# bghira/universal-metal-flash-attention

Measured on AMD Instinct MI355X. Metric: SDPA fwd TFLOPS (bf16) + int8 speedup, B=1 H=24 S=4096 D=128, 1/2/4/8 GPU, higher is better.
Workload: dtype bf16

## Files before the change

universal-metal-flash-attention_amd/csrc/fa_fwd16_w64.hip:

```cpp
#include <algorithm>
#include <cmath>
#include <cstdlib>
#include <type_traits>

#include "fa_fwd16_w64_params.h"

namespace umfa {

#define W64_I8 0
#define W64_BODY_INC "fa_fwd16_w64_body.inc"
#define W64_T __bf16
#define W64_MFMA "v_mfma_f32_32x32x16_bf16"
#define W64_MFMA_QK "v_mfma_f32_32x32x16_bf16"
#define W64_MSUM "v_mfma_f32_4x4x4_16b_bf16"
#define W64_ONES_BITS 0x3f803f80u
#define W64_LAZY_PARTS 1
#define W64_CVT "v_cvt_pk_bf16_f32"
#define W64_KERNEL fa_fwd16_w64_bf16
#include "fa_fwd16_w64_kernel.inc"
#undef W64_T
#undef W64_MFMA
#undef W64_MFMA_QK
#undef W64_MSUM
#undef W64_ONES_BITS
// ... 152 lines not shown
}

static int w64_cu_count() { return device_cu_count(); }

static bool w64_is_window(const FwdParams& p) { return p.mask_kind == MK_WINDOW; }
static uint32_t w64_win_left(const FwdParams& p) { return p.win_left < p.Sq ? p.win_left : p.Sq; }
static uint32_t w64_win_right(const FwdParams& p) { return p.causal ? 0u : (p.win_right < p.Skv ? p.win_right : p.Skv); }
static uint32_t w64_tiles_per_item(const FwdParams& p) {
    const uint32_t T = (p.Skv + 63) / 64;
    if (!w64_is_window(p)) return T;
    const uint64_t tw = ((uint64_t)w64_win_left(p) + 63) / 64 + (255ull + w64_win_right(p)) / 64 + 1;
    return tw < T ? (uint32_t)tw : T;
}

static uint32_t w64_grid(const FwdParams& p);

struct W64Cost { float t0, c_seg, t_step, c_fold, cast_a, cast_tbps; };
struct R128Cost { float t0, c_item, tau1, f2, f3, cast_a, cast_tbps, c_tail, g16; };
static const W64Cost kW64Cost[2][2] = {
    {{1.9654f, 5.6596f, 1.0164f, 1.8670f, 4.8672f, 4.1271f}, {9.3795f, 0.0000f, 1.1237f, 48.8617f, 2.7924f, 2.2478f}},
    {{0.4243f, 10.5808f, 1.5482f, 3.2266f, 3.4018f, 3.8643f}, {0.0000f, 6.7763f, 1.4334f, 52.2072f, 2.5095f, 2.6358f}}};
static const R128Cost kR128Cost[2][2] = {
    {{1.9627f, 3.9851f, 0.6098f, 2.0000f, 1.0000f, 0.0000f, 20.0000f, 1.3083f, 0.9054f}, {0.2449f, 5.9446f, 0.7894f, 1.4608f, 1.0000f, 0.0000f, 20.0000f, 0.6456f, 0.8727f}},
    {{0.0000f, 8.3967f, 1.0624f, 2.0000f, 2.8549f, 5.1811f, 20.0000f, 3.2320f, 1.0191f}, {0.0000f, 8.4229f, 1.2922f, 1.7176f, 1.0000f, 0.0000f, 12.7398f, 0.4806f, 0.8916f}}};
struct CbalCost { float a1, b1, a2, b2; };
static const CbalCost kCbalCost[2] = {{8.5243f, 1.1660f, 11.3665f, 1.3999f}, {11.7677f, 1.5652f, 21.1185f, 1.7844f}};

static double route_v_megabytes(const FwdParams& p) {
    return (double)(p.vs[0] == 0 ? 1u : p.B) * (p.vs[1] == 0 ? 1u : p.H) * p.Skv * p.D * 2.0 * 1e-6;
}

double fwd_w64_predict_us(const FwdParams& p) {
    const W64Cost& c = kW64Cost[p.D == 64 ? 0 : 1][p.causal ? 1 : 0];
    const uint64_t nqb = (p.Sq + 255) / 256, items = (uint64_t)p.B * p.H * nqb, T = (p.Skv + 63) / 64;
    const uint64_t G = w64_grid(p);
    double segs, steps, fold = 0.0;
    if (p.causal) {
        const uint64_t jobs = (uint64_t)p.B * p.H * ((nqb + 1) / 2), rounds = (jobs + G - 1) / G;
        uint64_t longest = 0;
        for (uint64_t j = 0; j < (nqb + 1) / 2; ++j) {
            const uint64_t a = std::min<uint64_t>(T, 4 * j + 4), m = nqb - 1 - j, b2 = m != j ? std::min<uint64_t>(T, 4 * m + 4) : 0;
            longest = std::max(longest, a + b2);
        }
        segs = 2.0 * rounds;
        steps = (double)(rounds * longest);
    } else {
        const uint64_t full = items / G, rem = items % G;
        segs = (double)(full + (rem ? 1 : 0));
        steps = (double)(full * T + (rem ? (rem * T + G - 1) / G : 0));
        if (rem) fold = std::max((double)G / (double)rem - 1.0, 0.0);
    }
    const double cast = (p.in_prec == P_BF16 && p.pv16) ? c.cast_a + 2.0 * route_v_megabytes(p) / c.cast_tbps : 0.0;
    return c.t0 + cast + segs * c.c_seg + steps * c.t_step + fold * c.c_fold;
}

double fwd_16_predict_us(const FwdParams& p) {
    const R128Cost& c = kR128Cost[p.D == 64 ? 0 : 1][p.causal ? 1 : 0];
    const uint64_t cus = (uint64_t)w64_cu_count();
    const uint64_t nqb = (p.Sq + 127) / 128, items = (uint64_t)p.B * p.H * nqb, T = (p.Skv + 63) / 64;
    const uint32_t R = (p.D == 128 && !p.causal) ? 3u : 2u;
    const double fr[4] = {0.0, 1.0, c.f2, c.f3};
    const double tau1 = (p.in_prec == P_BF16 && p.pv16) ? c.tau1 : c.tau1 * c.g16;
    const FwdSplitPlan plan = fwd_16_split_plan(p);
    const uint64_t k = plan.nsplit > 1 ? plan.nsplit : 1;
    const double n = (double)(items * k) / (double)cus;
    double body;
    if (plan.cbal) {
        const uint64_t lastq = nqb - 1;
        const double h = 0.5 * (double)(std::min<uint64_t>(T, 2) + std::min<uint64_t>(T, (lastq * 128 + 128 + 63) / 64));
        const CbalCost& cb = kCbalCost[p.D == 64 ? 0 : 1];
        const double one = cb.a1 + cb.b1 * h, two = cb.a2 + cb.b2 * h;
        const uint64_t full = (uint64_t)(n / 2.0);
        const double rest = n - 2.0 * (double)full;
        body = ((double)full * two + (rest > 1e-9 ? (rest <= 1.0 ? one : two) : 0.0)) * (p.in_prec == P_BF16 && p.pv16 ? 1.0 : (double)c.g16) - c.t0;
    } else if (p.causal) {
        uint64_t tot = 0, longest = 0;
        for (uint64_t qb = 0; qb < nqb; ++qb) {
            const uint64_t len = std::min<uint64_t>(T, (qb * 128 + 128 + 63) / 64);
            tot += len;
            longest = std::max(longest, len);
        }
        tot *= (uint64_t)p.B * p.H;
        if (n <= (double)R) {
            const int r = std::max(1, (int)std::ceil(n));
            body = c.c_item + (double)longest * tau1 * fr[r];
        } else {
            const double thr = (double)tot / (double)cus * tau1 * fr[R] / R + n * c.c_item / R;
            body = std::max(thr + c.c_tail * (double)longest * tau1, c.c_item + (double)longest * tau1 * fr[R]);
        }
    } else {
        const double L = (double)T / (double)k;
        const uint64_t full = (uint64_t)(n / R);
        const int rest = (int)std::ceil(n - (double)(full * R) - 1e-9);
        body = (double)full * (c.c_item + L * tau1 * fr[R]) + (rest > 0 ? c.c_item + L * tau1 * fr[rest] : 0.0) + (k > 1 ? c.c_tail * (double)k : 0.0);
    }
    const bool cast_on = p.in_prec == P_BF16 && p.pv16 && route_v_megabytes(p) * 1e6 >= (double)((size_t)16 << 20) && p.Sq >= 1024;
    const double cast = cast_on ? c.cast_a + 2.0 * route_v_megabytes(p) / c.cast_tbps : 0.0;
    return c.t0 + cast + body;
}

bool fwd_w64_supported(const FwdParams& p) {
    if (tuning().no_w64.load(std::memory_order_relaxed) || !fwd_16_supported(p)) return false;
    if ((p.D != 128 && p.D != 64) || (p.mask_kind != MK_NONE && p.mask_kind != MK_WINDOW && p.mask_kind != MK_BOOL && p.mask_kind != MK_F16 && p.mask_kind != MK_BF16 && p.mask_kind != MK_F32)) return false;
    if (p.mask_kind == MK_F16 || p.mask_kind == MK_BF16 || p.mask_kind == MK_F32) {
        if (tuning().no_w64_mask.load(std::memory_order_relaxed) || tuning().no_w64_bias.load(std::memory_order_relaxed) || !p.mask || (p.D != 128 && p.D != 64) || p.rope_cos || p.causal) return false;
        if (p.in_prec == P_BF16 && !p.pv16) return false;
        const bool ragged = !p.mask_padded && (p.Sq % 64 != 0 || p.Skv % 64 != 0);
        if (p.Sq < 256 || p.Skv < 64 || (p.Sq % 64 != 0 && p.Sq < 1024) || ((p.Skv + 63) / 64) > 1024u) return false;
        if (ragged && tuning().no_w64_ragged_mask.load(std::memory_order_relaxed)) return false;
        if (p.out_prec != P_FP32 && p.out_prec != p.in_prec) return false;
        if (p.ms[3] != 1) return false;
        if (!mask_needs_copy(p)) {
            if (((uintptr_t)p.mask & 15) != 0 || (p.ms[0] & 7) != 0 || (p.ms[1] & 7) != 0 || (p.ms[2] & 7) != 0) return false;
        } else if (tuning().no_w64_ragged_mask.load(std::memory_order_relaxed) && p.mask_kind == MK_F16) {
            return false;
        }
        if (p.mask_kind != MK_F32 && p.ms[2] != 0 && (uint64_t)p.ms[2] * 2 * 64 > 0x7fffffffull) return false;
        if (mask_copy_bytes(p) > ((size_t)1 << 30)) return false;
        if (p.mask_kind == MK_F32) {
            if (tuning().no_w64_f32_mask.load(std::memory_order_relaxed)) return false;
            const int ratio = tuning().f32_mask_ratio.load(std::memory_order_relaxed);
            if (ratio > 0) {
                const uint64_t Bm = p.ms[0] != 0 ? p.B : 1, Hm = p.ms[1] != 0 ? p.H : 1, eb = 2;
                const uint64_t mask_bytes = Bm * Hm * p.Sq * p.Skv * 4, qkvo = (uint64_t)p.B * p.H * p.D * ((uint64_t)p.Sq * (eb + 4) + 2ull * p.Skv * eb);
                if (mask_bytes > (uint64_t)ratio * qkvo) return false;
            } else if (!mask_flags_worthwhile(p)) {
                return false;
            }
        }
        if (w64_grid(p) > 512u) return false;
        if (tuning().force_w64.load(std::memory_order_relaxed)) return true;
        const uint64_t blocks = (uint64_t)p.B * p.H * ((p.Sq + 255) / 256), cus = (uint64_t)w64_cu_count();
        return blocks >= cus;
    }
    if (p.mask_kind == MK_BOOL) {
        if (tuning().no_w64_mask.load(std::memory_order_relaxed) || !p.mask || (p.D != 128 && p.D != 64) || p.rope_cos) return false;
        if (p.in_prec == P_BF16 && !p.pv16) return false;
        if (p.Skv < 64 || p.Sq < 256 || (p.Sq % 256 != 0 && p.Sq < 1024) || ((p.Skv + 63) / 64) > 1024u) return false;
        if (p.out_prec != P_FP32 && p.out_prec != p.in_prec) return false;
        const uint64_t blocks = (uint64_t)p.B * p.H * ((p.Sq + 255) / 256), cus = (uint64_t)w64_cu_count();
        if (w64_grid(p) > 512u) return false;
        if (tuning().force_w64.load(std::memory_order_relaxed)) return true;
        if (p.causal) return false;
        if (p.in_prec == P_BF16 && p.Sq < 1024) return false;
        if (p.in_prec == P_BF16 && p.Sq < 2048 && ((p.ms[0] == 0 && p.ms[1] == 0) || p.ms[2] == 0)) return false;
        return blocks >= cus || (p.ms[2] == 0 && blocks * ((p.Skv + 63) / 64) >= cus * 10) || ((p.ms[0] != 0 || p.ms[1] != 0) && blocks * 8 >= cus * 3);
    }
    if (w64_is_window(p) && p.rope_cos) return false;
    if (p.D == 64 && p.rope_cos) return false;
    if (p.Skv < 64 || p.Sq < 256 || (p.Sq % 256 != 0 && p.Sq < 1024)) return false;
    if (p.out_prec != P_FP32 && p.out_prec != p.in_prec) return false;
    if (!tuning().force_w64.load(std::memory_order_relaxed)) {
        if (w64_is_window(p)) {
            const uint64_t cus = (uint64_t)w64_cu_count(), nqb = (p.Sq + 255) / 256;
            const uint64_t items = (uint64_t)p.B * p.H * nqb, steps = items * w64_tiles_per_item(p);
            if (items % cus != 0 && steps < cus * 10) return false;
        } else if (!(fwd_w64_predict_us(p) < fwd_16_predict_us(p))) {
            return false;
        }
    }
    return true;
}

static uint32_t w64_grid(const FwdParams& p) {
    if (p.mask_kind == MK_BOOL || p.mask_kind == MK_F16 || p.mask_kind == MK_BF16) {
        const uint64_t items = (uint64_t)p.B * p.H * ((p.Sq + 255) / 256);
        const uint64_t cus = (uint64_t)w64_cu_count();
        if (const int gi = tuning().w64_grid.load(std::memory_order_relaxed)) {
            if (gi > 0 && (uint64_t)gi <= cus && (uint64_t)gi <= items && gi <= 512) return (uint32_t)gi;
        }
        const uint64_t gmax = cus < 512 ? cus : 512;
        if (items < cus) return (uint32_t)((p.ms[2] == 0 && items * ((p.Skv + 63) / 64) >= cus * 10) ? gmax : items);
        return (uint32_t)gmax;
    }
    const bool pairs = p.causal && !w64_is_window(p);
    uint64_t total = (uint64_t)p.B * p.H * ((p.Sq + 255) / 256) * w64_tiles_per_item(p);
    if (pairs) total = (uint64_t)p.B * p.H * (((p.Sq + 255) / 256 + 1) / 2);
    const uint32_t cus = (uint32_t)w64_cu_count();
    if (const int gi = tuning().w64_grid.load(std::memory_order_relaxed)) {
        const uint32_t g = (uint32_t)gi;
        if (gi > 0 && g <= cus && g <= total) return g;
    }
    if (!pairs) {
        const uint64_t items = (uint64_t)p.B * p.H * ((p.Sq + 255) / 256);
        if (items < cus && cus / items >= 2 && items * (cus / items) <= total) return (uint32_t)(items * (cus / items));
        if (items < cus && 2 * (uint64_t)w64_tiles_per_item(p) * (cus - items) < 35 * cus) return (uint32_t)items;
    }
    return total < cus ? (uint32_t)total : cus;
}

uint32_t fwd_w64_grid(const FwdParams& p) { return w64_grid(p); }

FwdW64Plan fwd_w64_plan(const FwdParams& p) {
    FwdW64Plan plan;
    const uint32_t items = p.B * p.H * ((p.Sq + 255) / 256);
    (void)items;
    plan.cnt_bytes = ((size_t)w64_grid(p) * sizeof(uint32_t) + 255) & ~(size_t)255;
    plan.buf_bytes = (size_t)2 * w64_grid(p) * (4 * 2 * 17 * 1024);
    return plan;
}

template <typename KFN>
static hipError_t launch_w64_kernel(KFN kfn, const FwdParams& p, const W64Params& wp, hipStream_t stream) {
    const uint32_t grid = w64_grid(p);
    const size_t lds = 65536 + 4 * 32 * (512 + 16) + 64 + 4096 + 8192 + 2048 + 64;
    if (hipError_t e = ensure_dynamic_lds((const void*)kfn, lds); e != hipSuccess) return e;
    hipLaunchKernelGGL(kfn, dim3(grid), dim3(256), lds, stream, wp);
    return hipGetLastError();
}

hipError_t launch_fwd_w64(const FwdParams& p, float* part_buf, uint32_t* part_cnt, hipStream_t stream, const char** name) {
    if (!fwd_w64_supported(p) || !part_buf || !part_cnt) return hipErrorNotSupported;
    W64Params wp;
    wp.q = p.q; wp.k = p.k; wp.v = p.v; wp.o = p.o; wp.lse = p.lse;
    for (int i = 0; i < 3; ++i) { wp.qs[i] = p.qs[i]; wp.ks[i] = p.ks[i]; wp.vs[i] = p.vs[i]; }
    wp.B = p.B; wp.H = p.H; wp.Sq = p.Sq; wp.Skv = p.Skv;
    wp.scale = p.scale;
    wp.n_items = p.B * p.H * ((p.Sq + 255) / 256);
    wp.T = (p.Skv + 63) / 64;
    wp.part_buf = part_buf;
    wp.part_cnt = part_cnt;
    w64_softmax_policy(p.in_prec, &wp.tau, &wp.lazy);
    wp.skew = (uint32_t)tuning().w64_skew.load(std::memory_order_relaxed);
    if (tuning().w64_skew.load(std::memory_order_relaxed) == -1) wp.skew = 0xffffffffu;
    wp.rope_cos = p.rope_cos; wp.rope_sin = p.rope_sin; wp.rope_tb = p.rope_tb;
    wp.vsc = p.vsc; wp.vsc_bs = p.vsc_bs; wp.vsc_hs = p.vsc_hs;
    if (p.in_prec == P_BF16 && p.pv16 && !p.vsc) return hipErrorInvalidValue;
    wp.Tw = wp.T; wp.win_left = wp.win_right = 0;
    const bool rope = p.rope_cos != nullptr, window = w64_is_window(p), fp32o = p.out_prec == P_FP32, maska = p.mask_kind == MK_F16, maskt = p.mask_kind == MK_BOOL || maska;
    wp.mask = nullptr; wp.mask_s[0] = wp.mask_s[1] = wp.mask_s[2] = 0;
    wp.guard = maska ? p.guard : nullptr;
    if (p.guard && (!maska || p.guard_want != 0u)) return hipErrorInvalidValue;
    if (maskt) {
        if ((!maska && !p.mk_bits) || !p.mk_list || !p.mk_cnt) return hipErrorInvalidValue;
        if (maska) { wp.mask = p.mask; wp.mask_s[0] = p.ms[0]; wp.mask_s[1] = p.ms[1]; wp.mask_s[2] = p.ms[2]; }
        wp.mk_bits = p.mk_bits; wp.mk_list = p.mk_list; wp.mk_cnt = p.mk_cnt;
        wp.mk_bs = p.mk_bs; wp.mk_hs = p.mk_hs; wp.mk_nrb64 = p.mk_nrb64;
        wp.mk_prefix = p.mk_prefix;
#ifndef W64_LAB_MASK_FORCE_LAZY
        if (p.ms[2] != 0 || p.causal || tuning().no_w64_mask_lazy.load(std::memory_order_relaxed)) wp.lazy = 0;
#endif
    }
    if (rope && p.out_prec != p.in_prec) return hipErrorNotSupported;
    if (window) {
        wp.Tw = w64_tiles_per_item(p);
        wp.win_left = (int32_t)w64_win_left(p);
        wp.win_right = (int32_t)w64_win_right(p);
    }
#define W64_FAMILY(FAM, T16, HAS_ROPE)                                                                                         \
    do {                                                                                                                       \
        if constexpr (HAS_ROPE >= 2) {        \
            if (maskt) return fp32o ? launch_w64_kernel(FAM<float, false, false, false, true>, p, wp, stream) : launch_w64_kernel(FAM<T16, false, false, false, true>, p, wp, stream); \
        }                                                                                                                      \
        if constexpr (HAS_ROPE == 1 || HAS_ROPE == 2) {                                                                        \
            if (rope) return p.causal ? launch_w64_kernel(FAM<T16, true, true>, p, wp, stream) : launch_w64_kernel(FAM<T16, false, true>, p, wp, stream); \
        }                                                                                                                      \
        if (window) return fp32o ? launch_w64_kernel(FAM<float, false, false, true>, p, wp, stream) : launch_w64_kernel(FAM<T16, false, false, true>, p, wp, stream); \
        if (p.causal) return fp32o ? launch_w64_kernel(FAM<float, true>, p, wp, stream) : launch_w64_kernel(FAM<T16, true>, p, wp, stream); \
        return fp32o ? launch_w64_kernel(FAM<float, false>, p, wp, stream) : launch_w64_kernel(FAM<T16, false>, p, wp, stream); \
    } while (0)
    static const char* const names[3][2][3] = {
        {{"fa_fwd16_w64<bf16,128>", "fa_fwd16_w64<bf16,128,rope>", "fa_fwd16_w64<bf16,128,window>"},
         {"fa_fwd16_w64<bf16,64>", "fa_fwd16_w64<bf16,64,rope>", "fa_fwd16_w64<bf16,64,window>"}},
        {{"fa_fwd16_w64<bf16,128,pv16>", "fa_fwd16_w64<bf16,128,pv16,rope>", "fa_fwd16_w64<bf16,128,pv16,window>"},
         {"fa_fwd16_w64<bf16,64,pv16>", "fa_fwd16_w64<bf16,64,pv16,rope>", "fa_fwd16_w64<bf16,64,pv16,window>"}},
        {{"fa_fwd16_w64<fp16,128>", "fa_fwd16_w64<fp16,128,rope>", "fa_fwd16_w64<fp16,128,window>"},
         {"fa_fwd16_w64<fp16,64>", "fa_fwd16_w64<fp16,64,rope>", "fa_fwd16_w64<fp16,64,window>"}}};
    if (p.D == 64 && rope) return hipErrorNotSupported;
    const int fam = p.in_prec == P_BF16 ? (p.pv16 ? 1 : 0) : 2;
    if (maskt && fam == 0) return hipErrorNotSupported;
    if (maska && fam == 0) return hipErrorNotSupported;
    if (maska) {
        *name = p.D == 64 ? (fam == 1 ? "fa_fwd16_w64<bf16,64,pv16,bias>" : "fa_fwd16_w64<fp16,64,bias>") : (fam == 1 ? "fa_fwd16_w64<bf16,128,pv16,bias>" : "fa_fwd16_w64<fp16,128,bias>");
        return launch_fwd_w64_bias(wp, fam, fp32o, w64_grid(p), 65536 + 4 * 32 * (512 + 16) + 64 + 4096 + 8192 + 2048 + 64, stream, (int)p.D);
    }
    *name = maska ? (fam == 1 ? "fa_fwd16_w64<bf16,128,pv16,bias>" : "fa_fwd16_w64<fp16,128,bias>") : maskt ? (p.D == 64 ? (fam == 1 ? "fa_fwd16_w64<bf16,64,pv16,mask>" : "fa_fwd16_w64<fp16,64,mask>")
                               : (fam == 1 ? "fa_fwd16_w64<bf16,128,pv16,mask>" : "fa_fwd16_w64<fp16,128,mask>"))
                  : names[fam][p.D == 64 ? 1 : 0][rope ? 1 : window ? 2 : 0];
    if (p.D == 64) {
        if (fam == 0) W64_FAMILY(fa_fwd16_w64d64_bf16, __bf16, 0);
        if (fam == 1) W64_FAMILY(fa_fwd16_w64d64_bf16pv16, __bf16, 3);
        W64_FAMILY(fa_fwd16_w64d64_f16, _Float16, 3);
    }
    if (fam == 0) W64_FAMILY(fa_fwd16_w64_bf16, __bf16, 1);
    if (fam == 1) W64_FAMILY(fa_fwd16_w64_bf16pv16, __bf16, 2);
    W64_FAMILY(fa_fwd16_w64_f16, _Float16, 2);
#undef W64_FAMILY
}

bool fwd_w64_i8_supported(const FwdParams& p) {
    if (tuning().no_w64.load(std::memory_order_relaxed) || p.D != 128) return false;
    if (!(p.scale > 0.0f)) return false;
    if (p.Skv < 64 || p.Sq < 256 || (p.Sq % 256 != 0 && p.Sq < 1024)) return false;
    if (p.mask_kind == MK_BOOL && p.mask) {
        if (tuning().no_w64_mask.load(std::memory_order_relaxed) || p.causal) return false;
        if (((p.Skv + 63) / 64) > 1024u || w64_grid(p) > 512u) return false;
        if (tuning().force_w64.load(std::memory_order_relaxed)) return true;
        const uint64_t blocks = (uint64_t)p.B * p.H * ((p.Sq + 255) / 256), cus = (uint64_t)w64_cu_count();
        return blocks >= cus || (p.ms[2] == 0 && blocks * ((p.Skv + 63) / 64) >= cus * 10) || ((p.ms[0] != 0 || p.ms[1] != 0) && blocks * 8 >= cus * 3);
    }
    return p.mask_kind == MK_NONE && !p.mask;
}

hipError_t launch_fwd_w64_i8(const FwdParams& p, const QuantViews& v, float* part_buf, uint32_t* part_cnt, hipStream_t stream) {
    if (!fwd_w64_i8_supported(p) || !part_buf || !part_cnt || v.dpq != 128) return hipErrorNotSupported;
    W64I8Params wp;
    wp.q8 = v.q8; wp.k8 = v.k8; wp.v16 = (const _Float16*)v.v16;
    wp.v8 = v.v8; wp.v_e8 = v.v_e8;
    wp.q_scale = v.q_scale; wp.k_scale = v.k_scale;
    wp.o = p.o; wp.lse = p.lse;
    wp.B = p.B; wp.H = p.H; wp.Sq = p.Sq; wp.Skv = p.Skv; wp.nqblk = v.nqblk; wp.nkblk = v.nkblk;
    wp.scale = p.scale;
    wp.n_items = p.B * p.H * ((p.Sq + 255) / 256);
    wp.T = (p.Skv + 63) / 64;
    wp.part_buf = part_buf;
    wp.part_cnt = part_cnt;
    w64_softmax_policy(P_FP16, &wp.tau, &wp.lazy);
    wp.skew = (uint32_t)tuning().w64_skew.load(std::memory_order_relaxed);
    wp.vsc = v.v8 ? nullptr : p.vsc;
    const uint32_t grid = w64_grid(p);
    const bool f8 = v.v8 != nullptr, maskt = p.mask_kind == MK_BOOL;
    wp.mk_bits = wp.mk_list = wp.mk_cnt = nullptr; wp.mk_bs = wp.mk_hs = wp.mk_nrb64 = 0;
    if (maskt) {
        if (f8 || p.causal || !p.mk_bits || !p.mk_list || !p.mk_cnt) return hipErrorInvalidValue;
        wp.mk_bits = p.mk_bits; wp.mk_list = p.mk_list; wp.mk_cnt = p.mk_cnt;
        wp.mk_bs = p.mk_bs; wp.mk_hs = p.mk_hs; wp.mk_nrb64 = p.mk_nrb64;
        if (p.ms[2] != 0 || tuning().no_w64_mask_lazy.load(std::memory_order_relaxed)) wp.lazy = 0;
    }
    const size_t lds = maskt ? 65536 + 4 * 32 * (512 + 16) + 64 + 4096 + 8192 + 2048 + 64 : 65536 + 4 * 32 * (512 + 16) + 16;
    auto kfn = f8 ? (p.causal ? fa_fwd_w64_i8f8<float, true> : fa_fwd_w64_i8f8<float, false>)
                  : maskt ? fa_fwd_w64_i8<float, false, true>
                          : (p.causal ? fa_fwd_w64_i8<float, true> : fa_fwd_w64_i8<float, false>);
    if (hipError_t e = ensure_dynamic_lds((const void*)kfn, lds); e != hipSuccess) return e;
    hipLaunchKernelGGL(kfn, dim3(grid), dim3(256), lds, stream, wp);
    return hipGetLastError();
}

}
```

universal-metal-flash-attention_amd/csrc/fa_fwd16_w64_kernel.inc:

```

#ifdef W64_ABL_NOBAR
#define W64_ITER_BARRIER() asm volatile("" ::: "memory")
#elif defined(W64_LAB_WAITSTAMP)
#define W64_ITER_BARRIER()                                                                         \
    do {                                                                                           \
        asm volatile("s_waitcnt lgkmcnt(0)" ::: "memory");                                         \
        const unsigned long long w0_ = __builtin_amdgcn_s_memtime();                               \
        asm volatile("s_waitcnt vmcnt(0) lgkmcnt(0)" ::: "memory");                                \
        const unsigned long long w1_ = __builtin_amdgcn_s_memtime();                               \
        asm volatile("s_waitcnt lgkmcnt(0)\n\ts_barrier" ::: "memory");                            \
        const unsigned long long w2_ = __builtin_amdgcn_s_memtime();                               \
        asm volatile("s_waitcnt lgkmcnt(0)" ::: "memory");                                         \
        st_wait += w1_ - w0_;                                                                      \
        st_bar += w2_ - w1_;                                                                       \
    } while (0)
#elif defined(W64_ABL_VMCNT8)
#define W64_ITER_BARRIER() asm volatile("s_waitcnt vmcnt(8) lgkmcnt(0)\n\ts_barrier" ::: "memory")
#else
#define W64_ITER_BARRIER() asm volatile("s_waitcnt vmcnt(0) lgkmcnt(0)\n\ts_barrier" ::: "memory")
#endif
#ifdef W64_ABL_NODMA
#define W64_DMA_ON 0
#else
#define W64_DMA_ON 1
// ... 74 lines not shown
    typedef typename M::V4 V4;
#if !W64_I8
    typedef V8 KF;
#endif
    typedef unsigned u32x4_t __attribute__((ext_vector_type(4)));
    constexpr int NDB = W64_DP / 32;
    constexpr int ROW_IN = 2 * W64_DP;
    constexpr int VSLOT = W64_F8 ? 8192 : 64 * ROW_IN;
    constexpr int VRING = W64_I8 ? 32768 : 2 * KSLOT;
    const float TAU = p.tau;
#if !W64_I8
    if constexpr (MASKA) {
        if (p.guard != nullptr && *p.guard != 0u) return;
    }
#endif

    extern __shared__ __attribute__((aligned(16))) char smem[];
    const int tid = threadIdx.x, lane = tid & 63, ql = lane & 31, hi = lane >> 5;
    const int uw = __builtin_amdgcn_readfirstlane(tid >> 6);
    const uint32_t lds0 = (uint32_t)(size_t)((LDS_AS char*)smem);
#ifndef W64_LAZY_PARTS
#define W64_LAZY_PARTS 0
#endif
#if W64_MSUM_ON && !W64_F8
    ms_init_ones(W64_ONES_BITS);
#define W64_L_ZERO() ms_zero_l()
#define W64_L_SCALE(A0, A1) ms_scale_l((A0), (A1))
#define W64_L_READ(L0, L1) ms_read_l((L0), (L1))
#elif !W64_F8
#define W64_L_ZERO() do { _Pragma("unroll") for (int j_ = 0; j_ < 4; ++j_) l4[0][j_] = l4[1][j_] = 0.0f; } while (0)
#define W64_L_SCALE(A0, A1) do { _Pragma("unroll") for (int j_ = 0; j_ < 4; ++j_) { l4[0][j_] *= (A0); l4[1][j_] *= (A1); } } while (0)
#define W64_L_READ(L0, L1) ((L0) = (l4[0][0] + l4[0][1]) + (l4[0][2] + l4[0][3]), (L1) = (l4[1][0] + l4[1][1]) + (l4[1][2] + l4[1][3]))
#endif
#if W64_LAZY_PARTS
    const bool lazy_on = p.lazy != 0;
    bool force_exact = false;
#ifndef W64_LAZY_HI16
#define W64_LAZY_HI16 0x1p10f
#endif
    constexpr float LAZY_HI = W64_LAZY_PARTS == 2 ? W64_LAZY_HI16 : 0x1p30f, LAZY_OVF = W64_LAZY_PARTS == 2 ? 0x1p15f : 0x1p100f;
    constexpr float LAZY_LOST = W64_LAZY_PARTS == 2 ? 0x1p-6f : 0x1p-100f;
    constexpr unsigned OVF_FLAG_OFF = 65536u + 4u * 32u * (512u + 16u);
    if (threadIdx.x == 0) *(volatile uint32_t LDS_AS*)(uintptr_t)(lds0 + OVF_FLAG_OFF) = 0u;
    __builtin_amdgcn_s_waitcnt(0xc07f);
#endif

    auto tr_read_at = [](unsigned addr) -> V4 {
        if constexpr (__is_same(T, __bf16)) {
            return __builtin_bit_cast(V4, __builtin_amdgcn_ds_read_tr16_b64_v4bf16((bf16x4_t LDS_AS*)(uintptr_t)addr));
        } else {
            return __builtin_bit_cast(V4, __builtin_amdgcn_ds_read_tr16_b64_v4i16((s16x4 LDS_AS*)(uintptr_t)addr));
        }
    };

    unsigned kaddr[KS];
#pragma unroll
    for (int ks = 0; ks < KS; ++ks)
        kaddr[ks] = lds0 + (unsigned)(W64_I8 ? k8_off_128(ql, 2 * ks + hi) : k_off<W64_DP>(ql, 2 * ks + hi));
    auto k_frag = [&](int koff, int ks) -> KF { return *(const KF LDS_AS*)(uintptr_t)(kaddr[ks] + (unsigned)koff); };
    const int tr_qq = (lane >> 2) & 3, tr_pp = lane & 3, tr_g1 = (lane >> 4) & 1;
    unsigned vtr[NDB];
#pragma unroll
    for (int i = 0; i < NDB; ++i)
        vtr[i] = lds0 + (unsigned)(v_off<W64_DP>(4 * hi + tr_qq, 4 * i + 2 * tr_g1 + (tr_pp >> 1)) + 8 * (tr_pp & 1));
    auto v_frag = [&](int voff, int db, int st) -> V8 {
        const V4 lo = tr_read_at(vtr[db] + (unsigned)(voff + (16 * st) * ROW_IN));
        const V4 hi4 = tr_read_at(vtr[db] + (unsigned)(voff + (16 * st + 8) * ROW_IN));
        return __builtin_shufflevector(lo, hi4, 0, 1, 2, 3, 4, 5, 6, 7);
    };
    (void)v_frag;

#if W64_F8
    typedef int i32x8 __attribute__((ext_vector_type(8)));
    const unsigned v8addr = lds0 + (unsigned)lane * 16u;
    auto v8_frag = [&](int voff, int db) -> i32x8 {
        const i32x4 lo = *(const i32x4 LDS_AS*)(uintptr_t)(v8addr + (unsigned)(voff + db * 2048));
        const i32x4 hi4 = *(const i32x4 LDS_AS*)(uintptr_t)(v8addr + (unsigned)(voff + db * 2048 + 1024));
        return __builtin_shufflevector(lo, hi4, 0, 1, 2, 3, 4, 5, 6, 7);
    };
#endif

#if W64_I8
    const int k_stride_b = 128, v_stride_b = 256, q_stride_b = 128;
#else
    const int k_stride_b = (int)p.ks[2] * 2, v_stride_b = (int)p.vs[2] * 2, q_stride_b = (int)p.qs[2] * 2;
#endif
    int kdma0[4], vdma0[4];
    {
        constexpr int RPI = 1024 / ROW_IN, CPR = ROW_IN / 16, PPW = 16 / RPI;
        const int d_r = lane / CPR, d_c = lane % CPR;
        (void)d_c;
#pragma unroll
        for (int j = 0; j < 4; ++j) {
            const int row = (uw * PPW + (j % PPW)) * RPI + d_r;
            (void)row;
#if W64_F8
            vdma0[j] = ((uw * 2 + (j & 1)) * 64 + lane) * 16;
#else
            vdma0[j] = row * v_stride_b + (v_off<W64_DP>(row, d_c) - row * ROW_IN);
#endif
#if W64_I8
            const int krow = (uw * 2 + (j & 1)) * 8 + (lane >> 3), kc = lane & 7;
            kdma0[j] = krow * 128 + (k8_off_128(krow, kc) - krow * 128);
#else
            kdma0[j] = row * k_stride_b + (k_off<W64_DP>(row, d_c) - row * ROW_IN);
#endif
        }
    }
    const int k_step0 = 64 * k_stride_b, v_step0 = W64_F8 ? 8192 : 64 * v_stride_b;
    const unsigned lds_wave = __builtin_amdgcn_readfirstlane(lds0 + (unsigned)uw * (W64_F8 ? 2048u : (unsigned)(16 * ROW_IN)));
#if W64_I8
    const unsigned lds_wave_k = __builtin_amdgcn_readfirstlane(lds0 + (unsigned)uw * 2048u);
    float c2 = 0.0f;
#ifndef W64_I8_NOBIAS
    constexpr float I8_BIAS = 12582912.0f;
#if W64_F8
    f8_init_consts();
#else
    i8_init_bias();
#endif
    float nmb[2] = {0.f, 0.f};
#endif
#else
    const unsigned lds_wave_k = lds_wave;
    const float c2 = p.scale * UMFA_LOG2E;
#endif

    const uint32_t G = gridDim.x;
    const uint32_t w = xcd_remap(blockIdx.x, G);
    const uint32_t T_ = p.T;
    const uint32_t nqb = (p.Sq + 255) / 256;
    const bool ktail = (p.Skv & 63) != 0;
    const uint32_t jobs_per_head = (nqb + 1) / 2, n_jobs = p.B * p.H * jobs_per_head;
    uint32_t Tst = T_;
    int win_left = 0, win_right = 0;
#if !W64_I8
    if constexpr (WINDOW) { Tst = p.Tw; win_left = p.win_left; win_right = p.win_right; }
#endif
    (void)win_left; (void)win_right;
    constexpr bool SPARSE = CAUSAL || WINDOW || MASKT;
    auto mk_slab = [&](uint32_t bh_) -> uint32_t { return (bh_ / p.H) * p.mk_bs + (bh_ % p.H) * p.mk_hs; };
    auto item_tiles = [&](uint32_t item) -> uint32_t {
        if constexpr (MASKT) return p.mk_cnt[mk_slab(item / nqb) * nqb + item % nqb];
        if constexpr (!CAUSAL) return Tst;
        const uint32_t q = item % nqb;
        return 4 * q + 4 < T_ ? 4 * q + 4 : T_;
    };
    const bool whole_rem = !CAUSAL && p.skew == 0xffffffffu;
    const uint32_t full_rounds = CAUSAL ? 0u : whole_rem ? (p.n_items + G - 1) / G : p.n_items / G;
    const uint32_t rem_items = (CAUSAL || whole_rem) ? 0u : p.n_items - full_rounds * G;
    constexpr unsigned MK_PREFIX_OFF = 65536u + 4u * 32u * (512u + 16u) + 64u + 4096u + 8192u;
    if constexpr (MASKT) {
        if (rem_items) {
            volatile uint32_t* const pf = (volatile uint32_t*)(smem + MK_PREFIX_OFF);
            const uint32_t first = full_rounds * G, j0 = threadIdx.x, j1 = threadIdx.x + 256u;
            for (uint32_t j = threadIdx.x; j < rem_items; j += 256u) {
                const uint32_t it_ = first + j;
                pf[1 + j] = p.mk_cnt[mk_slab(it_ / nqb) * nqb + it_ % nqb];
            }
            if (threadIdx.x == 0) pf[0] = 0u;
            __syncthreads();
            for (uint32_t off = 1; off < rem_items; off <<= 1) {
                const uint32_t a0 = (j0 < rem_items && j0 >= off) ? pf[1 + j0 - off] : 0u;
                const uint32_t a1 = (j1 < rem_items && j1 >= off) ? pf[1 + j1 - off] : 0u;
                __syncthreads();
                if (j0 < rem_items) pf[1 + j0] += a0;
                if (j1 < rem_items) pf[1 + j1] += a1;
                __syncthreads();
            }
        }
    }
    auto mk_prefix_at = [&](uint32_t j) -> uint32_t {
        return (uint32_t)__builtin_amdgcn_readfirstlane((int)((volatile const uint32_t*)(smem + MK_PREFIX_OFF))[j]);
    };
    (void)mk_prefix_at;
    auto item_start = [&](uint32_t litem) -> uint64_t {
        if constexpr (MASKT) return mk_prefix_at(litem);
        return (uint64_t)litem * Tst;
    };
    auto item_of_step = [&](uint64_t step) -> uint32_t {
        if constexpr (MASKT) {
            uint32_t lo = 0, hi_ = rem_items - 1;
            while (lo < hi_) {
                const uint32_t mid = (lo + hi_ + 1) >> 1;
                if (mk_prefix_at(mid) <= step) lo = mid; else hi_ = mid - 1;
            }
            return lo;
        }
        return (uint32_t)(step / Tst);
    };
    const uint64_t total = MASKT ? (rem_items ? (uint64_t)mk_prefix_at(rem_items) : 0ull) : (uint64_t)rem_items * Tst;
    const uint32_t skew = (!MASKT && rem_items && G == 2 * rem_items && p.skew != 0xffffffffu && 2 * p.skew < Tst) ? p.skew : 0u;
    const uint32_t Gs = (MASKT && total < G) ? (uint32_t)total : G;
    auto slice_bound = [&](uint32_t g) -> uint32_t {
        if constexpr (MASKT) { if (g >= Gs) return (uint32_t)total; }
        return (uint32_t)(total * g / Gs) - ((g & 1u) ? skew : 0u);
    };
    const uint32_t s_begin = slice_bound(w), s_end = slice_bound(w + 1);
#ifdef W64_LAB_GAPSTAMP
    unsigned long long st_g[4] = {0, 0, 0, 0}, st_gprev = 0;
#define W64_GSTAMP(k)                                                                            \
    do {                                                                                         \
        asm volatile("s_waitcnt lgkmcnt(0)" ::: "memory");                                       \
        const unsigned long long now_ = __builtin_amdgcn_s_memtime();                            \
        asm volatile("s_waitcnt lgkmcnt(0)" ::: "memory");                                       \
        if (st_gprev) st_g[k] += now_ - st_gprev;                                                \
        st_gprev = now_;                                                                         \
    } while (0)
#endif
#ifdef W64_LAB_FSTAMP
    unsigned long long fs_now[8] = {0, 0, 0, 0, 0, 0, 0, 0};
    uint32_t fs_acc[8] = {0, 0, 0, 0, 0, 0, 0, 0}, fs_last = 0, fs_tiles = 0;
    bool fs_valid = false;
#define W64_FSTAMP(k) asm volatile("s_memtime %0" : "=s"(fs_now[k]))
#define W64_FSTAMP_END(n)                                                                           \
    do {                                                                                            \
        asm volatile("s_waitcnt lgkmcnt(0)" ::: "memory");                                          \
        if (fs_valid) fs_acc[0] += (uint32_t)fs_now[0] - fs_last;                                   \
        _Pragma("unroll") for (int k_ = 1; k_ < (n); ++k_) fs_acc[k_] += (uint32_t)fs_now[k_] - (uint32_t)fs_now[k_ - 1]; \
        fs_last = (uint32_t)fs_now[(n) - 1];                                                        \
        fs_valid = true;                                                                            \
        ++fs_tiles;                                                                                 \
    } while (0)
#endif
#ifdef W64_LAB_STAMPS
    const unsigned long long st_rt0 = __builtin_amdgcn_s_memrealtime(), st_ck0 = __builtin_amdgcn_s_memtime();
    unsigned long long st_pro = 0, st_loop = 0, st_drain = 0, st_epi = 0, st_t = 0, st_wait = 0, st_bar = 0;
#define W64_STAMP(acc) do { const unsigned long long now_ = __builtin_amdgcn_s_memtime(); acc += now_ - st_t; st_t = now_; } while (0)
#else
#define W64_STAMP(acc) do { } while (0)
#endif

    uint32_t ntail = 0;
    bool tail_first = false;
    if (s_end > s_begin) {
        const uint32_t it0 = item_of_step(s_begin), it1 = item_of_step(s_end - 1);
        ntail = it1 - it0 + 1;
        tail_first = item_start(it0) != s_begin;
    }
    const uint32_t my_jobs = CAUSAL ? (n_jobs > w ? (n_jobs - w + G - 1) / G : 0u) : 0u;
    const uint32_t nseg = CAUSAL ? 2 * my_jobs : full_rounds + ntail;

    auto make_srd = [&](const void* base, uint32_t bytes) {
        const unsigned long long a = (unsigned long long)base;
        i32x4 d;
        d[0] = __builtin_amdgcn_readfirstlane((int)(a & 0xffffffffu));
        d[1] = __builtin_amdgcn_readfirstlane((int)((a >> 32) & 0xffffu));
        d[2] = __builtin_amdgcn_readfirstlane((int)bytes);
        d[3] = 0x00020000;
        return d;
    };
    auto seg_decode = [&](uint32_t si_, uint32_t& item_, uint32_t& t0_, uint32_t& n_, uint32_t& litem_, bool& desc_) -> bool {
        litem_ = 0;
        desc_ = false;
        if constexpr (CAUSAL) {
            const uint32_t job = (si_ >> 1) * G + w, jbh = job / jobs_per_head, jj = job % jobs_per_head;
            desc_ = (si_ & 1) != 0;
            const uint32_t q = desc_ ? nqb - 1 - jj : jj;
            if (desc_ && q == jj) return false;
            item_ = jbh * nqb + q;
            t0_ = 0;
            n_ = item_tiles(item_);
        } else {
            const bool is_tail = tail_first ? (si_ < ntail) : (si_ >= full_rounds);
            if (is_tail) {
                const uint32_t ti = tail_first ? si_ : si_ - full_rounds;
                litem_ = item_of_step(s_begin) + ti;
                const uint64_t ist = item_start(litem_), ien = MASKT ? item_start(litem_ + 1) : ist + Tst;
                const uint64_t sb = ist > s_begin ? ist : s_begin, se = ien < s_end ? ien : s_end;
                t0_ = (uint32_t)(sb - ist);
                n_ = (uint32_t)(se - sb);
                item_ = full_rounds * G + litem_;
            } else {
                item_ = (tail_first ? si_ - ntail : si_) * G + w;
                if (item_ >= p.n_items) return false;
                t0_ = 0;
                n_ = MASKT ? item_tiles(item_) : Tst;
            }
        }
        return true;
    };
#ifndef W64_MFMA16
#define W64_MFMA16 "v_mfma_f32_16x16x32_bf16"
#endif
#ifndef W64_PREFETCH_NEXT
#define W64_PREFETCH_NEXT 0
#endif
#if W64_PREFETCH_NEXT
    static_assert(!WINDOW, "the prefetch computes the next segment's first tile without the window offset");
    KF qf[2][KS];
    int kdma[4];
    bool have_pref = false;
#endif
#if W64_I8
    constexpr bool ROPE_ON = false;
    (void)ROPE_ON;
#else
    constexpr bool ROPE_ON = ROPE;
    (void)ROPE_ON;
#endif

    for (uint32_t si = 0; si < nseg; ++si) {
        int tid_s = tid;
        if constexpr (MASKA) asm volatile("" : "+v"(tid_s));
        const int lane = tid_s & 63, ql = lane & 31, hi = lane >> 5;
#ifdef W64_LAB_STAMPS
        if (si) { asm volatile("s_waitcnt vmcnt(0)" ::: "memory"); W64_STAMP(st_epi); }
#endif
        uint32_t item, t0, n, litem = 0;
        bool desc = false;
#if W64_LAZY_PARTS
        bool lazy = lazy_on && !force_exact;
        force_exact = false;
        bool ovf = false;
#endif
        if (!seg_decode(si, item, t0, n, litem, desc)) continue;
#if !W64_PREFETCH_NEXT
        KF qf[2][KS];
        int kdma[4];
        constexpr bool have_pref = false;
#endif
        auto issue_q_k0 = [&](uint32_t item_, uint32_t tfirst_, int k_step_) {
            const uint32_t bh_ = item_ / nqb, qblk_ = item_ % nqb;
            const uint32_t q0_ = qblk_ * 256 + (uint32_t)uw * 64;
#if W64_I8
            const int8_t* qp_ = p.q8 + (int64_t)bh_ * p.Sq * 128;
            const int8_t* kp_ = p.k8 + (int64_t)bh_ * p.Skv * 128;
            const auto q_rsrc_ = __builtin_amdgcn_make_buffer_rsrc((void*)qp_, 0, (int)(p.Sq * 128u), 0x00020000);
            const i32x4 k_srd_ = make_srd(kp_, p.Skv * 128u);
#else
            const uint32_t b_ = bh_ / p.H, h_ = bh_ % p.H;
            const T* qp_ = (const T*)p.q + ((int64_t)b_ * p.qs[0] + (int64_t)h_ * p.qs[1]);
            const T* kp_ = (const T*)p.k + ((int64_t)b_ * p.ks[0] + (int64_t)h_ * p.ks[1]);
            const auto q_rsrc_ = __builtin_amdgcn_make_buffer_rsrc((void*)qp_, 0, (int)((p.Sq - 1) * (uint32_t)q_stride_b + ROW_IN), 0x00020000);
            const i32x4 k_srd_ = make_srd(kp_, (p.Skv - 1) * (uint32_t)k_stride_b + ROW_IN);
#endif
#pragma unroll
            for (int j = 0; j < 4; ++j) kdma[j] = kdma0[j] + (int)tfirst_ * k_step0;
#pragma unroll
            for (int j = 0; j < (W64_I8 ? 2 : W64_DP / 32); ++j) {
                asm volatile("s_mov_b32 m0, %0\n\ts_nop 0\n\tbuffer_load_dwordx4 %1, %2, 0 offen lds"
                             ::"s"(lds_wave_k + j * 1024), "v"(kdma[j]), "s"(k_srd_) : "memory");
                kdma[j] += k_step_;
            }
#pragma unroll
            for (int qb = 0; qb < 2; ++qb) {
                const int qoff = (int)(q0_ + 32 * qb + ql) * q_stride_b + 16 * hi;
#pragma unroll
                for (int ks = 0; ks < KS; ++ks)
                    qf[qb][ks] = __builtin_bit_cast(KF, __builtin_amdgcn_raw_buffer_load_b128(q_rsrc_, qoff + 32 * ks, 0, 0));
            }
        };
        const uint32_t Ti = item_tiles(item);
        const uint32_t bh = item / nqb, qblk = item % nqb;
        const uint32_t b = bh / p.H, h = bh % p.H;
        const uint32_t q0 = qblk * 256 + (uint32_t)uw * 64;

#if W64_I8
        (void)b; (void)h;
        const int8_t* qp = p.q8 + (int64_t)bh * p.Sq * 128;
        const int8_t* kp = p.k8 + (int64_t)bh * p.Skv * 128;
#if W64_F8
        const uint8_t* vp = p.v8 + (int64_t)bh * T_ * 8192;
        const uint32_t* __restrict__ vexp = p.v_e8 + (int64_t)bh * p.nkblk;
        const i32x4 v_srd = make_srd(vp, T_ * 8192u);
#else
        const _Float16* vp = p.v16 + (int64_t)bh * p.Skv * 128;
        const i32x4 v_srd = make_srd(vp, p.Skv * 256u);
#endif
        const auto q_rsrc = __builtin_amdgcn_make_buffer_rsrc((void*)qp, 0, (int)(p.Sq * 128u), 0x00020000);
        const i32x4 k_srd = make_srd(kp, p.Skv * 128u);
        const float sq = (q0 < p.Sq ? p.q_scale[(int64_t)bh * p.nqblk + q0 / 64] : 0.0f) * p.scale * UMFA_LOG2E;
        const float* __restrict__ ksc = p.k_scale + (int64_t)bh * p.nkblk;
        int sc_win = -1;
        float ksc_w = 0.0f;
#if W64_F8
        unsigned vexp_w = 0x7f7f7f7fu;
#endif
        auto load_scale_window = [&](uint32_t tile) {
            const int win = (int)(tile >> 6);
            if (win != sc_win) {
                sc_win = win;
                const uint32_t t = ((uint32_t)win << 6) + (uint32_t)lane;
                ksc_w = t < p.nkblk ? ksc[t] : 0.0f;
#if W64_F8
                vexp_w = t < p.nkblk ? vexp[t] : 0x7f7f7f7fu;
#endif
                __builtin_amdgcn_s_waitcnt(0x0F70);
            }
        };
        auto k_scale_of = [&](uint32_t tile) -> float {
            load_scale_window(tile);
            return __builtin_bit_cast(float, __builtin_amdgcn_readlane(__builtin_bit_cast(int, ksc_w), (int)(tile & 63u)));
        };
#ifndef W64_I8_NOBIAS
        float kmax = 0.0f;
        for (uint32_t t = lane; t < p.nkblk; t += 64) kmax = fmaxf(kmax, ksc[t]);
#pragma unroll
        for (int off = 32; off > 0; off >>= 1) kmax = fmaxf(kmax, __shfl_xor(kmax, off, 64));
        const float bias_bound = fmaxf(I8_BIAS * 1.25f * sq * kmax, 0x1p-60f);
        const int eb = ((__builtin_bit_cast(int, bias_bound) >> 23) & 0xff) - 126;
        const float mgrid = __builtin_bit_cast(float, (eb - 24 + 127) << 23), inv_mgrid = __builtin_bit_cast(float, (24 - eb + 127) << 23);
        const float cgrid = __builtin_bit_cast(float, (eb - 46 + 127) << 23), inv_cgrid = __builtin_bit_cast(float, (46 - eb + 127) << 23);
#define W64_C2(x) (__builtin_rintf((x) * inv_cgrid) * cgrid)
#define W64_MGRID(x) (__builtin_ceilf((x) * inv_mgrid) * mgrid)
#if W64_LAZY_PARTS
        lazy = lazy && eb <= 24;
#endif
#else
#define W64_C2(x) (x)
#define W64_MGRID(x) (x)
#endif
#else
#define W64_MGRID(x) (x)
        const T* qp = (const T*)p.q + ((int64_t)b * p.qs[0] + (int64_t)h * p.qs[1]);
        const T* kp = (const T*)p.k + ((int64_t)b * p.ks[0] + (int64_t)h * p.ks[1]);
        const T* vp = (const T*)p.v + ((int64_t)b * p.vs[0] + (int64_t)h * p.vs[1]);
        const auto q_rsrc = __builtin_amdgcn_make_buffer_rsrc((void*)qp, 0, (int)((p.Sq - 1) * (uint32_t)q_stride_b + ROW_IN), 0x00020000);
        const i32x4 k_srd = make_srd(kp, (p.Skv - 1) * (uint32_t)k_stride_b + ROW_IN);
        const i32x4 v_srd = make_srd(vp, (p.Skv - 1) * (uint32_t)v_stride_b + ROW_IN);
#endif

        uint32_t toff = 0;
        if constexpr (WINDOW) {
            const uint32_t blk0 = qblk * 256u;
            const uint32_t lo = blk0 > (uint32_t)win_left ? (blk0 - (uint32_t)win_left) / 64u : 0u;
            toff = lo < T_ - Tst ? lo : T_ - Tst;
        }
        uint32_t tfirst = toff + (desc ? n - 1 : t0);
        int k_step = desc ? -k_step0 : k_step0, v_step = desc ? -v_step0 : v_step0;
        const int dm_step = desc ? -64 : 64;
        const uint32_t* __restrict__ mk_lst = MASKT ? p.mk_list + (uint64_t)(mk_slab(bh) * nqb + qblk) * T_ * 2 : nullptr;
        constexpr unsigned MK_LIST_OFF = 65536u + 4u * 32u * (512u + 16u) + 64u + 4096u;
        const unsigned mk_list_lds = lds0 + MK_LIST_OFF;
        uint32_t mk_tile = 0, mk_cls = 2, mk_next = 0;
        uint32_t mk_ncls = 0;
        (void)mk_ncls;
        auto mk_class = [&](uint32_t) -> uint32_t { return mk_cls; };
        auto tile_at = [&](uint32_t i) -> uint32_t {
            if constexpr (MASKT) return mk_tile;
            return toff + (desc ? n - 1 - i : t0 + i);
        };
        auto mk_steps = [&](uint32_t i) {
            if constexpr (MASKT) {
                typedef unsigned u32x2_t __attribute__((ext_vector_type(2)));
                const u32x2_t e = *(const u32x2_t LDS_AS*)(uintptr_t)(mk_list_lds + 8u * i);
                const uint32_t e0 = (uint32_t)__builtin_amdgcn_readfirstlane((int)e[0]), e1 = (uint32_t)__builtin_amdgcn_readfirstlane((int)e[1]);
                mk_tile = e0 & 0xffffu;
                mk_cls = (e0 >> (16 + 2 * uw)) & 3u;
                mk_ncls = (e0 >> (24 + 2 * uw)) & 3u;
                mk_next = e1 & 0xffffu;
                k_step = ((int)(e1 >> 16) - (int)mk_next) * k_step0;
                v_step = ((int)mk_next - (int)mk_tile) * v_step0;
            }
        };
        unsigned mwc[2] = {0u, 0u}, mtmp;
        i32x4 mk_srd = {0, 0, 0, 0};
        constexpr unsigned MK_RING_OFF = 65536u + 4u * 32u * (512u + 16u) + 64u;
        const unsigned mk_ring = __builtin_amdgcn_readfirstlane(lds0 + MK_RING_OFF + (unsigned)uw * 1024u);
        if constexpr (MASKT && !MASKA) {
            const uint32_t rb64 = 4 * qblk + (uint32_t)uw;
            mk_srd = make_srd(p.mk_bits + ((uint64_t)mk_slab(bh) * p.mk_nrb64 + rb64) * T_ * 128, rb64 < p.mk_nrb64 ? T_ * 512u : 0u);
        }
#if !W64_I8
        typedef unsigned u32x2_t __attribute__((ext_vector_type(2)));
        u32x2_t mta[2][2] = {};
        (void)mta;
        int ma_col = -1;
        int ma_soff = 0;
        (void)ma_col; (void)ma_soff;
        i32x4 ma_srd = {0, 0, 0, 0};
        const unsigned ma_ring = __builtin_amdgcn_readfirstlane(lds0 + 65536u + (unsigned)uw * (32u * (512u + 16u)));
        unsigned ma_lane = (unsigned)lane;
        asm volatile("" : "+v"(ma_lane));
        unsigned ma_x16 = 0, ma_row0 = 0;
        auto ma_loop_constants = [&]() {
            if constexpr (MASKA) {
                unsigned l2 = ma_lane;
                asm volatile("" : "+v"(l2));
                const unsigned ql_ = l2 & 31u, hi_ = l2 >> 5;
                ma_x16 = 16u * (ql_ & 7u);
                ma_row0 = ma_ring + 128u * ql_ + 8u * hi_;
            }
        };
        const float ma_k = MASKA ? __builtin_bit_cast(float, __builtin_amdgcn_readfirstlane(__builtin_bit_cast(int, 1.0f / p.scale))) : 0.0f;
        int ma_voff = 0, ma_rs8 = 0;
        (void)ma_row0; (void)ma_x16; (void)ma_k;
        auto ma_read = [&](unsigned off, unsigned c16) -> u32x2_t {
            unsigned a;
            if (c16 & 64u) asm volatile("v_xad_u32 %0, %1, %2, %3\n\tv_xor_b32 %0, 64, %0" : "=v"(a) : "v"(ma_x16), "n"(c16 & 48u), "v"(ma_row0));
            else asm volatile("v_xad_u32 %0, %1, %2, %3" : "=v"(a) : "v"(ma_x16), "n"(c16 & 48u), "v"(ma_row0));
            return *(const u32x2_t LDS_AS*)(uintptr_t)(a + off);
        };
        (void)ma_read;
        if constexpr (MASKA) {
            const int64_t rs = p.mask_s[2];
            const _Float16* mp = (const _Float16*)p.mask + ((int64_t)b * p.mask_s[0] + (int64_t)h * p.mask_s[1] + (int64_t)q0 * rs);
            ma_srd = make_srd(mp, q0 < p.Sq ? (rs ? (uint32_t)(64 * rs * 2) : p.T * 128u) : 0u);
            ma_rs8 = (int)(8 * rs * 2);
            ma_voff = (int)(ma_lane >> 3) * (int)(rs * 2) + 16 * (int)((ma_lane & 7u) ^ ((ma_lane >> 3) & 7u));
        }
#endif
        auto mk_request = [&](uint32_t i, uint32_t tile) {
#if !W64_I8
            if constexpr (MASKA) {
                if (i == 0) {
                    if (mk_cls != 2u) {
                        const int col = (int)(tile * 128u);
#pragma unroll
                        for (int j = 0; j < 8; ++j)
                            asm volatile("s_mov_b32 m0, %0\n\ts_nop 0\n\tbuffer_load_dwordx4 %1, %2, %3 offen lds"
                                         :: "s"(ma_ring + (unsigned)j * 1024u), "v"(ma_voff), "s"(ma_srd), "s"(col + j * ma_rs8) : "memory");
                    }
                } else {
                    ma_col = mk_ncls != 2u ? (int)(tile * 128u) : -1;
                    ma_soff = ma_col;
                }
            } else
#endif
            if constexpr (MASKT) {
                const int voff = (int)(tile * 512u) + lane * 4;
                const unsigned dst = mk_ring + (i & 1u) * 512u;
                asm volatile("s_mov_b32 m0, %0\n\ts_nop 0\n\tbuffer_load_dword %1, %2, 0 offen lds\n\t"
                             "buffer_load_dword %1, %2, 0 offen offset:256 lds"
                             :: "s"(dst), "v"(voff), "s"(mk_srd) : "memory");
            }
        };
        auto mk_take = [&](uint32_t i) {
            if constexpr (MASKT && !MASKA) {
                const unsigned a = mk_ring + (i & 1u) * 512u + (unsigned)lane * 4u;
                mwc[0] = *(const unsigned LDS_AS*)(uintptr_t)a;
                mwc[1] = *(const unsigned LDS_AS*)(uintptr_t)(a + 256u);
            }
        };
        (void)mtmp;
        if constexpr (MASKT) {
            asm volatile("s_barrier" ::: "memory");
            for (uint32_t j = (uint32_t)tid; j < 2 * n; j += 256u) *(unsigned LDS_AS*)(uintptr_t)(mk_list_lds + 4u * j) = mk_lst[2 * t0 + j];
            __builtin_amdgcn_s_waitcnt(0x0F70);
            asm volatile("s_waitcnt lgkmcnt(0)\n\ts_barrier" ::: "memory");
            mk_steps(0);
            tfirst = mk_tile;
            k_step = ((int)mk_next - (int)mk_tile) * k_step0;
        }
        auto win_edge = [&](uint32_t t) -> bool {
            const int64_t k0_ = 64 * (int64_t)t;
            return k0_ + 63 > (int64_t)q0 + win_right || k0_ + win_left < (int64_t)q0 + 63;
        };
        (void)win_edge;
        int vdma[4];
#pragma unroll
        for (int j = 0; j < 4; ++j) vdma[j] = vdma0[j] + (int)tfirst * v_step0;

#ifdef W64_LAB_STAMPS
        st_t = __builtin_amdgcn_s_memtime();
#endif
        asm volatile("s_barrier" ::: "memory");
        mk_request(0, tfirst);
        KF kf[2][KS];
#if !W64_I8
        if constexpr (ROPE) {
#pragma unroll
            for (int j = 0; j < 4; ++j) kdma[j] = kdma0[j] + (int)tfirst * k_step0;
#pragma unroll
            for (int j = 0; j < 4; ++j) {
                asm volatile("s_mov_b32 m0, %0\n\ts_nop 0\n\tbuffer_load_dwordx4 %1, %2, 0 offen lds"
                             ::"s"(lds_wave_k + j * 1024), "v"(kdma[j]), "s"(k_srd) : "memory");
                kdma[j] += k_step;
            }
            const unsigned qst = lds0 + 65536u + (unsigned)uw * (32 * (512 + 16));
#pragma unroll 4
            for (int it = 0; it < 16; ++it) {
                const int r = it * 4 + (lane >> 4), c = lane & 15;
                const uint32_t row = q0 + (uint32_t)r;
                const V8 v = __builtin_bit_cast(V8, __builtin_amdgcn_raw_buffer_load_b128(q_rsrc, (int)row * q_stride_b + 16 * c, 0, 0));
                const int64_t at = (int64_t)b * p.rope_tb + (int64_t)(row < p.Sq ? row : 0) * 128 + 8 * c;
                const V8 o = rope_fragment<T, V8>(v, p.rope_cos, p.rope_sin, at);
                *(V8 LDS_AS*)(uintptr_t)(qst + (unsigned)(r * 256 + ((c ^ (r & 15)) << 4))) = o;
            }
            __builtin_amdgcn_fence(__ATOMIC_RELEASE, "wavefront");
            __builtin_amdgcn_wave_barrier();
            __builtin_amdgcn_fence(__ATOMIC_ACQUIRE, "wavefront");
#pragma unroll
            for (int qb = 0; qb < 2; ++qb) {
                const int r = 32 * qb + ql;
#pragma unroll
                for (int ks = 0; ks < KS; ++ks)
                    qf[qb][ks] = *(const V8 LDS_AS*)(uintptr_t)(qst + (unsigned)(r * 256 + (((2 * ks + hi) ^ (r & 15)) << 4)));
            }
        } else
#endif
        {
            (void)q_rsrc;
            if (!have_pref) issue_q_k0(item, tfirst, k_step);
        }
#if W64_PREFETCH_NEXT
        have_pref = false;
#endif
        zero_o();
#if !W64_F8
#if !W64_MSUM_ON
        float l4[2][4];
#endif
        W64_L_ZERO();
#endif
        asm volatile("s_waitcnt vmcnt(0)\n\ts_barrier" ::: "memory");
        __builtin_amdgcn_s_waitcnt(0x0F70);
#pragma unroll
        for (int ks = 0; ks < 4; ++ks) kf[0][ks] = k_frag(0, ks);

#if W64_F8
        i32x8 vf8[4];
        f8_zero_l();
#else
        V8 vf[4][NDB];
#endif
        float mr[2] = {-INFINITY, -INFINITY}, mo[2] = {-INFINITY, -INFINITY}, nm[2] = {0.f, 0.f}, mx[2][2] = {{0.f, 0.f}, {0.f, 0.f}};
        bool pending = false;
        float em[2] = {0.f, 0.f};
        int dmask[2], dleft = 0;
        {
            constexpr int NEVER = -(1 << 28);
#ifdef W64_FORCE_MASKED
            const int causal_term = NEVER;
#else
            const int diag_term = (int)(64 * tfirst) + 4 * hi - (int)q0 - ql;
            const int causal_term = CAUSAL ? diag_term : WINDOW ? diag_term - win_right : NEVER;
            if constexpr (WINDOW) dleft = diag_term + win_left;
#endif
#pragma unroll
            for (int qb = 0; qb < 2; ++qb) {
                const int tail_term = ktail ? (int)(64 * tfirst) + 4 * hi - (int)p.Skv + 1 + 32 * qb : NEVER;
                dmask[qb] = causal_term > tail_term ? causal_term : tail_term;
            }
        }
        (void)dleft;
        const float neg_inf = -INFINITY;
        const uint32_t diag0 = 4 * qblk;

#if W64_I8 && !defined(W64_I8_NOBIAS)
#define W64_UNBIAS(x) ((x) - I8_BIAS)
#define W64_SET_NMB() (nmb[0] = __builtin_fmaf(-I8_BIAS, c2, nm[0]), nmb[1] = __builtin_fmaf(-I8_BIAS, c2, nm[1]))
#else
#define W64_UNBIAS(x) (x)
#define W64_SET_NMB() ((void)0)
#endif
#define W64_DECIDE()                                                                                            \
    do {                                                                                                        \
        const float mc0 = W64_UNBIAS(max_xor32(fmaxf(mx[0][0], mx[0][1]))) * c2;                                \
        const float mc1 = W64_UNBIAS(max_xor32(fmaxf(mx[1][0], mx[1][1]))) * c2;                                \
        pending = __builtin_amdgcn_ballot_w64((mc0 - mr[0] > TAU) | (mc1 - mr[1] > TAU)) != 0;                  \
        mo[0] = mr[0];                                                                                          \
        mo[1] = mr[1];                                                                                          \
        mr[0] = pending ? W64_MGRID(fmaxf(mr[0], mc0)) : mr[0];                                                 \
        mr[1] = pending ? W64_MGRID(fmaxf(mr[1], mc1)) : mr[1];                                                 \
         \
        nm[0] = (W64_NMSEL && SPARSE && mr[0] == -INFINITY) ? 0.0f : -mr[0];                                                 \
        nm[1] = (W64_NMSEL && SPARSE && mr[1] == -INFINITY) ? 0.0f : -mr[1];                                                 \
        W64_SET_NMB();                                                                                          \
    } while (0)

#if W64_F8
#define W64_SCALE_LACC(A0, A1) f8_scale_l((A0), (A1))
#define W64_SET_VSC(T) (load_scale_window(T), f8_set_vscale((unsigned)__builtin_amdgcn_readlane((int)vexp_w, (int)((T) & 63u))))
#else
#define W64_SCALE_LACC(A0, A1) W64_L_SCALE((A0), (A1))
#define W64_SET_VSC(T) ((void)0)
#endif
#define W64_DECIDE2()                                                                                           \
    do {                                                                                                        \
        em[0] = max_xor32(fmaxf(mx[0][0], mx[0][1]));                                                           \
        em[1] = max_xor32(fmaxf(mx[1][0], mx[1][1]));                                                           \
         \
        pending = __builtin_amdgcn_ballot_w64((em[0] > TAU) | (em[1] > TAU) |                                   \
                                              (SPARSE && ((mr[0] == -INFINITY && em[0] > -INFINITY) |           \
                                                          (mr[1] == -INFINITY && em[1] > -INFINITY)))) != 0;    \
    } while (0)
#define W64_MOVE_REF(FIX)                                                                                       \
    do {                                                                                                        \
        const float mc0 = em[0] - nm[0], mc1 = em[1] - nm[1];      \
        mo[0] = mr[0];                                                                                          \
        mo[1] = mr[1];                                                                                          \
        mr[0] = W64_MGRID(fmaxf(mr[0], mc0));                                                                   \
        mr[1] = W64_MGRID(fmaxf(mr[1], mc1));                                                                   \
        const float n0 = (W64_NMSEL && SPARSE && mr[0] == -INFINITY) ? 0.0f : -mr[0];                           \
        const float n1 = (W64_NMSEL && SPARSE && mr[1] == -INFINITY) ? 0.0f : -mr[1];                           \
        FIX(n0 - nm[0], n1 - nm[1]);                                                                            \
        nm[0] = n0;                                                                                             \
        nm[1] = n1;                                                                                             \
    } while (0)
#define W64_NOFIX(A, B) ((void)0)

#define W64_END_ITER(KNEXT, RESCALE, FIX)                                                                        \
    do {                                                                                                        \
        if (W64_RESCALE_ON && (RESCALE) && pending) {                                                           \
            if (W64_SPEC) W64_MOVE_REF(FIX);                                                                    \
            const float a0 = mo[0] == mr[0] ? 1.0f : __builtin_amdgcn_exp2f(mo[0] - mr[0]);                     \
            const float a1 = mo[1] == mr[1] ? 1.0f : __builtin_amdgcn_exp2f(mo[1] - mr[1]);                     \
            asm volatile("s_nop 15\n\ts_nop 15");                                                               \
            scale_o0(a0);                                                                                       \
            scale_o1(a1);                                                                                       \
            W64_SCALE_LACC(a0, a1);                                                                             \
        }                                                                                                       \
        W64_END_BARRIER(KNEXT);                                                                                 \
    } while (0)

#if W64_LAZY_PARTS
#if W64_MSUM_ON
#define W64_LAZY_QUICK()                                                                                        \
        unsigned long long c0_, c1_;                                                                            \
        asm volatile("v_cmp_nle_f32_e64 %0, v118, %2\n\tv_cmp_nle_f32_e64 %1, v122, %2"                         \
                     : "=s"(c0_), "=s"(c1_) : "s"(LAZY_HI));                                                    \
        const bool lazy_hit_ = (c0_ | c1_) != 0
#elif defined(W64_LAB_NOLAZYCHK)
#define W64_LAZY_QUICK() const bool lazy_hit_ = false
#else
#define W64_LAZY_QUICK()                                                                                        \
        float q0_, q1_;                                                                                         \
        W64_L_READ(q0_, q1_);                                                                                   \
        const bool lazy_hit_ = __builtin_amdgcn_ballot_w64(!(q0_ <= LAZY_HI) | !(q1_ <= LAZY_HI)) != 0
#endif
#define W64_END_ITER_LAZY(KNEXT, FIX)                                                                           \
    do {                                                                                                        \
        W64_LAZY_QUICK();                                                                                       \
        if (lazy_hit_ && !ovf) {                                                                                \
            float l0_, l1_;                                                                                     \
            W64_L_READ(l0_, l1_);                                                                               \
            const float r0_ = l0_ + xor32(l0_), r1_ = l1_ + xor32(l1_);                                         \
            if (__builtin_amdgcn_ballot_w64(!(r0_ < LAZY_OVF) | !(r1_ < LAZY_OVF)) != 0) {                      \
                ovf = true;                                                                                     \
            } else {                                                                                            \
                const int k0_ = r0_ >= 2.0f ? (int)((__builtin_bit_cast(unsigned, r0_) >> 23) & 0xffu) - 127 : 0; \
                const int k1_ = r1_ >= 2.0f ? (int)((__builtin_bit_cast(unsigned, r1_) >> 23) & 0xffu) - 127 : 0; \
                const float s0_ = __builtin_bit_cast(float, (unsigned)(127 - k0_) << 23);                       \
                const float s1_ = __builtin_bit_cast(float, (unsigned)(127 - k1_) << 23);                       \
                asm volatile("s_nop 15\n\ts_nop 15");                                                           \
                W64_L_SCALE(s0_, s1_);                                                                          \
                scale_o0(s0_);                                                                                  \
                scale_o1(s1_);                                                                                  \
                mr[0] += (float)k0_;                                                                            \
                mr[1] += (float)k1_;                                                                            \
                nm[0] = -mr[0];                                                                                 \
                nm[1] = -mr[1];                                                                                 \
                FIX(-(float)k0_, -(float)k1_);                                                                  \
            }                                                                                                   \
        }                                                                                                       \
        W64_END_BARRIER(KNEXT);                                                                                 \
    } while (0)
#endif

#if !W64_I8
        ma_loop_constants();
#endif
        W64_STAMP(st_pro);
#define W64_KOFF 0
#define W64_KNEXT KSLOT
#define W64_VOFF 0
#define W64_KDST KSLOT
#define W64_VDST VRING
#define W64_MOFF 0u
#define W64_MDST 8192u
#if W64_I8
        c2 = W64_C2(sq * k_scale_of(tile_at(0)));
#endif
        mk_steps(0);
        mk_request(1, mk_next);
        if (W64_MASKED_TILE(0)) {
            mk_take(0);
#define W64_PART 5
#include W64_BODY_INC
#undef W64_PART
        } else {
#define W64_PART 0
#include W64_BODY_INC
#undef W64_PART
        }
        dmask[0] += dm_step;
        dmask[1] += dm_step;
        if constexpr (WINDOW) dleft += dm_step;
        W64_END_ITER(KSLOT, false, W64_NOFIX);
#if W64_LAZY_PARTS
        if (SPARSE && lazy) {
            mr[0] = mr[0] == -INFINITY ? 0.0f : mr[0];
            mr[1] = mr[1] == -INFINITY ? 0.0f : mr[1];
            nm[0] = -mr[0];
            nm[1] = -mr[1];
        }
#endif
#undef W64_KOFF
#undef W64_KNEXT
#undef W64_VOFF
#undef W64_KDST
#undef W64_VDST
#undef W64_MOFF
#undef W64_MDST

        uint32_t i = 1;
        bool last_a;
        while (true) {
            if (i >= n) { last_a = true; break; }
#define W64_KOFF KSLOT
#define W64_KNEXT 0
#define W64_VOFF VRING
#define W64_KDST 0
#define W64_VDST (VRING + VSLOT)
#define W64_MOFF 8192u
#define W64_MDST 0u
            mk_steps(i);
            mk_request(i + 1, mk_next);
#if W64_I8
            c2 = W64_C2(sq * k_scale_of(tile_at(i)));
            W64_SET_NMB();
            W64_SET_VSC(tile_at(i - 1));
#endif
#if W64_LAZY_PARTS
            if (lazy) {
                if (W64_MASKED_TILE(i)) {
                    mk_take(i);
#define W64_PART 10
#include W64_BODY_INC
#undef W64_PART
                } else {
#define W64_PART 8
#include W64_BODY_INC
#undef W64_PART
                }
                dmask[0] += dm_step;
                dmask[1] += dm_step;
                if constexpr (WINDOW) dleft += dm_step;
                W64_END_ITER_LAZY(0, fix_e_b);
            } else
#endif
            {
            if (W64_MASKED_TILE(i)) {
                mk_take(i);
#define W64_PART 6
#include W64_BODY_INC
#undef W64_PART
            } else {
#define W64_PART 1
#include W64_BODY_INC
#undef W64_PART
            }
            dmask[0] += dm_step;
            dmask[1] += dm_step;
            if constexpr (WINDOW) dleft += dm_step;
            W64_END_ITER(0, true, fix_e_b);
            }
#undef W64_KOFF
#undef W64_KNEXT
#undef W64_VOFF
#undef W64_KDST
#undef W64_VDST
#undef W64_MOFF
#undef W64_MDST
            ++i;
            if (i >= n) { last_a = false; break; }
#define W64_KOFF 0
#define W64_KNEXT KSLOT
#define W64_VOFF (VRING + VSLOT)
#define W64_KDST KSLOT
#define W64_VDST VRING
#define W64_MOFF 0u
#define W64_MDST 8192u
            mk_steps(i);
            mk_request(i + 1, mk_next);
#if W64_I8
            c2 = W64_C2(sq * k_scale_of(tile_at(i)));
            W64_SET_NMB();
            W64_SET_VSC(tile_at(i - 1));
#endif
#if W64_LAZY_PARTS
            if (lazy) {
                if (W64_MASKED_TILE(i)) {
                    mk_take(i);
#define W64_PART 11
#include W64_BODY_INC
#undef W64_PART
                } else {
#define W64_PART 9
#include W64_BODY_INC
#undef W64_PART
                }
                dmask[0] += dm_step;
                dmask[1] += dm_step;
                if constexpr (WINDOW) dleft += dm_step;
                W64_END_ITER_LAZY(KSLOT, fix_e_a);
            } else
#endif
            {
            if (W64_MASKED_TILE(i)) {
                mk_take(i);
#define W64_PART 7
#include W64_BODY_INC
#undef W64_PART
            } else {
#define W64_PART 2
#include W64_BODY_INC
#undef W64_PART
            }
// ... 332 lines not shown
```

universal-metal-flash-attention_amd/csrc/fa_fwd16_w64_params.h:

```cpp
#pragma once
#include <cstdint>

#include "fa_common.h"
#include "fa_fwd_16_kernel.h"
#include "kernels.h"

namespace umfa {

struct W64Params {
    const void* q;
    const void* k;
    const void* v;
    void* o;
    float* lse;
    int64_t qs[3], ks[3], vs[3];
    uint32_t B, H, Sq, Skv;
    float scale;
    uint32_t n_items, T;
    float* part_buf;
    uint32_t* part_cnt;
    float tau;
    uint32_t lazy;
    uint32_t skew;
    uint32_t Tw;
    int32_t win_left, win_right;
    const float* rope_cos;
    const float* rope_sin;
    int64_t rope_tb;
    const uint32_t* mk_bits;
    const uint32_t* mk_list;
    const uint32_t* mk_cnt;
    uint32_t mk_bs, mk_hs, mk_nrb64;
    const uint32_t* mk_prefix;
    const void* mask;
    int64_t mask_s[3];
    const float* vsc;
    uint32_t vsc_bs, vsc_hs;
    const uint32_t* guard;
};

#include "fa_fwd16_w64_regs.inc"

__device__ __forceinline__ constexpr int k8_off_128(int row, int ch) { return row * 128 + 16 * (ch ^ ((row >> 1) & 7)); }

struct W64I8Params {
    const int8_t* q8;
    const int8_t* k8;
    const _Float16* v16;
    const uint8_t* v8;
    const uint32_t* v_e8;
    const float* q_scale;
    const float* k_scale;
    void* o;
    float* lse;
    uint32_t B, H, Sq, Skv, nqblk, nkblk;
    float scale;
    uint32_t n_items, T;
    float* part_buf;
    uint32_t* part_cnt;
    float tau;
    uint32_t lazy;
    uint32_t skew;
    const uint32_t* mk_bits;
    const uint32_t* mk_list;
    const uint32_t* mk_cnt;
    uint32_t mk_bs, mk_hs, mk_nrb64;
    const float* vsc;
};

hipError_t launch_fwd_w64_bias(const W64Params& wp, int family, bool fp32_out, uint32_t grid, size_t lds, hipStream_t stream, int head_dim);

}
```

universal-metal-flash-attention_amd/csrc/fa_quant.hip:

```cpp
#include <climits>
#include <cstring>

#include <type_traits>

#include "fa_common.h"
#include "kernels.h"

namespace umfa {

#define LDS_AS __attribute__((address_space(3)))
typedef _Float16 f16x4_t __attribute__((ext_vector_type(4)));

constexpr int QBLK = 64;

struct QuantParams {
    const void* src[3];
    int8_t* q8;
    int8_t* k8;
    _Float16* v16;
    uint8_t* v8;
    uint32_t* v_e8;
    float* f32[3];
    _Float16* f16[3];
    uint32_t* overflow;
    float* scale[3];
    uint32_t rows[3];
    uint32_t nblk[3];
    uint32_t BH, D, DPQ;
    int in_prec;
    float qmax;
    int qlo, qhi;
    int t_first, t_end;
    uint32_t* vhdr;
    const uint32_t* famax;
    int v_exchange;
    uint32_t wait_ticks;
};

__device__ __forceinline__ int vimage_exponent(unsigned amax_b16) {
    if (amax_b16 == 0) return 0;
    int E = (int)(amax_b16 >> 7);
    E = E > 254 ? 254 : E;
    const int e = (E ? E - 127 : -126) - 13;
    return e < -100 ? -100 : e;
}
__device__ __forceinline__ float exp2i(int e) { return __uint_as_float((unsigned)(127 + e) << 23); }

__device__ __forceinline__ int v8_off(int kk, int d) {
    const int k32 = kk & 31, h = (k32 >> 2) & 1, b = (k32 & 3) + 4 * (k32 >> 3);
    return (d >> 5) * 2048 + (kk >> 5) * 1024 + (32 * h + (d & 31)) * 16 + b;
}

__device__ __forceinline__ float div_by_block_scale(float a, float b, float r1) {
    const float q0 = a * r1;
    const float e1 = __builtin_fmaf(-b, q0, a);
    const float q1 = __builtin_fmaf(e1, r1, q0);
    const float e2 = __builtin_fmaf(-b, q1, a);
    return __builtin_fmaf(e2, r1, q1);
}

typedef float f32x2_t __attribute__((ext_vector_type(2)));
__device__ __forceinline__ void quant_pair_fast(float a0, float a1, float b, float r1, int qlo, int qhi, int& q0, int& q1) {
    const f32x2_t a = {a0, a1}, bb = {b, b}, rr = {r1, r1};
    const f32x2_t y0 = a * rr;
    const f32x2_t e1 = __builtin_elementwise_fma(-bb, y0, a);
    const f32x2_t y1 = __builtin_elementwise_fma(e1, rr, y0);
    const f32x2_t e2 = __builtin_elementwise_fma(-bb, y1, a);
    const f32x2_t y = __builtin_elementwise_fma(e2, rr, y1);
    const f32x2_t h = {__builtin_copysignf(0x1.fffffep-2f, y[0]), __builtin_copysignf(0x1.fffffep-2f, y[1])};
    const f32x2_t t = y + h;
    q0 = max(min((int)t[0], qhi), qlo);
    q1 = max(min((int)t[1], qhi), qlo);
}

template <int MODE, bool IN16>
__global__ __launch_bounds__(256) void quantize_kernel(QuantParams p) {
    __shared__ float red[4];
    __shared__ __attribute__((aligned(16))) unsigned char v8img[8192];
    constexpr int MAXC = 8;
    typedef unsigned u32x4 __attribute__((ext_vector_type(4)));
    uint32_t id = blockIdx.x;
    int t = p.t_first;
    while (t < p.t_end - 1 && id >= p.BH * p.nblk[t]) { id -= p.BH * p.nblk[t]; ++t; }
    const uint32_t bh = id / p.nblk[t], blk = id % p.nblk[t];
    const uint32_t row0 = blk * QBLK;
    const uint32_t nrows = min((uint32_t)QBLK, p.rows[t] - row0);
    const int64_t base = ((int64_t)bh * p.rows[t] + row0) * p.D;
    const uint32_t cpr = p.D / 8;
    const uint32_t nchunks = nrows * cpr;
    const int tid = threadIdx.x;
    const bool is_bf16 = p.in_prec == P_BF16;

    typename std::conditional<IN16, u32x4, f32x4>::type xr[MAXC][IN16 ? 1 : 2];
    auto X = [&](int c, int j) -> float {
        if constexpr (IN16) {
            const unsigned w = xr[c][0][j >> 1];
            if (is_bf16) return __uint_as_float((j & 1) ? (w & 0xffff0000u) : (w << 16));
            return (float)__builtin_bit_cast(_Float16, (uint16_t)((j & 1) ? (w >> 16) : (w & 0xffffu)));
        } else {
            return xr[c][j >> 2][j & 3];
        }
    };
    float amax = 0.0f;
#pragma unroll
    for (int c = 0; c < MAXC; ++c) {
        const uint32_t ch = tid + 256 * c;
        if (ch < nchunks) {
            const int64_t e0 = base + (int64_t)ch * 8;
            if constexpr (IN16) {
                xr[c][0] = *(const u32x4*)((const uint16_t*)p.src[t] + e0);
            } else {
                xr[c][0] = *(const f32x4*)((const float*)p.src[t] + e0);
                xr[c][1] = *(const f32x4*)((const float*)p.src[t] + e0 + 4);
            }
        }
    }
#pragma unroll
    for (int c = 0; c < MAXC; ++c) {
        const uint32_t ch = tid + 256 * c;
        if (ch < nchunks) {
#pragma unroll
            for (int j = 0; j < 8; ++j) amax = fmaxf(amax, fabsf(X(c, j)));
        }
    }
    float sc;
    if (MODE != 1) {
#pragma unroll
        for (int off = 32; off > 0; off >>= 1) amax = fmaxf(amax, __shfl_xor(amax, off, 64));
        if ((tid & 63) == 0) red[tid >> 6] = amax;
        __syncthreads();
        amax = fmaxf(fmaxf(red[0], red[1]), fmaxf(red[2], red[3]));
        if (MODE == 0) {
            if (tid == 0) p.scale[t][bh * p.nblk[t] + blk] = amax;
            return;
        }
        sc = amax > 0.0f ? amax / p.qmax : 1.0f;
        if (tid == 0) p.scale[t][bh * p.nblk[t] + blk] = sc;
    } else {
        sc = p.scale[t][bh * p.nblk[t] + blk];
    }
    if (MODE == 2 && t == 2 && p.v8) {
        int e = 0;
        if (amax > 0.0f) {
            (void)frexpf(amax * (1.0f / 448.0f), &e);
            e = e < -126 ? -126 : e;
        }
        const float inv = __builtin_amdgcn_ldexpf(1.0f, -e);
        if (tid == 0) {
            const uint32_t byte = (uint32_t)(e + 127) & 0xffu;
            p.v_e8[bh * p.nblk[2] + blk] = byte * 0x01010101u;
            p.scale[2][bh * p.nblk[2] + blk] = __builtin_amdgcn_ldexpf(1.0f, e);
        }
        *(i32x4*)(v8img + tid * 32) = i32x4{0, 0, 0, 0};
        *(i32x4*)(v8img + tid * 32 + 16) = i32x4{0, 0, 0, 0};
        __syncthreads();
#pragma unroll
        for (int c = 0; c < MAXC; ++c) {
            const uint32_t ch = tid + 256 * c;
            if (ch < nchunks) {
                const int r = (int)(ch / cpr), d0 = (int)(ch % cpr) * 8;
#pragma unroll
                for (int j = 0; j < 8; j += 2) {
                    const unsigned w = (unsigned)__builtin_amdgcn_cvt_pk_fp8_f32(X(c, j) * inv, X(c, j + 1) * inv, 0, false);
                    v8img[v8_off(r, d0 + j)] = (unsigned char)(w & 0xff);
                    v8img[v8_off(r, d0 + j + 1)] = (unsigned char)((w >> 8) & 0xff);
                }
            }
        }
        __syncthreads();
        uint8_t* dst = p.v8 + ((int64_t)bh * p.nblk[2] + blk) * 8192;
        *(i32x4*)(dst + tid * 16) = *(const i32x4*)(v8img + tid * 16);
        *(i32x4*)(dst + 4096 + tid * 16) = *(const i32x4*)(v8img + 4096 + tid * 16);
        return;
    }
    const int64_t orow0 = (int64_t)bh * p.rows[t] + row0;
    const float rcp0 = __builtin_amdgcn_rcpf(sc);
    const float rcp1 = __builtin_fmaf(__builtin_fmaf(-sc, rcp0, 1.0f), rcp0, rcp0);
    const bool fast_div = sc >= 0x1p-60f && sc <= 0x1p60f;
    const float scv = (t == 2 && p.vhdr) ? sc * exp2i(-vimage_exponent(p.vhdr[VSC_HDR_WORDS * (size_t)bh + VSC_HDR_AMAX])) : sc;
    const float scf = p.famax ? sc * exp2i(-unit_exponent(p.famax[t])) : sc;
    bool f16_ovf = false;
#pragma unroll
    for (int c = 0; c < MAXC; ++c) {
        const uint32_t ch = tid + 256 * c;
        if (ch < nchunks) {
            const uint32_t r = ch / cpr, d0 = (ch % cpr) * 8;
            int q[8];
#pragma unroll
            for (int j = 0; j < 8; ++j) {
                const float xv = X(c, j);
                const float y = fast_div ? div_by_block_scale(xv, sc, rcp1) : xv / sc;
                const float half = __builtin_copysignf(0x1.fffffep-2f, y);
                const int qv = (int)(y + half);
                q[j] = max(min(qv, p.qhi), p.qlo);
            }
            if (t < 2) {
                const uint32_t a0 = __builtin_amdgcn_perm((uint32_t)q[1], (uint32_t)q[0], 0x0c0c0400u);
                const uint32_t a1 = __builtin_amdgcn_perm((uint32_t)q[3], (uint32_t)q[2], 0x04000c0cu);
                const uint32_t b0 = __builtin_amdgcn_perm((uint32_t)q[5], (uint32_t)q[4], 0x0c0c0400u);
                const uint32_t b1 = __builtin_amdgcn_perm((uint32_t)q[7], (uint32_t)q[6], 0x04000c0cu);
                const uint32_t w0 = a0 | a1, w1 = b0 | b1;
                int8_t* dst = (t == 0 ? p.q8 : p.k8) + (orow0 + r) * p.DPQ + d0;
                *(uint2*)dst = make_uint2(w0, w1);
            } else {
                f16x8 hv;
#pragma unroll
                for (int j = 0; j < 8; ++j) hv[j] = (_Float16)((float)q[j] * scv);
                *(f16x8*)(p.v16 + (orow0 + r) * p.DPQ + d0) = hv;
            }
            if (p.f16[t]) {
                f16x8 hv;
#pragma unroll
                for (int j = 0; j < 8; ++j) {
                    const float y = (float)q[j] * scf;
                    f16_ovf |= !(fabsf(y) <= 65504.0f);
                    hv[j] = (_Float16)y;
                }
                *(f16x8*)(p.f16[t] + (orow0 + r) * p.D + d0) = hv;
            }
            if (p.f32[t]) {
                float* f = p.f32[t] + (orow0 + r) * p.D + d0;
                *(f32x4*)f = f32x4{(float)q[0] * sc, (float)q[1] * sc, (float)q[2] * sc, (float)q[3] * sc};
                *(f32x4*)(f + 4) = f32x4{(float)q[4] * sc, (float)q[5] * sc, (float)q[6] * sc, (float)q[7] * sc};
            }
        }
    }
    if (f16_ovf && p.overflow) atomicOr(p.overflow, 1u);
    if (p.DPQ > p.D) {
        const uint32_t padc = (p.DPQ - p.D) / 8;
        for (uint32_t e = tid; e < nrows * padc; e += 256) {
            const uint32_t r = e / padc, d0 = p.D + (e % padc) * 8;
            if (t < 2) *(uint2*)((t == 0 ? p.q8 : p.k8) + (orow0 + r) * p.DPQ + d0) = make_uint2(0u, 0u);
            else *(i32x4*)(p.v16 + (orow0 + r) * p.DPQ + d0) = i32x4{0, 0, 0, 0};
        }
    }
}

typedef unsigned u32x4_q __attribute__((ext_vector_type(4)));
template <bool BF16> __device__ __forceinline__ float q16_elem(const u32x4_q& x, int j) {
    const unsigned w = x[j >> 1];
    if constexpr (BF16) return __uint_as_float((j & 1) ? (w & 0xffff0000u) : (w << 16));
    return (float)__builtin_bit_cast(_Float16, (uint16_t)((j & 1) ? (w >> 16) : (w & 0xffffu)));
}
template <int CPL, bool BF16, bool FAST, bool ISV>
__device__ __forceinline__ void quantize_wave_convert(const u32x4_q (&xr)[CPL], int lane, uint32_t nchunks, float sc, float rcp1, int qlo, int qhi,
                                                      int8_t* __restrict__ dst8, _Float16* __restrict__ dst16, float scv) {
#pragma unroll
    for (int c = 0; c < CPL; ++c) {
        const uint32_t ch = (uint32_t)lane + 64u * c;
        if (ch < nchunks) {
            int q[8];
            if constexpr (FAST) {
#pragma unroll
                for (int j = 0; j < 8; j += 2) quant_pair_fast(q16_elem<BF16>(xr[c], j), q16_elem<BF16>(xr[c], j + 1), sc, rcp1, qlo, qhi, q[j], q[j + 1]);
            } else {
#pragma unroll
                for (int j = 0; j < 8; ++j) {
                    const float y = q16_elem<BF16>(xr[c], j) / sc;
                    const float half = __builtin_copysignf(0x1.fffffep-2f, y);
                    q[j] = max(min((int)(y + half), qhi), qlo);
                }
            }
            if constexpr (!ISV) {
                const uint32_t a0 = __builtin_amdgcn_perm((uint32_t)q[1], (uint32_t)q[0], 0x0c0c0400u);
                const uint32_t a1 = __builtin_amdgcn_perm((uint32_t)q[3], (uint32_t)q[2], 0x04000c0cu);
                const uint32_t b0 = __builtin_amdgcn_perm((uint32_t)q[5], (uint32_t)q[4], 0x0c0c0400u);
                const uint32_t b1 = __builtin_amdgcn_perm((uint32_t)q[7], (uint32_t)q[6], 0x04000c0cu);
                *(uint2*)(dst8 + (int64_t)ch * 8) = make_uint2(a0 | a1, b0 | b1);
            } else {
                f16x8 hv;
#pragma unroll
                for (int j = 0; j < 8; ++j) hv[j] = (_Float16)((float)q[j] * scv);
                *(f16x8*)(dst16 + (int64_t)ch * 8) = hv;
            }
        }
    }
}

template <int CPL, bool BF16>
__global__ __launch_bounds__(256) void quantize_wave_kernel(QuantParams p) {
    const int lane = threadIdx.x & 63;
    uint32_t id = blockIdx.x * 4 + (threadIdx.x >> 6);
    int t = p.t_first;
    while (t < p.t_end - 1 && id >= p.BH * p.nblk[t]) { id -= p.BH * p.nblk[t]; ++t; }
    if (id >= p.BH * p.nblk[t]) return;
    const uint32_t bh = id / p.nblk[t], blk = id % p.nblk[t];
    const uint32_t row0 = blk * QBLK;
    const uint32_t nrows = min((uint32_t)QBLK, p.rows[t] - row0);
    constexpr uint32_t cpr = CPL;
    const uint32_t nchunks = nrows * cpr;
    const int64_t base = ((int64_t)bh * p.rows[t] + row0) * (int64_t)(8 * cpr);
    const uint16_t* __restrict__ src = (const uint16_t*)p.src[t] + base;
    u32x4_q xr[CPL];
#pragma unroll
    for (int c = 0; c < CPL; ++c) {
        const uint32_t ch = (uint32_t)lane + 64u * c;
        xr[c] = ch < nchunks ? __builtin_nontemporal_load((const u32x4_q*)(src + (int64_t)ch * 8)) : u32x4_q{0, 0, 0, 0};
    }
    float amax = 0.0f;
#pragma unroll
    for (int c = 0; c < CPL; ++c)
#pragma unroll
        for (int j = 0; j < 8; ++j) amax = fmaxf(amax, fabsf(q16_elem<BF16>(xr[c], j)));
#pragma unroll
    for (int off = 32; off > 0; off >>= 1) amax = fmaxf(amax, __shfl_xor(amax, off, 64));
#pragma unroll
    for (int c = 0; c < CPL; ++c) asm volatile("" : "+v"(xr[c]));
    int vexp = 0;
    if (t == 2 && p.vhdr) {
        uint32_t* const hw = p.vhdr + VSC_HDR_WORDS * (size_t)bh;
        if (p.v_exchange) {
            __shared__ unsigned wg_amax[4], slab_amax;
            const int wave = threadIdx.x >> 6;
            if (lane == 0) wg_amax[wave] = __float_as_uint(amax) >> 16;
            __syncthreads();
            const uint32_t chunk = blk >> 2, chunks = p.nblk[2] >> 2;
            if (wave == 0) {
                unsigned m = wg_amax[0];
                for (int w = 1; w < 4; ++w) m = wg_amax[w] > m ? wg_amax[w] : m;
                if (lane == 0) __hip_atomic_store(hw + chunk, 0x80000000u | m, __ATOMIC_RELAXED, __HIP_MEMORY_SCOPE_AGENT);
                const uint64_t t_in = __builtin_amdgcn_s_memrealtime();
                unsigned f;
                bool served = true;
                for (;;) {
                    f = (uint32_t)lane < chunks ? __hip_atomic_load(hw + lane, __ATOMIC_RELAXED, __HIP_MEMORY_SCOPE_AGENT) : 0x80000000u;
                    if (__builtin_amdgcn_ballot_w64((f & 0x80000000u) == 0) == 0) break;
                    if (__builtin_amdgcn_s_memrealtime() - t_in >= p.wait_ticks) { served = false; break; }
                    __builtin_amdgcn_s_sleep(2);
                }
                f &= 0x7fffffffu;
                if (!served) {
                    const uint16_t* __restrict__ s0 = (const uint16_t*)p.src[2] + (int64_t)bh * p.rows[2] * (int64_t)(8 * cpr);
                    const uint32_t total = p.rows[2] * cpr;
                    f = 0;
                    for (uint32_t i = (uint32_t)lane; i < total; i += 64) {
                        const u32x4_q x = *(const u32x4_q*)(s0 + (int64_t)i * 8);
                        float a = 0.0f;
#pragma unroll
                        for (int j = 0; j < 8; ++j) a = fmaxf(a, fabsf(q16_elem<BF16>(x, j)));
                        const unsigned b = __float_as_uint(a) >> 16;
                        f = b > f ? b : f;
                    }
                }
#pragma unroll
                for (int off = 32; off > 0; off >>= 1) {
                    const unsigned o = (unsigned)__shfl_xor((int)f, off, 64);
                    f = o > f ? o : f;
                }
                if (lane == 0) slab_amax = f;
            }
            __syncthreads();
            vexp = vimage_exponent(slab_amax);
            if (wave == 0) {
                unsigned d = 0;
                if (lane == 0) d = __hip_atomic_fetch_add(hw + VSC_HDR_DEPART, 1u, __ATOMIC_RELAXED, __HIP_MEMORY_SCOPE_AGENT);
                d = (unsigned)__builtin_amdgcn_readfirstlane((int)d);
                if (d == chunks - 1) {
                    if ((uint32_t)lane < chunks) __hip_atomic_store(hw + lane, 0u, __ATOMIC_RELAXED, __HIP_MEMORY_SCOPE_AGENT);
                    if (lane == 0) {
                        hw[VSC_HDR_SCALE] = (unsigned)(127 + vexp) << 23;
                        __hip_atomic_store(hw + VSC_HDR_DEPART, 0u, __ATOMIC_RELAXED, __HIP_MEMORY_SCOPE_AGENT);
                    }
                }
            }
        } else {
            vexp = vimage_exponent(hw[VSC_HDR_AMAX]);
        }
    }
    const float sc = amax > 0.0f ? amax / p.qmax : 1.0f;
    if (lane == 0) p.scale[t][bh * p.nblk[t] + blk] = sc;
    const float rcp0 = __builtin_amdgcn_rcpf(sc);
    const float rcp1 = __builtin_fmaf(__builtin_fmaf(-sc, rcp0, 1.0f), rcp0, rcp0);
    const bool fast_div = __builtin_amdgcn_readfirstlane((int)(sc >= 0x1p-60f && sc <= 0x1p60f)) != 0;
    int8_t* const d8 = (t == 0 ? p.q8 : p.k8) + base;
    _Float16* const d16 = p.v16 + base;
    if (t == 2) {
        const float scv = sc * exp2i(-vexp);
        if (fast_div) quantize_wave_convert<CPL, BF16, true, true>(xr, lane, nchunks, sc, rcp1, p.qlo, p.qhi, d8, d16, scv);
        else quantize_wave_convert<CPL, BF16, false, true>(xr, lane, nchunks, sc, rcp1, p.qlo, p.qhi, d8, d16, scv);
    } else {
        if (fast_div) quantize_wave_convert<CPL, BF16, true, false>(xr, lane, nchunks, sc, rcp1, p.qlo, p.qhi, d8, d16, sc);
        else quantize_wave_convert<CPL, BF16, false, false>(xr, lane, nchunks, sc, rcp1, p.qlo, p.qhi, d8, d16, sc);
    }
}

__global__ __launch_bounds__(256) void tensor_scale_kernel(float* s0, uint32_t n0, float* s1, uint32_t n1, float* s2,
                                                           uint32_t n2, float qmax) {
    __shared__ float red[4];
    float* s = blockIdx.x == 0 ? s0 : blockIdx.x == 1 ? s1 : s2;
    const uint32_t n = blockIdx.x == 0 ? n0 : blockIdx.x == 1 ? n1 : n2;
    float amax = 0.0f;
    for (uint32_t i = threadIdx.x; i < n; i += 256) amax = fmaxf(amax, s[i]);
#pragma unroll
    for (int off = 32; off > 0; off >>= 1) amax = fmaxf(amax, __shfl_xor(amax, off, 64));
    if ((threadIdx.x & 63) == 0) red[threadIdx.x >> 6] = amax;
    __syncthreads();
    amax = fmaxf(fmaxf(red[0], red[1]), fmaxf(red[2], red[3]));
    const float sc = amax > 0.0f ? amax / qmax : 1.0f;
    __syncthreads();
    for (uint32_t i = threadIdx.x; i < n; i += 256) s[i] = sc;
}

template <int MODE>
__global__ __launch_bounds__(256) void quantize_wide_kernel(QuantParams p) {
    __shared__ float red[4];
    uint32_t id = blockIdx.x;
    int t = p.t_first;
    while (t < p.t_end - 1 && id >= p.BH * p.nblk[t]) { id -= p.BH * p.nblk[t]; ++t; }
    const uint32_t bh = id / p.nblk[t], blk = id % p.nblk[t];
    const uint32_t row0 = blk * QBLK;
    const uint32_t nrows = min((uint32_t)QBLK, p.rows[t] - row0);
    const int64_t base = ((int64_t)bh * p.rows[t] + row0) * p.D;
    const uint32_t n = nrows * p.D;
    float sc;
    if (MODE != 1) {
        float amax = 0.0f;
        for (uint32_t i = threadIdx.x; i < n; i += 256) amax = fmaxf(amax, fabsf(load_as_float(p.src[t], base + i, p.in_prec)));
#pragma unroll
        for (int off = 32; off > 0; off >>= 1) amax = fmaxf(amax, __shfl_xor(amax, off, 64));
        if ((threadIdx.x & 63) == 0) red[threadIdx.x >> 6] = amax;
        __syncthreads();
        amax = fmaxf(fmaxf(red[0], red[1]), fmaxf(red[2], red[3]));
        if (MODE == 0) {
            if (threadIdx.x == 0) p.scale[t][bh * p.nblk[t] + blk] = amax;
            return;
        }
        sc = amax > 0.0f ? amax / p.qmax : 1.0f;
        if (threadIdx.x == 0) p.scale[t][bh * p.nblk[t] + blk] = sc;
    } else {
        sc = p.scale[t][bh * p.nblk[t] + blk];
    }
    float* const dst = p.f32[t] + base;
    for (uint32_t i = threadIdx.x; i < n; i += 256) {
        const float y = load_as_float(p.src[t], base + i, p.in_prec) / sc;
        const int qv = max(min((int)(y + __builtin_copysignf(0x1.fffffep-2f, y)), p.qhi), p.qlo);
        dst[i] = (float)qv * sc;
    }
}

template <int DP> __device__ __forceinline__ constexpr int k8_off(int row, int ch) {
    int sw = DP >= 256 ? (ch ^ (row & 15)) : DP == 128 ? (ch ^ ((row >> 1) & 7)) : (ch ^ ((row >> 2) & 3));
    return row * DP + 16 * sw;
}
template <int DP> __device__ __forceinline__ constexpr int v16_off(int row, int ch) {
    int sw = DP >= 128 ? (ch ^ ((row & 3) << 2)) : (ch ^ (((row >> 1) & 1) << 2));
    return row * (2 * DP) + 16 * sw;
}

struct I8FwdParams {
    const int8_t* q8;
    const int8_t* k8;
    const _Float16* v16;
    const float* q_scale;
    const float* k_scale;
    float* o;
    float* lse;
    const void* mask;
    int mask_kind;
    int64_t ms[4];
    uint32_t mf_bs, mf_hs;
    const uint8_t* mask_flags;
    uint32_t mf_nrb, mf_ntiles;
    uint32_t B, H, Sq, Skv, D;
    uint32_t nqblk, nkblk;
    float scale;
    const float* vsc;
};

template <int DP, bool CAUSAL, bool HAS_MASK, int BN>
__global__ __launch_bounds__(256, (DP > 128 ? 1 : (BN == 32 ? 3 : 2))) void fa_fwd_i8_kernel(I8FwdParams p) {
    constexpr int BM = 128;
    constexpr int NKB = BN / 32, NST = BN / 16;
    constexpr int NKS = DP / 32;
    constexpr int NDB = DP / 32;
    constexpr int KT_BYTES = BN * DP;
    constexpr int VT_BYTES = BN * DP * 2;
    constexpr int KCH = DP / 16, VCH = DP / 8;
    constexpr int NPK = KT_BYTES / 1024, NPV = VT_BYTES / 1024;

    extern __shared__ __attribute__((aligned(16))) char smem[];
    char* const Kbuf = smem;
    char* const Vbuf = smem + 2 * KT_BYTES;

    const int tid = threadIdx.x, wave = tid >> 6, lane = tid & 63, ql = lane & 31, hi = lane >> 5;
    const uint32_t nqb = (p.Sq + BM - 1) / BM;
    const uint32_t vid = xcd_remap(blockIdx.x, nqb * p.B * p.H);
    uint32_t bh = vid / nqb;
    uint32_t qb = vid % nqb;
    if (CAUSAL) {
        qb = nqb - 1 - qb;
        if ((nqb & 1) == 0 && DP <= 128 && (uint64_t)nqb * nqb * p.B * p.H <= 32768) {
            const uint32_t pi = vid >> 1, h2 = nqb >> 1, j = pi % h2;
            bh = pi / h2;
            qb = (((vid & 1) ^ (vid >> 5)) & 1) ? j : nqb - 1 - j;
        }
    }
    const uint32_t q_row = qb * BM + wave * 32 + ql;
    const uint32_t wave_q0 = qb * BM + wave * 32;
    const int D = (int)p.D;

    const int8_t* __restrict__ qp = p.q8 + (int64_t)bh * p.Sq * DP;
    const int8_t* kp = p.k8 + (int64_t)bh * p.Skv * DP;
    const _Float16* vp = p.v16 + (int64_t)bh * p.Skv * DP;

    i32x4 qf[NKS];
#pragma unroll
    for (int ks = 0; ks < NKS; ++ks) {
        if (q_row < p.Sq) qf[ks] = *(const i32x4*)(qp + (int64_t)q_row * DP + 32 * ks + 16 * hi);
        else qf[ks] = i32x4{0, 0, 0, 0};
    }
    const uint32_t wq_blk = wave_q0 / QBLK;
    const float sq = (wave_q0 < p.Sq ? p.q_scale[bh * p.nqblk + wq_blk] : 0.0f) * p.scale * UMFA_LOG2E;

    const int uw = __builtin_amdgcn_readfirstlane(wave);
    auto make_srd = [&](const void* base, uint32_t bytes) {
        const unsigned long long a = (unsigned long long)base;
        i32x4 d;
        d[0] = __builtin_amdgcn_readfirstlane((int)(a & 0xffffffffu));
        d[1] = __builtin_amdgcn_readfirstlane((int)((a >> 32) & 0xffffu));
        d[2] = __builtin_amdgcn_readfirstlane((int)bytes);
        d[3] = 0x00020000;
        return d;
    };
    const i32x4 k_srd = make_srd(kp, p.Skv * (uint32_t)DP);
    const i32x4 v_srd = make_srd(vp, p.Skv * (uint32_t)DP * 2);
    const unsigned lds0 = __builtin_amdgcn_readfirstlane((unsigned)(size_t)((LDS_AS char*)smem));
    constexpr int KRPI = 1024 / DP, VRPI = 1024 / (2 * DP);
    const int k_r = lane / KCH, k_c = lane % KCH, v_r = lane / VCH, v_c = lane % VCH;
#pragma unroll
    for (int i = 0; i < (2 * KT_BYTES + 2 * VT_BYTES) / 4096; ++i) *(i32x4*)(smem + i * 4096 + tid * 16) = i32x4{0, 0, 0, 0};
    __syncthreads();
    auto stage_load = [&](uint32_t t) {
        const int buf = t & 1;
#pragma unroll
        for (int n0 = 0; n0 < NPK; n0 += 4) {
            const int n = n0 + uw;
            if (n < NPK) {
                const int row = n * KRPI + k_r;
                const int voff = (int)(t * BN + row) * DP + (k8_off<DP>(row, k_c) - row * DP);
                asm volatile("s_mov_b32 m0, %0\n\ts_nop 0\n\tbuffer_load_dwordx4 %1, %2, 0 offen lds"
                             ::"s"(lds0 + buf * KT_BYTES + n * 1024), "v"(voff), "s"(k_srd) : "memory");
            }
        }
#pragma unroll
        for (int n0 = 0; n0 < NPV; n0 += 4) {
            const int n = n0 + uw;
            if (n < NPV) {
                const int row = n * VRPI + v_r;
                const int voff = (int)(t * BN + row) * (2 * DP) + (v16_off<DP>(row, v_c) - row * (2 * DP));
                asm volatile("s_mov_b32 m0, %0\n\ts_nop 0\n\tbuffer_load_dwordx4 %1, %2, 0 offen lds"
                             ::"s"(lds0 + 2 * KT_BYTES + buf * VT_BYTES + n * 1024), "v"(voff), "s"(v_srd) : "memory");
            }
        }
    };
    auto stage_write = [&](int) { asm volatile("s_waitcnt vmcnt(0)" ::: "memory"); __builtin_amdgcn_s_waitcnt(0x0F70); };

    uint32_t ntiles = (p.Skv + BN - 1) / BN;
    if (CAUSAL) {
        const uint32_t lim = (qb * BM + BM + BN - 1) / BN;
        ntiles = ntiles < lim ? ntiles : lim;
    }
    f32x16 acc[NDB];
#pragma unroll
    for (int i = 0; i < NDB; ++i)
#pragma unroll
        for (int r = 0; r < 16; ++r) acc[i][r] = 0.0f;
    float m = -INFINITY, l = 0.0f;
    const int tr_qq = (lane >> 2) & 3, tr_pp = lane & 3, tr_g1 = (lane >> 4) & 1;
    const int64_t mrow = HAS_MASK ? (int64_t)(bh / p.H) * p.ms[0] + (int64_t)(bh % p.H) * p.ms[1] + (int64_t)q_row * p.ms[2] : 0;
    const bool mvec = HAS_MASK && p.mask_kind == MK_F32 && p.ms[3] == 1 && (p.Skv & 3u) == 0 && ((uintptr_t)p.mask & 15) == 0 &&
                      ((p.ms[0] | p.ms[1] | p.ms[2]) & 3) == 0;
    const uint8_t* mf_row = nullptr;
    int mf_reg = 0;
    if (HAS_MASK && p.mask_flags && BN == 64 && wave_q0 / 32 < p.mf_nrb)
        mf_row = p.mask_flags + (((uint64_t)(bh / p.H) * p.mf_bs + (uint64_t)(bh % p.H) * p.mf_hs) * p.mf_nrb + wave_q0 / 32) * p.mf_ntiles;

    stage_load(0);
    stage_write(0);
    __syncthreads();

    for (uint32_t t = 0; t < ntiles; ++t) {
        const int cur = t & 1;
        const bool more = t + 1 < ntiles;
        if (more) stage_load(t + 1);
        const char* Kt = Kbuf + cur * KT_BYTES;
        const char* Vt = Vbuf + cur * VT_BYTES;
        const uint32_t key_base = t * BN;
        bool active = !CAUSAL || key_base <= wave_q0 + 31;
        int mflag = 0;
        if (HAS_MASK && mf_row) {
            if (t == 0 || (t & 63) == 0) {
                const uint32_t t64 = t & ~63u;
                mf_reg = t64 + lane < p.mf_ntiles ? (int)mf_row[t64 + lane] : 0;
            }
            mflag = __builtin_amdgcn_readlane(mf_reg, (int)(t & 63));
            active = active && mflag != 1;
        }
        if (active) {
            const float ct = sq * p.k_scale[bh * p.nkblk + key_base / QBLK];
            i32x16 s[NKB];
#pragma unroll
            for (int kb = 0; kb < NKB; ++kb) {
#pragma unroll
                for (int r = 0; r < 16; ++r) s[kb][r] = 0;
#pragma unroll
                for (int ks = 0; ks < NKS; ++ks) {
                    const i32x4 a = *(const i32x4*)(Kt + k8_off<DP>(32 * kb + ql, 2 * ks + hi));
                    s[kb] = __builtin_amdgcn_mfma_i32_32x32x32_i8(a, qf[ks], s[kb], 0, 0, 0);
                }
            }
            const bool edge = (key_base + BN > p.Skv) || (CAUSAL && key_base + BN - 1 > wave_q0);
            float m_use, m_new;
            float rs = 0.0f;
            f16x8 pf[NST];
            if (HAS_MASK && mflag != 2) {
                float tv[NKB][16];
                float mx = -INFINITY;
                if (mvec) {
#pragma unroll
                    for (int kb = 0; kb < NKB; ++kb)
#pragma unroll
                        for (int g = 0; g < 4; ++g) {
                            const uint32_t key0 = key_base + 32 * kb + 8 * g + 4 * hi;
                            f32x4 w = {0.0f, 0.0f, 0.0f, 0.0f};
                            if (mflag != 2 && key0 < p.Skv && q_row < p.Sq) w = __builtin_nontemporal_load((const f32x4*)((const float*)p.mask + mrow + key0));
#pragma unroll
                            for (int e = 0; e < 4; ++e) {
                                const int r = 4 * g + e;
                                float x = __builtin_fmaf(w[e], UMFA_LOG2E, (float)s[kb][r] * ct);
                                if (edge && (key0 + e >= p.Skv || (CAUSAL && key0 + e > q_row))) x = -INFINITY;
                                tv[kb][r] = x;
                                mx = fmaxf(mx, x);
                            }
                        }
                } else {
#pragma unroll
                for (int kb = 0; kb < NKB; ++kb)
#pragma unroll
                    for (int r = 0; r < 16; ++r) {
                        const uint32_t key = key_base + 32 * kb + acc_row(r, hi);
                        float x = (float)s[kb][r] * ct;
                        if (mflag != 2 && key < p.Skv && q_row < p.Sq) x += mask_term(p.mask, mrow + (int64_t)key * p.ms[3], p.mask_kind);
                        if (edge && (key >= p.Skv || (CAUSAL && key > q_row))) x = -INFINITY;
                        tv[kb][r] = x;
                        mx = fmaxf(mx, x);
                    }
                }
                mx = fmaxf(mx, xor32(mx));
                m_new = fmaxf(m, mx);
                m_use = m_new == -INFINITY ? 0.0f : m_new;
#pragma unroll
                for (int kb = 0; kb < NKB; ++kb)
#pragma unroll
                    for (int r = 0; r < 16; ++r) {
                        const float e = __builtin_amdgcn_exp2f(tv[kb][r] - m_use);
                        rs += e;
                        pf[2 * kb + (r >> 3)][r & 7] = (_Float16)e;
                    }
            } else {
                if (edge) {
#pragma unroll
                    for (int kb = 0; kb < NKB; ++kb)
#pragma unroll
                        for (int r = 0; r < 16; ++r) {
                            const uint32_t key = key_base + 32 * kb + acc_row(r, hi);
                            if (key >= p.Skv || (CAUSAL && key > q_row)) s[kb][r] = INT_MIN / 2;
                        }
                }
                int mxi = s[0][0];
#pragma unroll
                for (int kb = 0; kb < NKB; ++kb)
#pragma unroll
                    for (int r = 0; r < 16; ++r) mxi = max(mxi, s[kb][r]);
                float mx = (float)mxi * ct;
                mx = fmaxf(mx, xor32(mx));
                m_new = fmaxf(m, mx);
                m_use = m_new;
#pragma unroll
                for (int kb = 0; kb < NKB; ++kb)
#pragma unroll
                    for (int r = 0; r < 16; ++r) {
                        const float e = __builtin_amdgcn_exp2f(__builtin_fmaf((float)s[kb][r], ct, -m_use));
                        rs += e;
                        pf[2 * kb + (r >> 3)][r & 7] = (_Float16)e;
                    }
            }
            if (!__all(m_new == m)) {
                const float alpha = __builtin_amdgcn_exp2f(m - m_use);
                l *= alpha;
#pragma unroll
                for (int i = 0; i < NDB; ++i)
#pragma unroll
                    for (int r = 0; r < 16; ++r) acc[i][r] *= alpha;
                m = m_new;
            }
            l += rs;
#pragma unroll
            for (int i = 0; i < NDB; ++i)
#pragma unroll
                for (int st = 0; st < NST; ++st) {
                    const int row0 = 16 * st + 4 * hi + tr_qq;
                    const int ch = 4 * i + 2 * tr_g1 + (tr_pp >> 1);
                    const s16x4 lo = __builtin_amdgcn_ds_read_tr16_b64_v4i16((s16x4 LDS_AS*)(Vt + v16_off<DP>(row0, ch) + 8 * (tr_pp & 1)));
                    const s16x4 hi4 = __builtin_amdgcn_ds_read_tr16_b64_v4i16((s16x4 LDS_AS*)(Vt + v16_off<DP>(row0 + 8, ch) + 8 * (tr_pp & 1)));
                    const f16x8 a = __builtin_shufflevector(__builtin_bit_cast(f16x4_t, lo), __builtin_bit_cast(f16x4_t, hi4), 0, 1, 2, 3, 4, 5, 6, 7);
                    acc[i] = __builtin_amdgcn_mfma_f32_32x32x16_f16(a, pf[st], acc[i], 0, 0, 0);
                }
        }
        if (more) stage_write(cur ^ 1);
        __syncthreads();
    }

    const float lt = l + xor32(l);
    const float inv = lt > 0.0f ? (1.0f / lt) * (p.vsc ? p.vsc[VSC_HDR_WORDS * (size_t)bh + VSC_HDR_SCALE] : 1.0f) : 0.0f;
    if (q_row < p.Sq) {
        float* __restrict__ op = p.o + ((int64_t)bh * p.Sq + q_row) * D;
#pragma unroll
        for (int i = 0; i < NDB; ++i)
#pragma unroll
            for (int g = 0; g < 4; ++g) {
                const int d0 = 32 * i + 8 * g + 4 * hi;
                if (d0 < D) {
                    f32x4 val = {acc[i][4 * g] * inv, acc[i][4 * g + 1] * inv, acc[i][4 * g + 2] * inv, acc[i][4 * g + 3] * inv};
                    *(f32x4*)(op + d0) = val;
                }
            }
        if (p.lse && hi == 0) p.lse[(int64_t)bh * p.Sq + q_row] = lt > 0.0f ? (m + log2f(lt)) * UMFA_LN2 : -INFINITY;
    }
}

template <int PREC>
__global__ __launch_bounds__(256) void vimage_amax_kernel(const void* __restrict__ src, int64_t slab8, uint32_t chunks, uint32_t* __restrict__ hdr) {
    __shared__ unsigned wmax[4];
    const uint32_t bh = blockIdx.x / chunks, chunk = blockIdx.x - bh * chunks;
    constexpr int U = 8;
    unsigned amax = 0;
#pragma unroll
    for (int u = 0; u < U; ++u) {
        const int64_t i = ((int64_t)chunk * U + u) * 256 + threadIdx.x;
        if (i < slab8) {
            float a = 0.0f;
            if constexpr (PREC == P_FP32) {
                const f32x4 lo = ((const f32x4*)src)[2 * ((int64_t)bh * slab8 + i)], hi = ((const f32x4*)src)[2 * ((int64_t)bh * slab8 + i) + 1];
#pragma unroll
                for (int j = 0; j < 4; ++j) a = fmaxf(a, fmaxf(fabsf(lo[j]), fabsf(hi[j])));
            } else {
                const u32x4_q x = ((const u32x4_q*)src)[(int64_t)bh * slab8 + i];
#pragma unroll
                for (int j = 0; j < 8; ++j) a = fmaxf(a, fabsf(PREC == P_BF16 ? q16_elem<true>(x, j) : q16_elem<false>(x, j)));
            }
            const unsigned b = __float_as_uint(a) >> 16;
            amax = b > amax ? b : amax;
        }
    }
#pragma unroll
    for (int off = 32; off > 0; off >>= 1) {
        const unsigned o = (unsigned)__shfl_xor((int)amax, off, 64);
        amax = o > amax ? o : amax;
    }
    if ((threadIdx.x & 63) == 0) wmax[threadIdx.x >> 6] = amax;
    __syncthreads();
    if (threadIdx.x == 0) {
        for (int w = 1; w < 4; ++w) amax = wmax[w] > amax ? wmax[w] : amax;
        if (amax) (void)__hip_atomic_fetch_max(hdr + VSC_HDR_WORDS * (size_t)bh + VSC_HDR_AMAX, amax, __ATOMIC_RELAXED, __HIP_MEMORY_SCOPE_AGENT);
    }
}
__global__ __launch_bounds__(256) void vimage_finish_kernel(uint32_t* __restrict__ hdr, uint32_t slabs) {
    const uint32_t s = blockIdx.x * 256 + threadIdx.x;
    if (s >= slabs) return;
    uint32_t* const hw = hdr + VSC_HDR_WORDS * (size_t)s;
    hw[VSC_HDR_SCALE] = (unsigned)(127 + vimage_exponent(hw[VSC_HDR_AMAX])) << 23;
    hw[VSC_HDR_AMAX] = 0;
}

static inline size_t align256(size_t x) { return (x + 255) & ~(size_t)255; }
static inline uint32_t dp_of(uint32_t D) { return D <= 64 ? 64 : D <= 128 ? 128 : 256; }

struct WsLayout {
    size_t q8, k8, v16, sq, sk, sv, f32q, f32k, f32v, mflags, total;
};
static WsLayout ws_layout(uint32_t B, uint32_t H, uint32_t Sq, uint32_t Skv, uint32_t D, bool want_f32) {
    const size_t BH = (size_t)B * H, DP = dp_of(D);
    const size_t nqb = (Sq + QBLK - 1) / QBLK, nkb = (Skv + QBLK - 1) / QBLK;
    WsLayout w;
    size_t off = 0;
    if (D > 256) {
        w.q8 = w.k8 = w.v16 = 0;
        w.sq = off; off = align256(off + BH * nqb * 4);
        w.sk = off; off = align256(off + BH * nkb * 4);
        w.sv = off; off = align256(off + BH * nkb * 4);
        w.f32q = off; off = align256(off + BH * Sq * D * 4);
        w.f32k = off; off = align256(off + BH * Skv * D * 4);
        w.f32v = off; off = align256(off + BH * Skv * D * 4);
        w.mflags = off;
        w.total = off;
        return w;
    }
    w.q8 = off; off = align256(off + BH * Sq * DP);
    w.k8 = off; off = align256(off + BH * Skv * DP);
    w.v16 = off; off = align256(off + BH * Skv * DP * 2);
    w.sq = off; off = align256(off + BH * nqb * 4);
    w.sk = off; off = align256(off + BH * nkb * 4);
    w.sv = off; off = align256(off + BH * nkb * 4);
    off = align256(off + BH * nkb * 4);
    w.f32q = w.f32k = w.f32v = 0;
    if (want_f32) {
        w.f32q = off; off = align256(off + BH * Sq * D * 4);
        w.f32k = off; off = align256(off + BH * Skv * D * 4);
        w.f32v = off; off = align256(off + BH * Skv * D * 4);
    }
    w.mflags = off; off = align256(off + BH * ((Sq + 31) / 32) * ((Skv + 63) / 64));
    w.total = off;
    return w;
}

size_t quant_workspace_bytes(uint32_t B, uint32_t H, uint32_t Sq, uint32_t Skv, uint32_t D, bool want_f32) {
    return ws_layout(B, H, Sq, Skv, D, want_f32).total;
}

bool quantized_supported(uint32_t D) { return D >= 8 && D % 8 == 0 && D <= 1024; }

static hipError_t launch_quantize_wide(const void* q, const void* k, const void* v, int in_prec, uint32_t B, uint32_t H, uint32_t Sq, uint32_t Skv,
                                       uint32_t D, int bits, int quant_mode, void* workspace, QuantViews* views, hipStream_t stream) {
    const WsLayout w = ws_layout(B, H, Sq, Skv, D, true);
    char* ws = (char*)workspace;
    QuantParams qp;
    memset(&qp, 0, sizeof(qp));
    qp.src[0] = q; qp.src[1] = k; qp.src[2] = v;
    qp.scale[0] = (float*)(ws + w.sq); qp.scale[1] = (float*)(ws + w.sk); qp.scale[2] = (float*)(ws + w.sv);
    qp.f32[0] = (float*)(ws + w.f32q); qp.f32[1] = (float*)(ws + w.f32k); qp.f32[2] = (float*)(ws + w.f32v);
    qp.rows[0] = Sq; qp.rows[1] = Skv; qp.rows[2] = Skv;
    for (int t = 0; t < 3; ++t) qp.nblk[t] = (qp.rows[t] + QBLK - 1) / QBLK;
    qp.BH = B * H; qp.D = D; qp.DPQ = D;
    qp.in_prec = in_prec;
    qp.qmax = bits == 4 ? 7.0f : 127.0f;
    qp.qlo = bits == 4 ? -8 : -128;
    qp.qhi = bits == 4 ? 7 : 127;
    qp.t_first = 0; qp.t_end = 3;
    const uint32_t grid = qp.BH * (qp.nblk[0] + qp.nblk[1] + qp.nblk[2]);
    if (quant_mode == 2 || quant_mode == 3) {
        hipLaunchKernelGGL(quantize_wide_kernel<2>, dim3(grid), dim3(256), 0, stream, qp);
    } else {
        hipLaunchKernelGGL(quantize_wide_kernel<0>, dim3(grid), dim3(256), 0, stream, qp);
        hipLaunchKernelGGL(tensor_scale_kernel, dim3(3), dim3(256), 0, stream, qp.scale[0], qp.BH * qp.nblk[0], qp.scale[1], qp.BH * qp.nblk[1],
                           qp.scale[2], qp.BH * qp.nblk[2], qp.qmax);
        hipLaunchKernelGGL(quantize_wide_kernel<1>, dim3(grid), dim3(256), 0, stream, qp);
    }
    if (views) {
        memset(views, 0, sizeof(*views));
        views->q_scale = qp.scale[0]; views->k_scale = qp.scale[1]; views->v_scale = qp.scale[2];
        views->qf = qp.f32[0]; views->kf = qp.f32[1]; views->vf = qp.f32[2];
        views->nqblk = qp.nblk[0]; views->nkblk = qp.nblk[1]; views->dpq = D;
    }
    return hipGetLastError();
}

hipError_t launch_quantize(const void* q, const void* k, const void* v, int in_prec, uint32_t B, uint32_t H,
                           uint32_t Sq, uint32_t Skv, uint32_t D, int bits, int quant_mode, void* workspace,
                           int copies, QuantViews* views, hipStream_t stream, uint32_t* overflow, uint32_t* vhdr, const uint32_t* famax) {
    if (D > 256) {
        if (copies == 2) return hipErrorInvalidValue;
        return launch_quantize_wide(q, k, v, in_prec, B, H, Sq, Skv, D, bits, quant_mode, workspace, views, stream);
    }
    const bool want_f32 = copies != 0;
    const WsLayout w = ws_layout(B, H, Sq, Skv, D, want_f32);
    char* ws = (char*)workspace;
    QuantParams qp;
    memset(&qp, 0, sizeof(qp));
    qp.src[0] = q; qp.src[1] = k; qp.src[2] = v;
    qp.q8 = (int8_t*)(ws + w.q8);
    qp.k8 = (int8_t*)(ws + w.k8);
    qp.v16 = (_Float16*)(ws + w.v16);
    qp.scale[0] = (float*)(ws + w.sq);
    qp.scale[1] = (float*)(ws + w.sk);
    qp.scale[2] = (float*)(ws + w.sv);
    if (copies == 1) {
        qp.f32[0] = (float*)(ws + w.f32q);
        qp.f32[1] = (float*)(ws + w.f32k);
        qp.f32[2] = (float*)(ws + w.f32v);
    } else if (copies == 2) {
        qp.f16[0] = (_Float16*)(ws + w.f32q);
        qp.f16[1] = (_Float16*)(ws + w.f32k);
        qp.f16[2] = (_Float16*)(ws + w.f32v);
        qp.overflow = overflow;
        qp.famax = famax;
    }
    qp.rows[0] = Sq; qp.rows[1] = Skv; qp.rows[2] = Skv;
    for (int t = 0; t < 3; ++t) qp.nblk[t] = (qp.rows[t] + QBLK - 1) / QBLK;
    qp.BH = B * H; qp.D = D; qp.DPQ = dp_of(D);
    qp.in_prec = in_prec;
    qp.qmax = bits == 4 ? 7.0f : 127.0f;
    qp.qlo = bits == 4 ? -8 : -128;
    qp.qhi = bits == 4 ? 7 : 127;
    const uint32_t grid = qp.BH * (qp.nblk[0] + qp.nblk[1] + qp.nblk[2]);
    const bool f8v = quant_mode == 3 && D == 128 && bits == 8 && !want_f32;
    if (f8v) {
        qp.v8 = (uint8_t*)(ws + w.v16);
        qp.v_e8 = (uint32_t*)(ws + w.sv + (size_t)align256(qp.BH * qp.nblk[2] * 4));
    }
    if (quant_mode == 3) quant_mode = 2;
    const bool in16 = in_prec != P_FP32;
    qp.t_first = 0; qp.t_end = 3;
    const bool wave_form = quant_mode == 2 && in16 && !want_f32 && !f8v && (D == 128 || D == 64) && !tuning().quant_block_wg.load(std::memory_order_relaxed) &&
                           ((uintptr_t)q & 15) == 0 && ((uintptr_t)k & 15) == 0 && ((uintptr_t)v & 15) == 0;
    bool v_prepass = false;
    if (vhdr && !f8v) {
        qp.vhdr = vhdr;
        qp.wait_ticks = (uint32_t)std::min<int64_t>(std::max(tuning().cast_wait_us.load(std::memory_order_relaxed), 0), 1000000) * 100u;
        qp.v_exchange = wave_form && qp.nblk[2] % 4 == 0 && qp.nblk[2] / 4 <= 64 && ((uint64_t)qp.BH * (qp.nblk[0] + qp.nblk[1])) % 4 == 0 &&
                        !tuning().cast_two_pass.load(std::memory_order_relaxed);
        if (!qp.v_exchange) {
            v_prepass = true;
            const int64_t slab8 = (int64_t)Skv * D / 8;
            const uint32_t chunks = (uint32_t)((slab8 + 8 * 256 - 1) / (8 * 256));
            const dim3 g(qp.BH * chunks);
            if (in_prec == P_FP32) hipLaunchKernelGGL(vimage_amax_kernel<P_FP32>, g, dim3(256), 0, stream, v, slab8, chunks, vhdr);
            else if (in_prec == P_BF16) hipLaunchKernelGGL(vimage_amax_kernel<P_BF16>, g, dim3(256), 0, stream, v, slab8, chunks, vhdr);
            else hipLaunchKernelGGL(vimage_amax_kernel<P_FP16>, g, dim3(256), 0, stream, v, slab8, chunks, vhdr);
        }
    }
    if (wave_form) {
        QuantParams qw = qp;
        uint32_t nb = 0;
        for (int t = 0; t < qw.t_end; ++t) nb += qp.BH * qp.nblk[t];
        const dim3 gw((nb + 3) / 4);
        if (D == 128 && in_prec == P_BF16) hipLaunchKernelGGL((quantize_wave_kernel<16, true>), gw, dim3(256), 0, stream, qw);
        else if (D == 128) hipLaunchKernelGGL((quantize_wave_kernel<16, false>), gw, dim3(256), 0, stream, qw);
        else if (in_prec == P_BF16) hipLaunchKernelGGL((quantize_wave_kernel<8, true>), gw, dim3(256), 0, stream, qw);
        else hipLaunchKernelGGL((quantize_wave_kernel<8, false>), gw, dim3(256), 0, stream, qw);
    } else if (quant_mode == 2) {
        if (in16) hipLaunchKernelGGL((quantize_kernel<2, true>), dim3(grid), dim3(256), 0, stream, qp);
        else hipLaunchKernelGGL((quantize_kernel<2, false>), dim3(grid), dim3(256), 0, stream, qp);
    } else {
        if (in16) hipLaunchKernelGGL((quantize_kernel<0, true>), dim3(grid), dim3(256), 0, stream, qp);
        else hipLaunchKernelGGL((quantize_kernel<0, false>), dim3(grid), dim3(256), 0, stream, qp);
        hipLaunchKernelGGL(tensor_scale_kernel, dim3(3), dim3(256), 0, stream, qp.scale[0], qp.BH * qp.nblk[0],
                           qp.scale[1], qp.BH * qp.nblk[1], qp.scale[2], qp.BH * qp.nblk[2], qp.qmax);
        if (in16) hipLaunchKernelGGL((quantize_kernel<1, true>), dim3(grid), dim3(256), 0, stream, qp);
        else hipLaunchKernelGGL((quantize_kernel<1, false>), dim3(grid), dim3(256), 0, stream, qp);
    }
    if (v_prepass) hipLaunchKernelGGL(vimage_finish_kernel, dim3((qp.BH + 255) / 256), dim3(256), 0, stream, vhdr, qp.BH);
    if (views) {
        views->q8 = qp.q8; views->k8 = qp.k8; views->v16 = qp.v16;
        views->v8 = qp.v8; views->v_e8 = qp.v_e8;
        views->q_scale = qp.scale[0]; views->k_scale = qp.scale[1]; views->v_scale = qp.scale[2];
        views->qf = qp.f32[0]; views->kf = qp.f32[1]; views->vf = qp.f32[2];
        views->qh = qp.f16[0]; views->kh = qp.f16[1]; views->vh = qp.f16[2];
        views->nqblk = qp.nblk[0]; views->nkblk = qp.nblk[1]; views->dpq = qp.DPQ;
    }
    return hipGetLastError();
}

template <int DP, bool CAUSAL, bool HAS_MASK>
static hipError_t launch_i8_one(const I8FwdParams& p, hipStream_t stream) {
    constexpr int BN = 64;
    const uint32_t nqb = (p.Sq + 127) / 128;
    const size_t lds = 2 * BN * DP + 2 * BN * DP * 2;
    auto kfn = fa_fwd_i8_kernel<DP, CAUSAL, HAS_MASK, BN>;
    if (hipError_t e = ensure_dynamic_lds((const void*)kfn, lds); e != hipSuccess) return e;
    hipLaunchKernelGGL(kfn, dim3(nqb * p.B * p.H), dim3(256), lds, stream, p);
    return hipGetLastError();
}

template <int DP>
static hipError_t launch_i8_flags(const I8FwdParams& p, bool causal, hipStream_t stream) {
    const bool mk = p.mask != nullptr;
    if (causal) return mk ? launch_i8_one<DP, true, true>(p, stream) : launch_i8_one<DP, true, false>(p, stream);
    return mk ? launch_i8_one<DP, false, true>(p, stream) : launch_i8_one<DP, false, false>(p, stream);
}

hipError_t launch_quantized_fwd(const FwdParams& fp, int bits, int quant_mode, void* workspace, hipStream_t stream,
                                const char** name) {
    if (!quantized_supported(fp.D)) return hipErrorInvalidValue;
    if (fp.D > 256) {
        QuantViews v;
        if (hipError_t e = launch_quantize_wide(fp.q, fp.k, fp.v, fp.in_prec, fp.B, fp.H, fp.Sq, fp.Skv, fp.D, bits, quant_mode, workspace, &v, stream); e != hipSuccess) return e;
        FwdParams pw = fp;
        pw.q = v.qf; pw.k = v.kf; pw.v = v.vf;
        pw.in_prec = P_FP32; pw.out_prec = P_FP32;
        const int64_t D = fp.D;
        pw.qs[0] = (int64_t)fp.H * fp.Sq * D; pw.qs[1] = (int64_t)fp.Sq * D; pw.qs[2] = D; pw.qs[3] = 1;
        pw.ks[0] = pw.vs[0] = (int64_t)fp.H * fp.Skv * D; pw.ks[1] = pw.vs[1] = (int64_t)fp.Skv * D; pw.ks[2] = pw.vs[2] = D; pw.ks[3] = pw.vs[3] = 1;
        pw.os[0] = D; pw.os[1] = 1;
        pw.part_buf = nullptr; pw.part_cnt = nullptr; pw.vsc = nullptr; pw.pv16 = 0;
        if (fp.mask && fp.mask_kind == MK_NONE) {
            pw.mask_kind = MK_F32;
            pw.ms[0] = (int64_t)fp.H * fp.Sq * fp.Skv; pw.ms[1] = (int64_t)fp.Sq * fp.Skv; pw.ms[2] = fp.Skv; pw.ms[3] = 1;
        }
        const char* nm = "none";
        const hipError_t e = launch_fwd_wide(pw, stream, &nm);
        if (name) *name = bits == 4 ? "fa_fwd_wide<i4 images>" : "fa_fwd_wide<i8 images>";
        return e;
    }
    if (quant_mode == 3 && !(bits == 8 && fp.part_buf && fp.part_cnt && fwd_w64_i8_supported(fp) && !fp.mask)) quant_mode = 2;
    QuantViews v;
    hipError_t e = launch_quantize(fp.q, fp.k, fp.v, fp.in_prec, fp.B, fp.H, fp.Sq, fp.Skv, fp.D, bits, quant_mode,
                                   workspace, 0, &v, stream, nullptr, (uint32_t*)fp.vsc);
    if (e != hipSuccess) return e;
    I8FwdParams p;
    memset(&p, 0, sizeof(p));
    p.q8 = v.q8; p.k8 = v.k8; p.v16 = (const _Float16*)v.v16;
    p.q_scale = v.q_scale; p.k_scale = v.k_scale;
    p.vsc = v.v8 ? nullptr : fp.vsc;
    p.o = (float*)fp.o; p.lse = fp.lse;
    p.mask = fp.mask;
    const bool w64 = fp.part_buf && fp.part_cnt && fwd_w64_i8_supported(fp);
    if (fp.mask && !w64) {
        FwdParams mp = fp;
        if (fp.mask_kind == MK_NONE) {
            mp.mask_kind = MK_F32;
            mp.ms[0] = (int64_t)fp.H * fp.Sq * fp.Skv; mp.ms[1] = (int64_t)fp.Sq * fp.Skv; mp.ms[2] = fp.Skv; mp.ms[3] = 1;
        }
        if (mp.mask_kind == MK_WINDOW) return hipErrorInvalidValue;
        p.mask_kind = mp.mask_kind;
        for (int i = 0; i < 4; ++i) p.ms[i] = mp.ms[i];
        if (!tuning().no_mask_flags.load(std::memory_order_relaxed)) {
            uint8_t* fl = (uint8_t*)workspace + ws_layout(fp.B, fp.H, fp.Sq, fp.Skv, fp.D, false).mflags;
            if (launch_mask_flags(mp, fl, stream) == hipSuccess && mp.mask_flags) {
                p.mask_flags = mp.mask_flags; p.mf_nrb = mp.mf_nrb; p.mf_ntiles = mp.mf_ntiles;
                p.mf_bs = mp.mf_bs; p.mf_hs = mp.mf_hs;
            }
        }
    }
    p.B = fp.B; p.H = fp.H; p.Sq = fp.Sq; p.Skv = fp.Skv; p.D = fp.D;
    p.nqblk = v.nqblk; p.nkblk = v.nkblk;
    p.scale = fp.scale;
    const uint32_t dp = dp_of(fp.D);
    if (w64) {
        *name = v.v8 ? "fa_fwd_w64_i8f8<128>" : fp.mask ? (bits == 4 ? "fa_fwd_w64_i4<128,mask>" : "fa_fwd_w64_i8<128,mask>") : bits == 4 ? "fa_fwd_w64_i4<128>" : "fa_fwd_w64_i8<128>";
        return launch_fwd_w64_i8(fp, v, fp.part_buf, fp.part_cnt, stream);
    }
    if (dp == 64) { *name = bits == 4 ? "fa_fwd_i4<64>" : "fa_fwd_i8<64>"; return launch_i8_flags<64>(p, fp.causal, stream); }
    if (dp == 128) { *name = bits == 4 ? "fa_fwd_i4<128>" : "fa_fwd_i8<128>"; return launch_i8_flags<128>(p, fp.causal, stream); }
    *name = bits == 4 ? "fa_fwd_i4<256>" : "fa_fwd_i8<256>";
    return launch_i8_flags<256>(p, fp.causal, stream);
}

}
```

universal-metal-flash-attention_amd/csrc/kernels.h:

```cpp
#pragma once
#include <hip/hip_runtime.h>

#include <atomic>

#include "fa_common.h"

namespace umfa {

enum SoftmaxRef : int {
    SM_DEFAULT = 0,
    SM_EXACT = 1,
    SM_DEFERRED = 2,
    SM_LAZY = 3,
};
struct Tuning {
    std::atomic<int> sm_mode{SM_DEFAULT};
    std::atomic<float> sm_tau{6.0f};
    std::atomic<int> force_w64{0}, no_w64{0}, w64_grid{0}, w64_skew{0}, no_mask_flags{0}, bwd_exact{0}, bwd_dq{0}, bwd_persist{0},
        bwd_separate_delta{0}, no_split{0}, force_split{0}, no_dma{0}, bn64{0}, pv_fp16{0}, bwd_ds_store{0}, no_w64_mask{0}, ksplit{0}, no_pipe{0}, no_w64_mask_lazy{0}, no_w64_bias{0}, no_w64_f32_mask{0} ,
        no_mask_realign{0} ,
        no_w64_ragged_mask{0} ,
        mask_pass_ratio{0} ,
        f32_mask_ratio{0} ,
        cast_two_pass{0} , bwd_ds_lab{0} ,
        cast_u{0} ,
        quant_block_wg{0} ,
        cast_wait_us{100} ,
        decode_ks{0} ,
        cbal{0} ,
        cbal_delta{-1} ,
        sync_chunks{1} ,
        sync_chunked_calls{0} ,
        mirror_cache_hits{0} ,
        no_bwd_mask{0} ,
        sdpa_dropout{0} ;
};
Tuning& tuning();
bool set_tuning(const char* name, const char* value);
bool get_tuning(const char* name, char* out, size_t n);
int device_cu_count();
hipError_t ensure_dynamic_lds(const void* kernel, size_t bytes);

hipError_t launch_fwd_exact(const FwdParams& p, hipStream_t stream, const char** name);

hipError_t launch_fwd_wide(const FwdParams& p, hipStream_t stream, const char** name);
hipError_t launch_bwd_wide(const BwdParams& p, hipStream_t stream, const char** name);

hipError_t launch_fwd_16(const FwdParams& p, hipStream_t stream, const char** name);
bool fwd_16_supported(const FwdParams& p);
struct FwdSplitPlan {
    uint32_t n_full, nsplit;
    size_t buf_bytes, cnt_bytes;
    uint32_t decode = 0;
    uint32_t cbal = 0, cbal_delta = 0;
};
FwdSplitPlan fwd_16_split_plan(const FwdParams& p);

struct FwdW64Plan {
    size_t buf_bytes, cnt_bytes;
};
bool fwd_w64_supported(const FwdParams& p);
uint32_t fwd_w64_grid(const FwdParams& p);
double fwd_w64_predict_us(const FwdParams& p);
double fwd_16_predict_us(const FwdParams& p);
FwdW64Plan fwd_w64_plan(const FwdParams& p);
hipError_t launch_fwd_w64(const FwdParams& p, float* part_buf, uint32_t* part_cnt, hipStream_t stream, const char** name);

hipError_t launch_bwd(const BwdParams& p, hipStream_t stream, const char** name);
bool bwd_16_supported(const BwdParams& p);
hipError_t launch_bwd_16(const BwdParams& p, hipStream_t stream, const char** name);
bool bwd_16_mask_supported(const BwdParams& p);
hipError_t launch_bwd_16_masked(const BwdParams& p, hipStream_t stream, const char** name);

struct DropFwdParams : FwdParams {
    const int64_t* rng;
    uint32_t thresh;
    float dscale;
};
struct DropBwdParams : BwdParams {
    const int64_t* rng;
    uint32_t thresh;
    float dscale;
};
bool fwd_16_dropout_supported(const FwdParams& p);
hipError_t launch_fwd_16_dropout(const DropFwdParams& p, hipStream_t stream, const char** name);
bool bwd_16_dropout_supported(const BwdParams& p);
hipError_t launch_bwd_16_dropout(const DropBwdParams& p, hipStream_t stream, const char** name);
hipError_t launch_dropout_keep_mask(uint8_t* keep, uint32_t B, uint32_t H, uint32_t Sq, uint32_t Skv, const int64_t* rng, uint32_t thresh,
                                    hipStream_t stream);

struct RopeParams {
    const void* src;
    void* dst;
    const float* cos_table;
    const float* sin_table;
    int64_t src_batch_stride, src_head_stride, src_seq_stride;
    int64_t table_batch_stride;
    uint32_t B, H, S, D;
    int negate_sin;
};
hipError_t launch_rope(const RopeParams& p, int prec, hipStream_t stream);
hipError_t launch_hadamard(void* data, uint32_t block_size, uint32_t num_blocks, int prec, hipStream_t stream);

struct DequantParams {
    const void* src;
    float* dst;
    void* dst16;
    uint32_t* overflow;
    const float* block_scales;
    const int32_t* block_zero_points;
    uint32_t B, H_src, H_dst, S, D, block_size;
    float scale;
    int zero_point;
    int prec;
    int transposed;
    uint32_t* amax_word;
    const uint32_t* unit_amax;
};
hipError_t launch_dequant(const DequantParams& p, hipStream_t stream);
constexpr uint32_t VSC_HDR_WORDS = 128, VSC_HDR_DEPART = 64, VSC_HDR_SCALE = 65, VSC_HDR_AMAX = 66;
hipError_t launch_cast_rows_bf16_to_f16(const void* src, const int64_t* strides, void* dst, uint32_t B, uint32_t H, uint32_t S, uint32_t D,
                                        uint32_t* hdr, hipStream_t stream);
hipError_t launch_bwd16_rowc(const float* lse, const float* dvec, float* rowc, int64_t n, const float* d_mul , hipStream_t stream);
hipError_t launch_cast_f16_unit(const void* src, int prec, void* dst, int64_t n, uint32_t* hdr, hipStream_t stream, bool amax_done = false );
hipError_t launch_amax_dense(const void* src, int prec, int64_t n, uint32_t* word, hipStream_t stream);
hipError_t launch_amax_dense_n(int count , const void* const* src, int prec, const int64_t* n, uint32_t* const* word, hipStream_t stream);
hipError_t launch_bwd_units(uint32_t* hdr, hipStream_t stream, uint32_t* clean_flag = nullptr);
hipError_t launch_group_sum(const float* src, void* dst, uint32_t B, uint32_t H, uint32_t Hkv, int64_t slab, hipStream_t stream,
                            int out_prec = P_FP32);

struct QuantViews {
    const int8_t* q8;
    const int8_t* k8;
    const void* v16;
    const uint8_t* v8;
    const uint32_t* v_e8;
    const float* q_scale;
    const float* k_scale;
    const float* v_scale;
    const float* qf;
    const float* kf;
    const float* vf;
    const void* qh;
    const void* kh;
    const void* vh;
    uint32_t nqblk, nkblk, dpq;
};
bool quantized_supported(uint32_t D);
size_t quant_workspace_bytes(uint32_t B, uint32_t H, uint32_t Sq, uint32_t Skv, uint32_t D, bool want_f32);
hipError_t launch_quantize(const void* q, const void* k, const void* v, int in_prec, uint32_t B, uint32_t H,
                           uint32_t Sq, uint32_t Skv, uint32_t D, int bits, int quant_mode, void* workspace,
                           int copies, QuantViews* views, hipStream_t stream, uint32_t* overflow = nullptr,
                           uint32_t* vhdr = nullptr ,
                           const uint32_t* famax = nullptr );
hipError_t launch_quantized_fwd(const FwdParams& fp, int bits, int quant_mode, void* workspace, hipStream_t stream,
                                const char** name);
bool fwd_w64_i8_supported(const FwdParams& p);
hipError_t launch_fwd_w64_i8(const FwdParams& p, const QuantViews& v, float* part_buf, uint32_t* part_cnt, hipStream_t stream);

size_t mask_pack_bytes(const FwdParams& p);
hipError_t launch_mask_pack(FwdParams& p, void* scratch, hipStream_t stream);
struct CastRowsCall {
    const void* src;
    int64_t strides[4];
    void* dst;
    uint32_t B, H, S, D;
    uint32_t* hdr;
};
hipError_t launch_mask_classify(FwdParams& p, void* scratch, hipStream_t stream, const CastRowsCall* cast = nullptr);
bool mask_needs_copy(const FwdParams& p);
size_t mask_copy_bytes(const FwdParams& p);
hipError_t launch_cast_rows_and_mask_pack(const void* src, const int64_t* strides, void* dst, uint32_t B, uint32_t H, uint32_t S, uint32_t D,
                                          uint32_t* hdr, FwdParams& p, void* mask_scratch, hipStream_t stream);
size_t mask_flags_bytes(const FwdParams& p);
void mask_flags_describe(FwdParams& p, const uint8_t* flags);
bool mask_flags_worthwhile(const FwdParams& p);
bool mask_rows_scalar(const FwdParams& p);
size_t mask_realign_bytes(const FwdParams& p);
hipError_t launch_mask_realign(FwdParams& p, void* dst, hipStream_t stream);
hipError_t launch_mask_flags(FwdParams& p, uint8_t* flags, hipStream_t stream);

}
```

universal-metal-flash-attention_amd/csrc/tuning.hip:

```cpp
#include <cstdio>
#include <cstdlib>
#include <cstring>
#include <mutex>
#include <vector>

#include "kernels.h"

namespace umfa {

namespace {
int env_int(const char* name, int dflt) {
    const char* e = getenv(name);
    return (e && *e) ? atoi(e) : dflt;
}
bool env_flag(const char* name) {
    const char* e = getenv(name);
    return e && e[0] == '1';
}
}

Tuning& tuning() {
    static Tuning* t = [] {
        Tuning* x = new Tuning();
        const char* tau = getenv("UMFA_W64_TAU");
        const char* lazy = getenv("UMFA_W64_LAZY");
        if (tau && *tau) {
            const float v = (float)atof(tau);
            if (v >= 0.0f && v <= 16.0f) {
                x->sm_tau.store(v);
                x->sm_mode.store(v == 0.0f ? SM_EXACT : SM_DEFERRED);
            }
        }
        if (lazy && *lazy) x->sm_mode.store(lazy[0] != '0' ? SM_LAZY : (x->sm_mode.load() == SM_DEFAULT ? SM_DEFERRED : x->sm_mode.load()));
        x->force_w64.store(env_flag("UMFA_FORCE_W64"));
        x->no_w64.store(env_flag("UMFA_NO_W64"));
        x->w64_grid.store(env_int("UMFA_W64_GRID", 0));
        x->w64_skew.store(env_int("UMFA_W64_SKEW", 0));
        x->no_mask_flags.store(getenv("UMFA_NO_MASK_FLAGS") != nullptr);
        x->bwd_exact.store(getenv("UMFA_BWD_EXACT") != nullptr);
        x->bwd_dq.store(env_int("UMFA_BWD_DQ", 0));
        x->bwd_persist.store(getenv("UMFA_BWD_PERSIST") != nullptr);
        x->bwd_separate_delta.store(getenv("UMFA_LAB_SEPARATE_DELTA") != nullptr);
        x->no_split.store(env_flag("UMFA_NO_SPLIT"));
        x->force_split.store(env_int("UMFA_FORCE_SPLIT", 0));
        x->no_dma.store(env_flag("UMFA_NO_DMA"));
        x->bn64.store(env_flag("UMFA_BN64"));
        x->pv_fp16.store(env_int("UMFA_PV_FP16", 1) != 0);
        x->bwd_ds_store.store(env_flag("UMFA_BWD_DS_STORE"));
        x->no_w64_mask.store(env_flag("UMFA_NO_W64_MASK"));
        x->ksplit.store(env_flag("UMFA_KSPLIT"));
        x->no_pipe.store(env_flag("UMFA_NO_PIPE"));
        x->no_w64_mask_lazy.store(env_flag("UMFA_NO_W64_MASK_LAZY"));
        x->no_w64_bias.store(env_flag("UMFA_NO_W64_BIAS"));
        x->no_w64_f32_mask.store(env_flag("UMFA_NO_W64_F32_MASK"));
        x->cast_two_pass.store(env_flag("UMFA_CAST_TWO_PASS"));
        x->cast_u.store(env_int("UMFA_CAST_U", 0));
        x->quant_block_wg.store(env_flag("UMFA_QUANT_BLOCK_WG"));
        x->cast_wait_us.store(env_int("UMFA_CAST_WAIT_US", 100));
        x->bwd_ds_lab.store(env_int("UMFA_LAB_DS", 0));
        x->cbal.store(env_int("UMFA_CBAL", 0));
        x->decode_ks.store(env_int("UMFA_DECODE_KS", 0));
        x->cbal_delta.store(env_int("UMFA_CBAL_DELTA", -1));
        x->sync_chunks.store(env_int("UMFA_SYNC_CHUNKS", 1));
        x->sdpa_dropout.store(env_flag("UMFA_SDPA_DROPOUT"));
        return x;
    }();
    return *t;
}

bool set_tuning(const char* name, const char* value) {
    if (!name || !value) return false;
    Tuning& t = tuning();
    const int iv = atoi(value);
    const bool on = value[0] != '\0' && value[0] != '0';
    if (!strcmp(name, "softmax_reference")) {
        const int m = !strcmp(value, "default") ? SM_DEFAULT : !strcmp(value, "exact") ? SM_EXACT
                      : !strcmp(value, "deferred") ? SM_DEFERRED : !strcmp(value, "lazy") ? SM_LAZY : -1;
        if (m < 0) return false;
        t.sm_mode.store(m);
        return true;
    }
    if (!strcmp(name, "softmax_tau") || !strcmp(name, "w64_tau")) {
        const float v = (float)atof(value);
        if (!(v >= 0.0f && v <= 16.0f)) return false;
        t.sm_tau.store(v);
        if (!strcmp(name, "w64_tau")) t.sm_mode.store(v == 0.0f ? SM_EXACT : SM_DEFERRED);
        return true;
    }
    struct { const char* n; std::atomic<int>* v; bool flag; } tab[] = {
        {"force_w64", &t.force_w64, true}, {"no_w64", &t.no_w64, true}, {"w64_grid", &t.w64_grid, false}, {"w64_skew", &t.w64_skew, false},
        {"no_mask_flags", &t.no_mask_flags, true}, {"bwd_exact", &t.bwd_exact, true}, {"bwd_dq", &t.bwd_dq, false},
        {"bwd_persist", &t.bwd_persist, true}, {"bwd_separate_delta", &t.bwd_separate_delta, true},
        {"no_split", &t.no_split, true}, {"force_split", &t.force_split, false}, {"no_dma", &t.no_dma, true},
        {"bn64", &t.bn64, true}, {"pv_fp16", &t.pv_fp16, true}, {"bwd_ds_store", &t.bwd_ds_store, true}, {"no_w64_mask", &t.no_w64_mask, true}, {"ksplit", &t.ksplit, true}, {"no_pipe", &t.no_pipe, true}, {"no_w64_mask_lazy", &t.no_w64_mask_lazy, true}, {"no_w64_bias", &t.no_w64_bias, true}, {"no_w64_f32_mask", &t.no_w64_f32_mask, true}, {"f32_mask_ratio", &t.f32_mask_ratio, false}, {"mask_pass_ratio", &t.mask_pass_ratio, false}, {"no_w64_ragged_mask", &t.no_w64_ragged_mask, true}, {"no_mask_realign", &t.no_mask_realign, true}, {"no_bwd_mask", &t.no_bwd_mask, true}, {"sdpa_dropout", &t.sdpa_dropout, true},
        {"cast_two_pass", &t.cast_two_pass, true}, {"bwd_ds_lab", &t.bwd_ds_lab, false}, {"cast_u", &t.cast_u, false}, {"quant_block_wg", &t.quant_block_wg, true},
        {"cast_wait_us", &t.cast_wait_us, false}, {"cbal", &t.cbal, false}, {"cbal_delta", &t.cbal_delta, false}, {"decode_ks", &t.decode_ks, false}, {"sync_chunks", &t.sync_chunks, false}, {"sync_chunked_calls", &t.sync_chunked_calls, false}, {"mirror_cache_hits", &t.mirror_cache_hits, false},
    };
    for (auto& e : tab)
        if (!strcmp(name, e.n)) {
            e.v->store(e.flag ? (on ? 1 : 0) : iv);
            return true;
        }
    return false;
}

bool get_tuning(const char* name, char* out, size_t n) {
    if (!name || !out || n < 2) return false;
    Tuning& t = tuning();
    char buf[32];
    if (!strcmp(name, "softmax_reference")) {
        const int m = t.sm_mode.load();
        snprintf(buf, sizeof(buf), "%s", m == SM_EXACT ? "exact" : m == SM_DEFERRED ? "deferred" : m == SM_LAZY ? "lazy" : "default");
    } else if (!strcmp(name, "softmax_tau") || !strcmp(name, "w64_tau")) {
        snprintf(buf, sizeof(buf), "%g", (double)t.sm_tau.load());
    } else {
        struct { const char* n; std::atomic<int>* v; } tab[] = {
            {"force_w64", &t.force_w64}, {"no_w64", &t.no_w64}, {"w64_grid", &t.w64_grid}, {"w64_skew", &t.w64_skew},
            {"no_mask_flags", &t.no_mask_flags}, {"bwd_exact", &t.bwd_exact}, {"bwd_dq", &t.bwd_dq}, {"bwd_persist", &t.bwd_persist},
            {"bwd_separate_delta", &t.bwd_separate_delta}, {"no_split", &t.no_split}, {"force_split", &t.force_split},
            {"no_dma", &t.no_dma}, {"bn64", &t.bn64}, {"pv_fp16", &t.pv_fp16}, {"bwd_ds_store", &t.bwd_ds_store}, {"no_w64_mask", &t.no_w64_mask}, {"ksplit", &t.ksplit}, {"no_pipe", &t.no_pipe}, {"no_w64_mask_lazy", &t.no_w64_mask_lazy}, {"no_w64_bias", &t.no_w64_bias}, {"no_w64_f32_mask", &t.no_w64_f32_mask}, {"f32_mask_ratio", &t.f32_mask_ratio}, {"mask_pass_ratio", &t.mask_pass_ratio}, {"no_w64_ragged_mask", &t.no_w64_ragged_mask}, {"no_mask_realign", &t.no_mask_realign}, {"no_bwd_mask", &t.no_bwd_mask}, {"sdpa_dropout", &t.sdpa_dropout},
            {"cast_two_pass", &t.cast_two_pass}, {"bwd_ds_lab", &t.bwd_ds_lab}, {"cast_u", &t.cast_u}, {"quant_block_wg", &t.quant_block_wg},
            {"cast_wait_us", &t.cast_wait_us}, {"cbal", &t.cbal}, {"cbal_delta", &t.cbal_delta}, {"decode_ks", &t.decode_ks}, {"sync_chunks", &t.sync_chunks}, {"sync_chunked_calls", &t.sync_chunked_calls}, {"mirror_cache_hits", &t.mirror_cache_hits},
        };
        const std::atomic<int>* v = nullptr;
        for (auto& e : tab)
            if (!strcmp(name, e.n)) v = e.v;
        if (!v) return false;
        snprintf(buf, sizeof(buf), "%d", v->load());
    }
    if (strlen(buf) + 1 > n) return false;
    strcpy(out, buf);
    return true;
}

int device_cu_count() {
    static std::atomic<int> cus[64];
    int dev = 0;
    if (hipGetDevice(&dev) != hipSuccess || dev < 0 || dev >= 64) dev = 0;
    int n = cus[dev].load(std::memory_order_relaxed);
    if (n <= 0) {
        if (hipDeviceGetAttribute(&n, hipDeviceAttributeMultiprocessorCount, dev) != hipSuccess || n <= 0) n = 256;
        cus[dev].store(n, std::memory_order_relaxed);
    }
    return n;
}

hipError_t ensure_dynamic_lds(const void* kernel, size_t bytes) {
    if (bytes <= 48 * 1024) return hipSuccess;
    struct Entry { const void* k; int dev; size_t bytes; };
    static std::mutex mu;
    static std::vector<Entry> done;
    int dev = 0;
    if (hipGetDevice(&dev) != hipSuccess) dev = 0;
    std::lock_guard<std::mutex> lock(mu);
    for (const Entry& e : done)
        if (e.k == kernel && e.dev == dev && e.bytes >= bytes) return hipSuccess;
    hipError_t e = hipFuncSetAttribute(kernel, hipFuncAttributeMaxDynamicSharedMemorySize, (int)bytes);
    if (e != hipSuccess) return e;
    done.push_back({kernel, dev, bytes});
    return hipSuccess;
}

}
```

universal-metal-flash-attention_amd/umfa_torch/ops.py:

```python
from __future__ import annotations

import ctypes
from typing import Optional, Tuple

import torch

from umfa._ffi import (MFA_MASK_SCALAR_BF16, MFA_MASK_SCALAR_BYTE, MFA_MASK_SCALAR_FP16, MFA_MASK_SCALAR_FP32,
                       MFA_MASK_TYPE_ADDITIVE, MFA_MASK_TYPE_BOOL, MFA_MASK_TYPE_NONE, MFA_PRECISION_BF16,
                       MFA_PRECISION_FP16, MFA_PRECISION_FP32, MFAError, _check_error, _lib, mfa_context_t)

_PREC = {torch.float16: MFA_PRECISION_FP16, torch.bfloat16: MFA_PRECISION_BF16, torch.float32: MFA_PRECISION_FP32}
_PREC_NAME = {torch.float16: b"fp16", torch.bfloat16: b"bf16", torch.float32: b"fp32"}

_ctx = None


def context():
    global _ctx
    if _ctx is None:
        if not torch.cuda.is_available():
            raise RuntimeError("umfa_torch needs a ROCm device: there is no CPU fallback")
        h = mfa_context_t()
        _check_error(_lib.mfa_create_context(ctypes.byref(h)))
        _ctx = h
    return _ctx


def last_kernel() -> str:
    return _lib.umfa_last_kernel_name(context()).decode()


def release_scratch(stream=None, all_streams: bool = False) -> None:
    st = torch.cuda.current_stream().cuda_stream if stream is None else stream.cuda_stream
    _check_error(_lib.umfa_release_scratch(context(), ctypes.c_void_p(st), 1 if all_streams else 0))


_OPTION_NAMES = ("softmax_reference", "softmax_tau", "w64_tau", "force_w64", "no_w64", "w64_grid", "w64_skew", "no_mask_flags", "bwd_exact",
                 "bwd_dq", "bwd_persist", "bwd_separate_delta", "no_split", "force_split", "no_dma", "bn64", "pv_fp16", "bwd_ds_store", "no_w64_mask", "ksplit", "no_pipe", "no_w64_mask_lazy", "no_w64_bias", "no_w64_f32_mask", "f32_mask_ratio", "mask_pass_ratio", "no_w64_ragged_mask", "no_mask_realign",
                 "cast_two_pass", "bwd_ds_lab", "cast_u", "quant_block_wg", "cast_wait_us", "cbal", "cbal_delta", "decode_ks", "sync_chunks", "sync_chunked_calls", "mirror_cache_hits", "no_bwd_mask", "sdpa_dropout")


def get_option(name: str) -> str:
    buf = ctypes.create_string_buffer(64)
    _check_error(_lib.umfa_get_option(context(), name.encode(), buf, 64))
    return buf.value.decode()


def pv_fp16_status() -> int:
    return int(get_option("pv_fp16_status"))


def set_option(name: str, value) -> None:
    _check_error(_lib.umfa_set_option(context(), name.encode(), str(value).encode()))


class options:

    def __init__(self, **kw):
        unknown = [k for k in kw if k not in _OPTION_NAMES]
        if unknown:
            raise KeyError(f"unknown launcher switch(es) {unknown}; known: {_OPTION_NAMES}")
        self.kw = kw
        self.prev = {}

    def __enter__(self):
        prev = {k: get_option(k) for k in self.kw}
        if "w64_tau" in self.kw or "softmax_tau" in self.kw:
            prev.setdefault("softmax_reference", get_option("softmax_reference"))
        for k, v in self.kw.items():
            set_option(k, v)
        self.prev = prev
        return self

    def __exit__(self, *exc):
        ref = self.prev.pop("softmax_reference", None)
        for k, v in self.prev.items():
            set_option("softmax_tau" if k == "w64_tau" else k, v)
        if ref is not None:
            set_option("softmax_reference", ref)
        return False


def _i64(vals):
    return (ctypes.c_int64 * len(vals))(*[int(v) for v in vals])


def _mask_args(mask: Optional[torch.Tensor]):
    if mask is None:
        return None, None, None, 0, MFA_MASK_TYPE_NONE, MFA_MASK_SCALAR_BYTE
    if mask.dtype == torch.bool:
        mt, ms = MFA_MASK_TYPE_BOOL, MFA_MASK_SCALAR_BYTE
    elif mask.dtype == torch.float32:
        mt, ms = MFA_MASK_TYPE_ADDITIVE, MFA_MASK_SCALAR_FP32
    elif mask.dtype == torch.float16:
        mt, ms = MFA_MASK_TYPE_ADDITIVE, MFA_MASK_SCALAR_FP16
    elif mask.dtype == torch.bfloat16:
        mt, ms = MFA_MASK_TYPE_ADDITIVE, MFA_MASK_SCALAR_BF16
    else:
        raise TypeError(f"unsupported mask dtype {mask.dtype}")
    if mask.dim() > 4:
        raise ValueError("attention masks of more than 4 dims are not supported")
    return (ctypes.c_void_p(mask.data_ptr()), _i64(mask.shape), _i64(mask.stride()), mask.dim(), mt, ms)


def _quant_mode(name: str) -> int:
    n = name.lower()
    return 3 if "fp8" in n else 2 if n.startswith("block") else 0


def attention_forward(q: torch.Tensor, k: torch.Tensor, v: torch.Tensor, *, scale: Optional[float] = None,
                      causal: bool = False, mask: Optional[torch.Tensor] = None, out_dtype=None,
                      return_lse: bool = False, intermediate_dtype=None, out: Optional[torch.Tensor] = None,
                      window=None):
    assert q.is_cuda and k.is_cuda and v.is_cuda, "device tensors required"
    B, H, Sq, D = q.shape
    Skv = k.shape[2]
    if scale is None:
        scale = D ** -0.5
    out_dtype = out_dtype or q.dtype
    for t in (q, k, v):
        if t.stride(-1) != 1:
            raise ValueError("last dimension must be contiguous")
    if out is None:
        out = torch.empty((B, H, Sq, D), dtype=out_dtype, device=q.device)
    lse = torch.empty((B * H * Sq,), dtype=torch.float32, device=q.device) if return_lse else None
    if window is not None:
        if mask is not None:
            raise ValueError("window and mask are exclusive")
        mptr, mshape, mstr, mnd, mt, ms = None, _i64((int(window[0]), int(window[1]))), None, 0, 3, MFA_MASK_SCALAR_BYTE
    else:
        mptr, mshape, mstr, mnd, mt, ms = _mask_args(mask)
    inter = _PREC[intermediate_dtype or q.dtype]
    stream = torch.cuda.current_stream(q.device).cuda_stream
    _check_error(_lib.umfa_attention_forward_stream(
        context(), ctypes.c_void_p(stream),
        ctypes.c_void_p(q.data_ptr()), _i64(q.stride()), ctypes.c_void_p(k.data_ptr()), _i64(k.stride()),
        ctypes.c_void_p(v.data_ptr()), _i64(v.stride()), ctypes.c_void_p(out.data_ptr()), _PREC[out.dtype],
        ctypes.c_void_p(lse.data_ptr()) if lse is not None else None,
        mptr, mshape, mstr, mnd, mt, ms, B, Sq, Skv, H, D, float(scale), bool(causal), _PREC[q.dtype], inter))
    return (out, lse) if return_lse else out


def attention_encode(q, k, v, out32, *, scale=None, causal=False, mask=None, stream=None):
    B, H, Sq, D = q.shape
    Skv = k.shape[2]
    if scale is None:
        scale = D ** -0.5
    mptr, mshape, mstr, mnd, mt, ms = _mask_args(mask)
    s = stream if stream is not None else torch.cuda.current_stream(q.device).cuda_stream
    _check_error(_lib.mfa_attention_encode_mtl(
        context(), ctypes.c_void_p(s),
        ctypes.c_void_p(q.data_ptr()), 0, _i64(q.stride()), ctypes.c_void_p(k.data_ptr()), 0, _i64(k.stride()),
        ctypes.c_void_p(v.data_ptr()), 0, _i64(v.stride()), ctypes.c_void_p(out32.data_ptr()), 0,
        mptr, 0, mshape, mstr, mnd, mt, ms, B, Sq, Skv, H, D, float(scale), bool(causal),
        _PREC_NAME[q.dtype], _PREC_NAME[q.dtype]))
    return out32


class _DevBuf:

    def __init__(self, t: Optional[torch.Tensor]):
        from umfa._ffi import mfa_buffer_t
        self.handle = mfa_buffer_t()
        if t is not None:
            _check_error(_lib.mfa_buffer_from_mtl_buffer(context(), ctypes.c_void_p(t.data_ptr()),
                                                         t.numel() * t.element_size(), ctypes.byref(self.handle)))

    def close(self):
        if self.handle:
            _lib.mfa_destroy_buffer(self.handle)
            self.handle = None


def quantized_attention_forward(q, k, v, *, scale=None, causal=False, mask=None, bits: int = 8,
                                quant_mode: str = "blockwise"):
    B, H, Sq, D = q.shape
    Skv = k.shape[2]
    if scale is None:
        scale = D ** -0.5
    q, k, v = q.contiguous(), k.contiguous(), v.contiguous()
    out = torch.empty((B, H, Sq, D), dtype=torch.float32, device=q.device)
    lse = torch.empty((B * H * Sq,), dtype=torch.float32, device=q.device)
    m32 = None
    if mask is not None:
        m32 = torch.zeros((B, H, Sq, Skv), dtype=torch.float32, device=q.device)
        m32 = m32.masked_fill(~mask, float("-inf")) if mask.dtype == torch.bool else m32 + mask.float()
        m32 = m32.contiguous()
    torch.cuda.current_stream(q.device).synchronize()
    bufs = [_DevBuf(t) for t in (q, k, v, out, lse, m32)]
    try:
        _check_error(_lib.mfa_quantized_forward_with_lse(
            context(), *(b.handle for b in bufs), B, Sq, Skv, H, D, float(scale), bool(causal),
            4 if bits == 4 else 3, _quant_mode(quant_mode), _PREC[q.dtype]))
    finally:
        for b in bufs:
            b.close()
    return out, lse


def quantized_attention_forward_stream(q, k, v, *, scale=None, causal=False, mask=None, bits: int = 8,
                                       quant_mode: str = "blockwise", return_lse: bool = False, out=None, lse=None):
    B, H, Sq, D = q.shape
    Skv = k.shape[2]
    if scale is None:
        scale = D ** -0.5
    q, k, v = q.contiguous(), k.contiguous(), v.contiguous()
    if out is None:
        out = torch.empty((B, H, Sq, D), dtype=torch.float32, device=q.device)
    if lse is None:
        lse = torch.empty((B * H * Sq,), dtype=torch.float32, device=q.device)
    assert out.dtype == torch.float32 and out.is_contiguous() and lse.dtype == torch.float32 and lse.numel() == B * H * Sq
    vp = lambda t: ctypes.c_void_p(t.data_ptr()) if t is not None else None
    stream = ctypes.c_void_p(torch.cuda.current_stream(q.device).cuda_stream)
    tail = (B, Sq, Skv, H, D, float(scale), bool(causal), 4 if bits == 4 else 3, _quant_mode(quant_mode), _PREC[q.dtype])
    if mask is not None and hasattr(_lib, "umfa_quantized_forward_masked_stream"):
        mptr, mshape, mstr, mnd, mt, ms = _mask_args(mask)
        _check_error(_lib.umfa_quantized_forward_masked_stream(context(), stream, vp(q), vp(k), vp(v), vp(out), vp(lse), mptr, mshape, mstr, mnd, mt, ms, *tail))
        return (out, lse) if return_lse else out
    m32 = None
    if mask is not None:
        if mask.dtype == torch.float32 and tuple(mask.shape) == (B, H, Sq, Skv) and mask.is_contiguous():
            m32 = mask
        else:
            m32 = torch.zeros((B, H, Sq, Skv), dtype=torch.float32, device=q.device)
            m32 = (m32.masked_fill(~mask, float("-inf")) if mask.dtype == torch.bool else m32 + mask.float()).contiguous()
    _check_error(_lib.umfa_quantized_forward_stream(context(), stream, vp(q), vp(k), vp(v), vp(out), vp(lse), vp(m32), *tail))
    return (out, lse) if return_lse else out


def quantized_attention_backward_stream(dout, q, k, v, o32, lse, *, scale=None, causal=False, bits: int = 8,
                                        quant_mode: str = "blockwise"):
    B, H, Sq, D = q.shape
    Skv = k.shape[2]
    if scale is None:
        scale = D ** -0.5
    for t in (dout, q, k, v, o32, lse):
        assert t.is_cuda and t.is_contiguous()
    assert o32.dtype == torch.float32 and lse.dtype == torch.float32 and dout.dtype == q.dtype
    dq = torch.empty((B, H, Sq, D), dtype=torch.float32, device=q.device)
    dk = torch.empty((B, H, Skv, D), dtype=torch.float32, device=q.device)
    dv = torch.empty_like(dk)
    status = torch.zeros(1, dtype=torch.int32, device=q.device)
    vp = lambda t: ctypes.c_void_p(t.data_ptr())
    _check_error(_lib.umfa_quantized_backward_stream(
        context(), ctypes.c_void_p(torch.cuda.current_stream(q.device).cuda_stream), vp(q), vp(k), vp(v), vp(o32), vp(dout),
        vp(lse), vp(dq), vp(dk), vp(dv), vp(status), B, Sq, Skv, H, D, float(scale), bool(causal), 4 if bits == 4 else 3,
        _quant_mode(quant_mode), _PREC[q.dtype]))
    return dq, dk, dv, status


def attention_backward_gqa(dout, q, k, v, o, lse, *, scale: float, causal: bool = False):
    B, Hq, Sq, D = q.shape
    Hkv, Skv = k.shape[1], k.shape[2]
    for t in (dout, q, k, v, o, lse):
        assert t.is_cuda and t.is_contiguous()
    if q.dtype == torch.float32 or D not in (64, 128, 256) or Hq % Hkv:
        return None
    assert o.dtype in (torch.float32, q.dtype) and lse.dtype == torch.float32 and dout.dtype == q.dtype
    dq = torch.empty_like(q)
    dk, dv = torch.empty_like(k), torch.empty_like(v)
    dvec = torch.empty((B * Hq * Sq,), dtype=torch.float32, device=q.device)
    rc = _lib.umfa_attention_backward_gqa_stream(
        context(), ctypes.c_void_p(torch.cuda.current_stream(q.device).cuda_stream),
        *(ctypes.c_void_p(t.data_ptr()) for t in (dout, q, k, v, o, lse, dq, dk, dv, dvec)),
        B, Sq, Skv, Hq, Hkv, D, float(scale), bool(causal), _PREC[q.dtype], True, o.dtype != torch.float32)
    if rc == 1:
        return None
    _check_error(rc)
    return dq, dk, dv


def gpu_latency() -> float:
    return float(_lib.mfa_get_gpu_latency(context()))


def attention_backward(dout, q, k, v, o32, lse, *, scale: float, causal: bool = False, grads_in_input_type: bool = True,
                       intermediate_dtype=None, keep_fp32: bool = False, mask: Optional[torch.Tensor] = None, window=None):
    B, H, Sq, D = q.shape
    Skv = k.shape[2]
    for t in (dout, q, k, v, o32, lse):
        assert t.is_cuda and t.is_contiguous()
    assert o32.dtype in (torch.float32, q.dtype) and lse.dtype == torch.float32 and dout.dtype == q.dtype
    o_typed = o32.dtype != torch.float32
    inter = _PREC[intermediate_dtype or q.dtype]
    dvec = torch.empty((B * H * Sq,), dtype=torch.float32, device=q.device)
    stream = ctypes.c_void_p(torch.cuda.current_stream(q.device).cuda_stream)

    if window is not None:
        if mask is not None:
            raise ValueError("window and mask are exclusive")
        margs = (None, _i64((int(window[0]), int(window[1]))), None, 0, 3, MFA_MASK_SCALAR_BYTE)
    elif mask is not None:
        margs = _mask_args(mask)
    else:
        margs = None

    def call(gdt, typed):
        dq = torch.empty((B, H, Sq, D), dtype=gdt, device=q.device)
        dk = torch.empty((B, H, Skv, D), dtype=gdt, device=q.device)
        dv = torch.empty_like(dk)
        ptrs = (ctypes.c_void_p(t.data_ptr()) for t in (dout, q, k, v, o32, lse, dq, dk, dv, dvec))
        if margs is None:
            rc = _lib.umfa_attention_backward_stream(context(), stream, *ptrs, B, Sq, Skv, H, D, float(scale), bool(causal),
                                                     _PREC[q.dtype], inter, typed, o_typed)
        else:
            rc = _lib.umfa_attention_backward_masked_stream(context(), stream, *ptrs, B, Sq, Skv, H, D, float(scale), bool(causal),
                                                            _PREC[q.dtype], inter, typed, o_typed, *margs)
        return rc, dq, dk, dv

    if grads_in_input_type and not keep_fp32 and q.dtype != torch.float32:
        rc, dq, dk, dv = call(q.dtype, True)
        if rc == 0:
            return dq, dk, dv
    rc, dq, dk, dv = call(torch.float32, False)
    _check_error(rc)
    if keep_fp32:
        return dq, dk, dv
    return dq.to(q.dtype), dk.to(q.dtype), dv.to(q.dtype)


def attention_forward_dropout(q, k, v, dropout_p: float, rng_state: torch.Tensor, *, scale: float, causal: bool = False, out_dtype=None):
    B, H, Sq, D = q.shape
    Skv = k.shape[2]
    out = torch.empty((B, H, Sq, D), dtype=out_dtype or q.dtype, device=q.device)
    lse = torch.empty((B * H * Sq,), dtype=torch.float32, device=q.device)
    stream = torch.cuda.current_stream(q.device).cuda_stream
    _check_error(_lib.umfa_attention_forward_dropout_stream(
        context(), ctypes.c_void_p(stream), ctypes.c_void_p(q.data_ptr()), _i64(q.stride()), ctypes.c_void_p(k.data_ptr()), _i64(k.stride()),
        ctypes.c_void_p(v.data_ptr()), _i64(v.stride()), ctypes.c_void_p(out.data_ptr()), _PREC[out.dtype], ctypes.c_void_p(lse.data_ptr()),
        B, Sq, Skv, H, D, float(scale), bool(causal), _PREC[q.dtype], _PREC[q.dtype], float(dropout_p), ctypes.c_void_p(rng_state.data_ptr())))
    return out, lse


def attention_backward_dropout(dout, q, k, v, out, lse, dropout_p: float, rng_state: torch.Tensor, *, scale: float, causal: bool = False,
                               grads_in_input_type: bool = True):
    B, H, Sq, D = q.shape
    Skv = k.shape[2]
    for t in (dout, q, k, v, out, lse):
        assert t.is_cuda and t.is_contiguous()
    gdt = q.dtype if grads_in_input_type else torch.float32
    dq = torch.empty((B, H, Sq, D), dtype=gdt, device=q.device)
    dk = torch.empty((B, H, Skv, D), dtype=gdt, device=q.device)
# ... 306 lines not shown
```

Baseline: 1068.

## Fuse Q quantisation into the int8 w64 attention kernel

Adds a path where the int8 forward kernel reads bf16/fp16 Q directly, computes the per-64-row block scale with a wave amax, quantises it in LDS and builds the MFMA Q fragments in place. This removes the separate Q quantisation pass and its int8 Q write and re-read. The quantiser helpers move into a shared header, and a v_first ordering is added to the quantize kernel. In exchange, each kernel segment does extra loads and conversion work before its main loop and uses more registers and LDS traffic, and the scale setup is moved later in the segment.

```diff
diff --git a/universal-metal-flash-attention_amd/csrc/fa_fwd16_w64.hip b/universal-metal-flash-attention_amd/csrc/fa_fwd16_w64.hip
--- a/universal-metal-flash-attention_amd/csrc/fa_fwd16_w64.hip
+++ b/universal-metal-flash-attention_amd/csrc/fa_fwd16_w64.hip
@@ -478,7 +478,7 @@
     return p.mask_kind == MK_NONE && !p.mask;
 }
 
-hipError_t launch_fwd_w64_i8(const FwdParams& p, const QuantViews& v, float* part_buf, uint32_t* part_cnt, hipStream_t stream) {
+hipError_t launch_fwd_w64_i8(const FwdParams& p, const QuantViews& v, float* part_buf, uint32_t* part_cnt, hipStream_t stream, const void* q16, int bits) {
     if (!fwd_w64_i8_supported(p) || !part_buf || !part_cnt || v.dpq != 128) return hipErrorNotSupported;
     W64I8Params wp;
     wp.q8 = v.q8; wp.k8 = v.k8; wp.v16 = (const _Float16*)v.v16;
@@ -494,6 +494,13 @@
     w64_softmax_policy(P_FP16, &wp.tau, &wp.lazy);
     wp.skew = (uint32_t)tuning().w64_skew.load(std::memory_order_relaxed);
     wp.vsc = v.v8 ? nullptr : p.vsc;
+    if (q16 && (p.in_prec == P_FP32 || ((uintptr_t)q16 & 15) != 0 || (uint64_t)p.Sq * 256u >= 0x7fffffffull)) return hipErrorInvalidValue;
+    wp.q16 = q16;
+    wp.q16_hs = (int64_t)p.Sq * 128; wp.q16_rs = 128;
+    wp.q16_bf16 = p.in_prec == P_BF16 ? 1u : 0u;
+    wp.qmax = bits == 4 ? 7.0f : 127.0f;
+    wp.qlo = bits == 4 ? -8 : -128;
+    wp.qhi = bits == 4 ? 7 : 127;
     const uint32_t grid = w64_grid(p);
     const bool f8 = v.v8 != nullptr, maskt = p.mask_kind == MK_BOOL;
     wp.mk_bits = wp.mk_list = wp.mk_cnt = nullptr; wp.mk_bs = wp.mk_hs = wp.mk_nrb64 = 0;
diff --git a/universal-metal-flash-attention_amd/csrc/fa_fwd16_w64_kernel.inc b/universal-metal-flash-attention_amd/csrc/fa_fwd16_w64_kernel.inc
--- a/universal-metal-flash-attention_amd/csrc/fa_fwd16_w64_kernel.inc
+++ b/universal-metal-flash-attention_amd/csrc/fa_fwd16_w64_kernel.inc
@@ -400,7 +400,7 @@
 
     for (uint32_t si = 0; si < nseg; ++si) {
         int tid_s = tid;
-        if constexpr (MASKA) asm volatile("" : "+v"(tid_s));
+        if constexpr (MASKA || W64_I8) asm volatile("" : "+v"(tid_s));
         const int lane = tid_s & 63, ql = lane & 31, hi = lane >> 5;
 #ifdef W64_LAB_STAMPS
         if (si) { asm volatile("s_waitcnt vmcnt(0)" ::: "memory"); W64_STAMP(st_epi); }
@@ -417,6 +417,10 @@
         KF qf[2][KS];
         int kdma[4];
         constexpr bool have_pref = false;
+#endif
+#if W64_I8
+        int lane_q = tid_s & 63;
+        asm volatile("" : "+v"(lane_q));
 #endif
         auto issue_q_k0 = [&](uint32_t item_, uint32_t tfirst_, int k_step_) {
             const uint32_t bh_ = item_ / nqb, qblk_ = item_ % nqb;
@@ -441,6 +445,11 @@
                              ::"s"(lds_wave_k + j * 1024), "v"(kdma[j]), "s"(k_srd_) : "memory");
                 kdma[j] += k_step_;
             }
+#if W64_I8
+            if (p.q16 != nullptr) {
+                return;
+            }
+#endif
 #pragma unroll
             for (int qb = 0; qb < 2; ++qb) {
                 const int qoff = (int)(q0_ + 32 * qb + ql) * q_stride_b + 16 * hi;
@@ -468,7 +477,6 @@
 #endif
         const auto q_rsrc = __builtin_amdgcn_make_buffer_rsrc((void*)qp, 0, (int)(p.Sq * 128u), 0x00020000);
         const i32x4 k_srd = make_srd(kp, p.Skv * 128u);
-        const float sq = (q0 < p.Sq ? p.q_scale[(int64_t)bh * p.nqblk + q0 / 64] : 0.0f) * p.scale * UMFA_LOG2E;
         const float* __restrict__ ksc = p.k_scale + (int64_t)bh * p.nkblk;
         int sc_win = -1;
         float ksc_w = 0.0f;
@@ -491,24 +499,6 @@
             load_scale_window(tile);
             return __builtin_bit_cast(float, __builtin_amdgcn_readlane(__builtin_bit_cast(int, ksc_w), (int)(tile & 63u)));
         };
-#ifndef W64_I8_NOBIAS
-        float kmax = 0.0f;
-        for (uint32_t t = lane; t < p.nkblk; t += 64) kmax = fmaxf(kmax, ksc[t]);
-#pragma unroll
-        for (int off = 32; off > 0; off >>= 1) kmax = fmaxf(kmax, __shfl_xor(kmax, off, 64));
-        const float bias_bound = fmaxf(I8_BIAS * 1.25f * sq * kmax, 0x1p-60f);
-        const int eb = ((__builtin_bit_cast(int, bias_bound) >> 23) & 0xff) - 126;
-        const float mgrid = __builtin_bit_cast(float, (eb - 24 + 127) << 23), inv_mgrid = __builtin_bit_cast(float, (24 - eb + 127) << 23);
-        const float cgrid = __builtin_bit_cast(float, (eb - 46 + 127) << 23), inv_cgrid = __builtin_bit_cast(float, (46 - eb + 127) << 23);
-#define W64_C2(x) (__builtin_rintf((x) * inv_cgrid) * cgrid)
-#define W64_MGRID(x) (__builtin_ceilf((x) * inv_mgrid) * mgrid)
-#if W64_LAZY_PARTS
-        lazy = lazy && eb <= 24;
-#endif
-#else
-#define W64_C2(x) (x)
-#define W64_MGRID(x) (x)
-#endif
 #else
 #define W64_MGRID(x) (x)
         const T* qp = (const T*)p.q + ((int64_t)b * p.qs[0] + (int64_t)h * p.qs[1]);
@@ -694,6 +684,43 @@
         }
 #if W64_PREFETCH_NEXT
         have_pref = false;
+#endif
+#if W64_I8
+        float sq_blk;
+        if (p.q16 != nullptr) {
+#ifndef W64_Q16_HALVES
+#define W64_Q16_HALVES 2
+#endif
+            const unsigned qst = lds0 + 65536u + (unsigned)uw * (32 * (512 + 16));
+            const int rs_b = (int)p.q16_rs * 2;
+            const auto q16_rsrc = __builtin_amdgcn_make_buffer_rsrc((void*)((const uint16_t*)p.q16 + (int64_t)bh * p.q16_hs), 0,
+                                                                   (int)((p.Sq - 1) * (uint32_t)rs_b + 256u), 0x00020000);
+            const int qoff = (int)(q0 + (uint32_t)(lane_q >> 4)) * rs_b + 16 * (lane_q & 15);
+            const float sc_ = p.q16_bf16 ? w64_quantise_q<true, W64_Q16_HALVES>(q16_rsrc, qoff, rs_b, qf, qst, lane_q, p.qmax, p.qlo, p.qhi)
+                                         : w64_quantise_q<false, W64_Q16_HALVES>(q16_rsrc, qoff, rs_b, qf, qst, lane_q, p.qmax, p.qlo, p.qhi);
+            sq_blk = q0 < p.Sq ? sc_ : 0.0f;
+        } else {
+            sq_blk = q0 < p.Sq ? p.q_scale[(int64_t)bh * p.nqblk + q0 / 64] : 0.0f;
+        }
+        const float sq = sq_blk * p.scale * UMFA_LOG2E;
+#ifndef W64_I8_NOBIAS
+        float kmax = 0.0f;
+        for (uint32_t t = lane; t < p.nkblk; t += 64) kmax = fmaxf(kmax, ksc[t]);
+#pragma unroll
+        for (int off = 32; off > 0; off >>= 1) kmax = fmaxf(kmax, __shfl_xor(kmax, off, 64));
+        const float bias_bound = fmaxf(I8_BIAS * 1.25f * sq * kmax, 0x1p-60f);
+        const int eb = ((__builtin_bit_cast(int, bias_bound) >> 23) & 0xff) - 126;
+        const float mgrid = __builtin_bit_cast(float, (eb - 24 + 127) << 23), inv_mgrid = __builtin_bit_cast(float, (24 - eb + 127) << 23);
+        const float cgrid = __builtin_bit_cast(float, (eb - 46 + 127) << 23), inv_cgrid = __builtin_bit_cast(float, (46 - eb + 127) << 23);
+#define W64_C2(x) (__builtin_rintf((x) * inv_cgrid) * cgrid)
+#define W64_MGRID(x) (__builtin_ceilf((x) * inv_mgrid) * mgrid)
+#if W64_LAZY_PARTS
+        lazy = lazy && eb <= 24;
+#endif
+#else
+#define W64_C2(x) (x)
+#define W64_MGRID(x) (x)
+#endif
 #endif
         zero_o();
 #if !W64_F8
diff --git a/universal-metal-flash-attention_amd/csrc/fa_fwd16_w64_params.h b/universal-metal-flash-attention_amd/csrc/fa_fwd16_w64_params.h
--- a/universal-metal-flash-attention_amd/csrc/fa_fwd16_w64_params.h
+++ b/universal-metal-flash-attention_amd/csrc/fa_fwd16_w64_params.h
@@ -3,6 +3,7 @@
 
 #include "fa_common.h"
 #include "fa_fwd_16_kernel.h"
+#include "fa_quant_block.h"
 #include "kernels.h"
 
 namespace umfa {
@@ -66,7 +67,71 @@
     const uint32_t* mk_cnt;
     uint32_t mk_bs, mk_hs, mk_nrb64;
     const float* vsc;
+    const void* q16;
+    int64_t q16_hs;
+    uint32_t q16_rs;
+    uint32_t q16_bf16;
+    float qmax;
+    int32_t qlo, qhi;
 };
+
+template <bool FAST, bool BF16>
+__device__ __forceinline__ void w64_quantise_q_convert(unsigned stg, int lane, float sc, float rcp1, int qlo, int qhi) {
+    typedef __attribute__((address_space(3))) u32x4_q* lds_chunk_p;
+    typedef unsigned u32x2_q __attribute__((ext_vector_type(2)));
+    typedef __attribute__((address_space(3))) u32x2_q* lds_half_p;
+#pragma unroll
+    for (int i = 0; i < 16; ++i) {
+        const int r = 4 * i + (lane >> 4), c = lane & 15;
+        const unsigned a = stg + (unsigned)(r * 256 + ((c ^ (r & 15)) << 4));
+        const u32x4_q x = *(lds_chunk_p)(uintptr_t)a;
+        int q[8];
+        quant_chunk<BF16, FAST>(x, sc, rcp1, qlo, qhi, q);
+        const uint2 w = pack_chunk_i8(q);
+        *(lds_half_p)(uintptr_t)a = u32x2_q{w.x, w.y};
+    }
+}
+template <bool BF16, int NH>
+__device__ __forceinline__ float w64_quantise_q(__amdgpu_buffer_rsrc_t rsrc, int qoff, int rs_b, i32x4 (&qf)[2][4], unsigned stg, int lane, float qmax, int qlo,
+                                                int qhi) {
+    typedef __attribute__((address_space(3))) u32x4_q* lds_chunk_p;
+    typedef unsigned u32x2_q __attribute__((ext_vector_type(2)));
+    typedef __attribute__((address_space(3))) const u32x2_q* lds_half_p;
+    float amax = 0.0f;
+#pragma unroll
+    for (int h = 0; h < NH; ++h) {
+        constexpr int N = 16 / NH;
+        u32x4_q x[N];
+#pragma unroll
+        for (int j = 0; j < N; ++j) x[j] = __builtin_bit_cast(u32x4_q, __builtin_amdgcn_raw_buffer_load_b128(rsrc, qoff + 4 * (N * h + j) * rs_b, 0, 0));
+#pragma unroll
+        for (int j = 0; j < N; ++j) {
+            const int i = N * h + j, r = 4 * i + (lane >> 4), c = lane & 15;
+            *(lds_chunk_p)(uintptr_t)(stg + (unsigned)(r * 256 + ((c ^ (r & 15)) << 4))) = x[j];
+            amax = q16_chunk_amax<BF16>(x[j], amax);
+        }
+        asm volatile("" : "+v"(qoff) : "v"(amax));
+    }
+    amax = wave_amax(amax);
+    const BlockScale bs = block_scale(amax, qmax);
+    if (bs.fast_div) w64_quantise_q_convert<true, BF16>(stg, lane, bs.sc, bs.rcp1, qlo, qhi);
+    else w64_quantise_q_convert<false, BF16>(stg, lane, bs.sc, bs.rcp1, qlo, qhi);
+    __builtin_amdgcn_fence(__ATOMIC_RELEASE, "wavefront");
+    __builtin_amdgcn_wave_barrier();
+    __builtin_amdgcn_fence(__ATOMIC_ACQUIRE, "wavefront");
+    const int ql = lane & 31, hi = lane >> 5;
+#pragma unroll
+    for (int qb = 0; qb < 2; ++qb) {
+        const int r = 32 * qb + ql;
+#pragma unroll
+        for (int ks = 0; ks < 4; ++ks) {
+            const u32x2_q lo = *(lds_half_p)(uintptr_t)(stg + (unsigned)(r * 256 + (((4 * ks + 2 * hi) ^ (r & 15)) << 4)));
+            const u32x2_q up = *(lds_half_p)(uintptr_t)(stg + (unsigned)(r * 256 + (((4 * ks + 2 * hi + 1) ^ (r & 15)) << 4)));
+            qf[qb][ks] = i32x4{(int)lo.x, (int)lo.y, (int)up.x, (int)up.y};
+        }
+    }
+    return bs.sc;
+}
 
 hipError_t launch_fwd_w64_bias(const W64Params& wp, int family, bool fp32_out, uint32_t grid, size_t lds, hipStream_t stream, int head_dim);
 
diff --git a/universal-metal-flash-attention_amd/csrc/fa_quant.hip b/universal-metal-flash-attention_amd/csrc/fa_quant.hip
--- a/universal-metal-flash-attention_amd/csrc/fa_quant.hip
+++ b/universal-metal-flash-attention_amd/csrc/fa_quant.hip
@@ -4,6 +4,7 @@
 #include <type_traits>
 
 #include "fa_common.h"
+#include "fa_quant_block.h"
 #include "kernels.h"
 
 namespace umfa {
@@ -34,6 +35,7 @@
     uint32_t* vhdr;
     const uint32_t* famax;
     int v_exchange;
+    int v_first;
     uint32_t wait_ticks;
 };
 
@@ -51,27 +53,6 @@
     return (d >> 5) * 2048 + (kk >> 5) * 1024 + (32 * h + (d & 31)) * 16 + b;
 }
 
-__device__ __forceinline__ float div_by_block_scale(float a, float b, float r1) {
-    const float q0 = a * r1;
-    const float e1 = __builtin_fmaf(-b, q0, a);
-    const float q1 = __builtin_fmaf(e1, r1, q0);
-    const float e2 = __builtin_fmaf(-b, q1, a);
-    return __builtin_fmaf(e2, r1, q1);
-}
-
-typedef float f32x2_t __attribute__((ext_vector_type(2)));
-__device__ __forceinline__ void quant_pair_fast(float a0, float a1, float b, float r1, int qlo, int qhi, int& q0, int& q1) {
-    const f32x2_t a = {a0, a1}, bb = {b, b}, rr = {r1, r1};
-    const f32x2_t y0 = a * rr;
-    const f32x2_t e1 = __builtin_elementwise_fma(-bb, y0, a);
-    const f32x2_t y1 = __builtin_elementwise_fma(e1, rr, y0);
-    const f32x2_t e2 = __builtin_elementwise_fma(-bb, y1, a);
-    const f32x2_t y = __builtin_elementwise_fma(e2, rr, y1);
-    const f32x2_t h = {__builtin_copysignf(0x1.fffffep-2f, y[0]), __builtin_copysignf(0x1.fffffep-2f, y[1])};
-    const f32x2_t t = y + h;
-    q0 = max(min((int)t[0], qhi), qlo);
-    q1 = max(min((int)t[1], qhi), qlo);
-}
 
 template <int MODE, bool IN16>
 __global__ __launch_bounds__(256) void quantize_kernel(QuantParams p) {
@@ -236,12 +217,6 @@
     }
 }
 
-typedef unsigned u32x4_q __attribute__((ext_vector_type(4)));
-template <bool BF16> __device__ __forceinline__ float q16_elem(const u32x4_q& x, int j) {
-    const unsigned w = x[j >> 1];
-    if constexpr (BF16) return __uint_as_float((j & 1) ? (w & 0xffff0000u) : (w << 16));
-    return (float)__builtin_bit_cast(_Float16, (uint16_t)((j & 1) ? (w >> 16) : (w & 0xffffu)));
-}
 template <int CPL, bool BF16, bool FAST, bool ISV>
 __device__ __forceinline__ void quantize_wave_convert(const u32x4_q (&xr)[CPL], int lane, uint32_t nchunks, float sc, float rcp1, int qlo, int qhi,
                                                       int8_t* __restrict__ dst8, _Float16* __restrict__ dst16, float scv) {
@@ -250,23 +225,9 @@
         const uint32_t ch = (uint32_t)lane + 64u * c;
         if (ch < nchunks) {
             int q[8];
-            if constexpr (FAST) {
-#pragma unroll
-                for (int j = 0; j < 8; j += 2) quant_pair_fast(q16_elem<BF16>(xr[c], j), q16_elem<BF16>(xr[c], j + 1), sc, rcp1, qlo, qhi, q[j], q[j + 1]);
-            } else {
-#pragma unroll
-                for (int j = 0; j < 8; ++j) {
-                    const float y = q16_elem<BF16>(xr[c], j) / sc;
-                    const float half = __builtin_copysignf(0x1.fffffep-2f, y);
-                    q[j] = max(min((int)(y + half), qhi), qlo);
-                }
-            }
+            quant_chunk<BF16, FAST>(xr[c], sc, rcp1, qlo, qhi, q);
             if constexpr (!ISV) {
-                const uint32_t a0 = __builtin_amdgcn_perm((uint32_t)q[1], (uint32_t)q[0], 0x0c0c0400u);
-                const uint32_t a1 = __builtin_amdgcn_perm((uint32_t)q[3], (uint32_t)q[2], 0x04000c0cu);
-                const uint32_t b0 = __builtin_amdgcn_perm((uint32_t)q[5], (uint32_t)q[4], 0x0c0c0400u);
-                const uint32_t b1 = __builtin_amdgcn_perm((uint32_t)q[7], (uint32_t)q[6], 0x04000c0cu);
-                *(uint2*)(dst8 + (int64_t)ch * 8) = make_uint2(a0 | a1, b0 | b1);
+                *(uint2*)(dst8 + (int64_t)ch * 8) = pack_chunk_i8(q);
             } else {
                 f16x8 hv;
 #pragma unroll
@@ -281,8 +242,14 @@
 __global__ __launch_bounds__(256) void quantize_wave_kernel(QuantParams p) {
     const int lane = threadIdx.x & 63;
     uint32_t id = blockIdx.x * 4 + (threadIdx.x >> 6);
-    int t = p.t_first;
-    while (t < p.t_end - 1 && id >= p.BH * p.nblk[t]) { id -= p.BH * p.nblk[t]; ++t; }
+    int t;
+    if (p.v_first) {
+        t = p.t_end - 1;
+        while (t > p.t_first && id >= p.BH * p.nblk[t]) { id -= p.BH * p.nblk[t]; --t; }
+    } else {
+        t = p.t_first;
+        while (t < p.t_end - 1 && id >= p.BH * p.nblk[t]) { id -= p.BH * p.nblk[t]; ++t; }
+    }
     if (id >= p.BH * p.nblk[t]) return;
     const uint32_t bh = id / p.nblk[t], blk = id % p.nblk[t];
     const uint32_t row0 = blk * QBLK;
@@ -299,11 +266,8 @@
     }
     float amax = 0.0f;
 #pragma unroll
-    for (int c = 0; c < CPL; ++c)
-#pragma unroll
-        for (int j = 0; j < 8; ++j) amax = fmaxf(amax, fabsf(q16_elem<BF16>(xr[c], j)));
-#pragma unroll
-    for (int off = 32; off > 0; off >>= 1) amax = fmaxf(amax, __shfl_xor(amax, off, 64));
+    for (int c = 0; c < CPL; ++c) amax = q16_chunk_amax<BF16>(xr[c], amax);
+    amax = wave_amax(amax);
 #pragma unroll
     for (int c = 0; c < CPL; ++c) asm volatile("" : "+v"(xr[c]));
     int vexp = 0;
@@ -367,11 +331,10 @@
             vexp = vimage_exponent(hw[VSC_HDR_AMAX]);
         }
     }
-    const float sc = amax > 0.0f ? amax / p.qmax : 1.0f;
+    const BlockScale bs = block_scale(amax, p.qmax);
+    const float sc = bs.sc, rcp1 = bs.rcp1;
+    const bool fast_div = bs.fast_div;
     if (lane == 0) p.scale[t][bh * p.nblk[t] + blk] = sc;
-    const float rcp0 = __builtin_amdgcn_rcpf(sc);
-    const float rcp1 = __builtin_fmaf(__builtin_fmaf(-sc, rcp0, 1.0f), rcp0, rcp0);
-    const bool fast_div = __builtin_amdgcn_readfirstlane((int)(sc >= 0x1p-60f && sc <= 0x1p60f)) != 0;
     int8_t* const d8 = (t == 0 ? p.q8 : p.k8) + base;
     _Float16* const d16 = p.v16 + base;
     if (t == 2) {
@@ -857,7 +820,7 @@
 
 hipError_t launch_quantize(const void* q, const void* k, const void* v, int in_prec, uint32_t B, uint32_t H,
                            uint32_t Sq, uint32_t Skv, uint32_t D, int bits, int quant_mode, void* workspace,
-                           int copies, QuantViews* views, hipStream_t stream, uint32_t* overflow, uint32_t* vhdr, const uint32_t* famax) {
+                           int copies, QuantViews* views, hipStream_t stream, uint32_t* overflow, uint32_t* vhdr, const uint32_t* famax, int q_form) {
     if (D > 256) {
         if (copies == 2) return hipErrorInvalidValue;
         return launch_quantize_wide(q, k, v, in_prec, B, H, Sq, Skv, D, bits, quant_mode, workspace, views, stream);
@@ -892,7 +855,6 @@
     qp.qmax = bits == 4 ? 7.0f : 127.0f;
     qp.qlo = bits == 4 ? -8 : -128;
     qp.qhi = bits == 4 ? 7 : 127;
-    const uint32_t grid = qp.BH * (qp.nblk[0] + qp.nblk[1] + qp.nblk[2]);
     const bool f8v = quant_mode == 3 && D == 128 && bits == 8 && !want_f32;
     if (f8v) {
         qp.v8 = (uint8_t*)(ws + w.v16);
@@ -900,14 +862,21 @@
     }
     if (quant_mode == 3) quant_mode = 2;
     const bool in16 = in_prec != P_FP32;
-    qp.t_first = 0; qp.t_end = 3;
+    if (q_form != 0 && !(quant_mode == 2 && in16 && !want_f32 && D == 128)) return hipErrorInvalidValue;
+    qp.t_first = q_form != 0 ? 1 : 0; qp.t_end = 3;
+    qp.v_first = q_form == 1;
+    uint32_t nb_pass = 0;
+    for (int t = qp.t_first; t < qp.t_end; ++t) nb_pass += qp.BH * qp.nblk[t];
+    const uint32_t grid = nb_pass;
     const bool wave_form = quant_mode == 2 && in16 && !want_f32 && !f8v && (D == 128 || D == 64) && !tuning().quant_block_wg.load(std::memory_order_relaxed) &&
                            ((uintptr_t)q & 15) == 0 && ((uintptr_t)k & 15) == 0 && ((uintptr_t)v & 15) == 0;
     bool v_prepass = false;
     if (vhdr && !f8v) {
         qp.vhdr = vhdr;
         qp.wait_ticks = (uint32_t)std::min<int64_t>(std::max(tuning().cast_wait_us.load(std::memory_order_relaxed), 0), 1000000) * 100u;
-        qp.v_exchange = wave_form && qp.nblk[2] % 4 == 0 && qp.nblk[2] / 4 <= 64 && ((uint64_t)qp.BH * (qp.nblk[0] + qp.nblk[1])) % 4 == 0 &&
+        uint64_t waves_before_v = 0;
+        if (!qp.v_first) for (int t = qp.t_first; t < 2; ++t) waves_before_v += (uint64_t)qp.BH * qp.nblk[t];
+        qp.v_exchange = wave_form && qp.nblk[2] % 4 == 0 && qp.nblk[2] / 4 <= 64 && waves_before_v % 4 == 0 &&
                         !tuning().cast_two_pass.load(std::memory_order_relaxed);
         if (!qp.v_exchange) {
             v_prepass = true;
@@ -921,9 +890,7 @@
     }
     if (wave_form) {
         QuantParams qw = qp;
-        uint32_t nb = 0;
-        for (int t = 0; t < qw.t_end; ++t) nb += qp.BH * qp.nblk[t];
-        const dim3 gw((nb + 3) / 4);
+        const dim3 gw((nb_pass + 3) / 4);
         if (D == 128 && in_prec == P_BF16) hipLaunchKernelGGL((quantize_wave_kernel<16, true>), gw, dim3(256), 0, stream, qw);
         else if (D == 128) hipLaunchKernelGGL((quantize_wave_kernel<16, false>), gw, dim3(256), 0, stream, qw);
         else if (in_prec == P_BF16) hipLaunchKernelGGL((quantize_wave_kernel<8, true>), gw, dim3(256), 0, stream, qw);
@@ -994,8 +961,12 @@
     }
     if (quant_mode == 3 && !(bits == 8 && fp.part_buf && fp.part_cnt && fwd_w64_i8_supported(fp) && !fp.mask)) quant_mode = 2;
     QuantViews v;
+    const bool w64 = fp.part_buf && fp.part_cnt && fwd_w64_i8_supported(fp);
+    const int q_pass = tuning().quant_q_pass.load(std::memory_order_relaxed);
+    const bool q_inline = w64 && q_pass != 1 && fp.in_prec != P_FP32 && (quant_mode == 2 || quant_mode == 3) && fp.D == 128 &&
+                          ((uintptr_t)fp.q & 15) == 0 && (uint64_t)fp.Sq * 256u < 0x7fffffffull;
     hipError_t e = launch_quantize(fp.q, fp.k, fp.v, fp.in_prec, fp.B, fp.H, fp.Sq, fp.Skv, fp.D, bits, quant_mode,
-                                   workspace, 0, &v, stream, nullptr, (uint32_t*)fp.vsc);
+                                   workspace, 0, &v, stream, nullptr, (uint32_t*)fp.vsc, nullptr, q_inline ? (q_pass == 2 ? 2 : 1) : 0);
     if (e != hipSuccess) return e;
     I8FwdParams p;
     memset(&p, 0, sizeof(p));
@@ -1004,7 +975,6 @@
     p.vsc = v.v8 ? nullptr : fp.vsc;
     p.o = (float*)fp.o; p.lse = fp.lse;
     p.mask = fp.mask;
-    const bool w64 = fp.part_buf && fp.part_cnt && fwd_w64_i8_supported(fp);
     if (fp.mask && !w64) {
         FwdParams mp = fp;
         if (fp.mask_kind == MK_NONE) {
@@ -1028,7 +998,7 @@
     const uint32_t dp = dp_of(fp.D);
     if (w64) {
         *name = v.v8 ? "fa_fwd_w64_i8f8<128>" : fp.mask ? (bits == 4 ? "fa_fwd_w64_i4<128,mask>" : "fa_fwd_w64_i8<128,mask>") : bits == 4 ? "fa_fwd_w64_i4<128>" : "fa_fwd_w64_i8<128>";
-        return launch_fwd_w64_i8(fp, v, fp.part_buf, fp.part_cnt, stream);
+        return launch_fwd_w64_i8(fp, v, fp.part_buf, fp.part_cnt, stream, q_inline ? fp.q : nullptr, bits);
     }
     if (dp == 64) { *name = bits == 4 ? "fa_fwd_i4<64>" : "fa_fwd_i8<64>"; return launch_i8_flags<64>(p, fp.causal, stream); }
     if (dp == 128) { *name = bits == 4 ? "fa_fwd_i4<128>" : "fa_fwd_i8<128>"; return launch_i8_flags<128>(p, fp.causal, stream); }
diff --git a/universal-metal-flash-attention_amd/csrc/fa_quant_block.h b/universal-metal-flash-attention_amd/csrc/fa_quant_block.h
--- /dev/null
+++ b/universal-metal-flash-attention_amd/csrc/fa_quant_block.h
@@ -0,0 +1,82 @@
+#pragma once
+#include <cstdint>
+
+#include <hip/hip_runtime.h>
+
+namespace umfa {
+
+__device__ __forceinline__ float div_by_block_scale(float a, float b, float r1) {
+    const float q0 = a * r1;
+    const float e1 = __builtin_fmaf(-b, q0, a);
+    const float q1 = __builtin_fmaf(e1, r1, q0);
+    const float e2 = __builtin_fmaf(-b, q1, a);
+    return __builtin_fmaf(e2, r1, q1);
+}
+
+typedef float f32x2_t __attribute__((ext_vector_type(2)));
+__device__ __forceinline__ void quant_pair_fast(float a0, float a1, float b, float r1, int qlo, int qhi, int& q0, int& q1) {
+    const f32x2_t a = {a0, a1}, bb = {b, b}, rr = {r1, r1};
+    const f32x2_t y0 = a * rr;
+    const f32x2_t e1 = __builtin_elementwise_fma(-bb, y0, a);
+    const f32x2_t y1 = __builtin_elementwise_fma(e1, rr, y0);
+    const f32x2_t e2 = __builtin_elementwise_fma(-bb, y1, a);
+    const f32x2_t y = __builtin_elementwise_fma(e2, rr, y1);
+    const f32x2_t h = {__builtin_copysignf(0x1.fffffep-2f, y[0]), __builtin_copysignf(0x1.fffffep-2f, y[1])};
+    const f32x2_t t = y + h;
+    q0 = max(min((int)t[0], qhi), qlo);
+    q1 = max(min((int)t[1], qhi), qlo);
+}
+
+typedef unsigned u32x4_q __attribute__((ext_vector_type(4)));
+template <bool BF16> __device__ __forceinline__ float q16_elem(const u32x4_q& x, int j) {
+    const unsigned w = x[j >> 1];
+    if constexpr (BF16) return __uint_as_float((j & 1) ? (w & 0xffff0000u) : (w << 16));
+    return (float)__builtin_bit_cast(_Float16, (uint16_t)((j & 1) ? (w >> 16) : (w & 0xffffu)));
+}
+template <bool BF16> __device__ __forceinline__ float q16_chunk_amax(const u32x4_q& x, float amax) {
+#pragma unroll
+    for (int j = 0; j < 8; ++j) amax = fmaxf(amax, fabsf(q16_elem<BF16>(x, j)));
+    return amax;
+}
+__device__ __forceinline__ float wave_amax(float amax) {
+#pragma unroll
+    for (int off = 32; off > 0; off >>= 1) amax = fmaxf(amax, __shfl_xor(amax, off, 64));
+    return amax;
+}
+
+struct BlockScale {
+    float sc, rcp1;
+    bool fast_div;
+};
+__device__ __forceinline__ BlockScale block_scale(float amax, float qmax) {
+    BlockScale b;
+    b.sc = amax > 0.0f ? amax / qmax : 1.0f;
+    const float rcp0 = __builtin_amdgcn_rcpf(b.sc);
+    b.rcp1 = __builtin_fmaf(__builtin_fmaf(-b.sc, rcp0, 1.0f), rcp0, rcp0);
+    b.fast_div = __builtin_amdgcn_readfirstlane((int)(b.sc >= 0x1p-60f && b.sc <= 0x1p60f)) != 0;
+    return b;
+}
+
+template <bool BF16, bool FAST>
+__device__ __forceinline__ void quant_chunk(const u32x4_q& x, float sc, float rcp1, int qlo, int qhi, int (&q)[8]) {
+    if constexpr (FAST) {
+#pragma unroll
+        for (int j = 0; j < 8; j += 2) quant_pair_fast(q16_elem<BF16>(x, j), q16_elem<BF16>(x, j + 1), sc, rcp1, qlo, qhi, q[j], q[j + 1]);
+    } else {
+#pragma unroll
+        for (int j = 0; j < 8; ++j) {
+            const float y = q16_elem<BF16>(x, j) / sc;
+            const float half = __builtin_copysignf(0x1.fffffep-2f, y);
+            q[j] = max(min((int)(y + half), qhi), qlo);
+        }
+    }
+}
+__device__ __forceinline__ uint2 pack_chunk_i8(const int (&q)[8]) {
+    const uint32_t a0 = __builtin_amdgcn_perm((uint32_t)q[1], (uint32_t)q[0], 0x0c0c0400u);
+    const uint32_t a1 = __builtin_amdgcn_perm((uint32_t)q[3], (uint32_t)q[2], 0x04000c0cu);
+    const uint32_t b0 = __builtin_amdgcn_perm((uint32_t)q[5], (uint32_t)q[4], 0x0c0c0400u);
+    const uint32_t b1 = __builtin_amdgcn_perm((uint32_t)q[7], (uint32_t)q[6], 0x04000c0cu);
+    return make_uint2(a0 | a1, b0 | b1);
+}
+
+}
diff --git a/universal-metal-flash-attention_amd/csrc/kernels.h b/universal-metal-flash-attention_amd/csrc/kernels.h
--- a/universal-metal-flash-attention_amd/csrc/kernels.h
+++ b/universal-metal-flash-attention_amd/csrc/kernels.h
@@ -25,6 +25,7 @@
         cast_two_pass{0} , bwd_ds_lab{0} ,
         cast_u{0} ,
         quant_block_wg{0} ,
+        quant_q_pass{1} ,
         cast_wait_us{100} ,
         decode_ks{0} ,
         cbal{0} ,
@@ -152,11 +153,13 @@
                            uint32_t Sq, uint32_t Skv, uint32_t D, int bits, int quant_mode, void* workspace,
                            int copies, QuantViews* views, hipStream_t stream, uint32_t* overflow = nullptr,
                            uint32_t* vhdr = nullptr ,
-                           const uint32_t* famax = nullptr );
+                           const uint32_t* famax = nullptr ,
+                           int q_form = 0 );
 hipError_t launch_quantized_fwd(const FwdParams& fp, int bits, int quant_mode, void* workspace, hipStream_t stream,
                                 const char** name);
 bool fwd_w64_i8_supported(const FwdParams& p);
-hipError_t launch_fwd_w64_i8(const FwdParams& p, const QuantViews& v, float* part_buf, uint32_t* part_cnt, hipStream_t stream);
+hipError_t launch_fwd_w64_i8(const FwdParams& p, const QuantViews& v, float* part_buf, uint32_t* part_cnt, hipStream_t stream, const void* q16 = nullptr,
+                             int bits = 8);
 
 size_t mask_pack_bytes(const FwdParams& p);
 hipError_t launch_mask_pack(FwdParams& p, void* scratch, hipStream_t stream);
diff --git a/universal-metal-flash-attention_amd/csrc/tuning.hip b/universal-metal-flash-attention_amd/csrc/tuning.hip
--- a/universal-metal-flash-attention_amd/csrc/tuning.hip
+++ b/universal-metal-flash-attention_amd/csrc/tuning.hip
@@ -56,6 +56,7 @@
         x->cast_two_pass.store(env_flag("UMFA_CAST_TWO_PASS"));
         x->cast_u.store(env_int("UMFA_CAST_U", 0));
         x->quant_block_wg.store(env_flag("UMFA_QUANT_BLOCK_WG"));
+        x->quant_q_pass.store(env_int("UMFA_QUANT_Q_PASS", 1));
         x->cast_wait_us.store(env_int("UMFA_CAST_WAIT_US", 100));
         x->bwd_ds_lab.store(env_int("UMFA_LAB_DS", 0));
         x->cbal.store(env_int("UMFA_CBAL", 0));
@@ -93,7 +94,7 @@
         {"bwd_persist", &t.bwd_persist, true}, {"bwd_separate_delta", &t.bwd_separate_delta, true},
         {"no_split", &t.no_split, true}, {"force_split", &t.force_split, false}, {"no_dma", &t.no_dma, true},
         {"bn64", &t.bn64, true}, {"pv_fp16", &t.pv_fp16, true}, {"bwd_ds_store", &t.bwd_ds_store, true}, {"no_w64_mask", &t.no_w64_mask, true}, {"ksplit", &t.ksplit, true}, {"no_pipe", &t.no_pipe, true}, {"no_w64_mask_lazy", &t.no_w64_mask_lazy, true}, {"no_w64_bias", &t.no_w64_bias, true}, {"no_w64_f32_mask", &t.no_w64_f32_mask, true}, {"f32_mask_ratio", &t.f32_mask_ratio, false}, {"mask_pass_ratio", &t.mask_pass_ratio, false}, {"no_w64_ragged_mask", &t.no_w64_ragged_mask, true}, {"no_mask_realign", &t.no_mask_realign, true}, {"no_bwd_mask", &t.no_bwd_mask, true}, {"sdpa_dropout", &t.sdpa_dropout, true},
-        {"cast_two_pass", &t.cast_two_pass, true}, {"bwd_ds_lab", &t.bwd_ds_lab, false}, {"cast_u", &t.cast_u, false}, {"quant_block_wg", &t.quant_block_wg, true},
+        {"cast_two_pass", &t.cast_two_pass, true}, {"bwd_ds_lab", &t.bwd_ds_lab, false}, {"cast_u", &t.cast_u, false}, {"quant_block_wg", &t.quant_block_wg, true}, {"quant_q_pass", &t.quant_q_pass, false},
         {"cast_wait_us", &t.cast_wait_us, false}, {"cbal", &t.cbal, false}, {"cbal_delta", &t.cbal_delta, false}, {"decode_ks", &t.decode_ks, false}, {"sync_chunks", &t.sync_chunks, false}, {"sync_chunked_calls", &t.sync_chunked_calls, false}, {"mirror_cache_hits", &t.mirror_cache_hits, false},
     };
     for (auto& e : tab)
@@ -119,7 +120,7 @@
             {"no_mask_flags", &t.no_mask_flags}, {"bwd_exact", &t.bwd_exact}, {"bwd_dq", &t.bwd_dq}, {"bwd_persist", &t.bwd_persist},
             {"bwd_separate_delta", &t.bwd_separate_delta}, {"no_split", &t.no_split}, {"force_split", &t.force_split},
             {"no_dma", &t.no_dma}, {"bn64", &t.bn64}, {"pv_fp16", &t.pv_fp16}, {"bwd_ds_store", &t.bwd_ds_store}, {"no_w64_mask", &t.no_w64_mask}, {"ksplit", &t.ksplit}, {"no_pipe", &t.no_pipe}, {"no_w64_mask_lazy", &t.no_w64_mask_lazy}, {"no_w64_bias", &t.no_w64_bias}, {"no_w64_f32_mask", &t.no_w64_f32_mask}, {"f32_mask_ratio", &t.f32_mask_ratio}, {"mask_pass_ratio", &t.mask_pass_ratio}, {"no_w64_ragged_mask", &t.no_w64_ragged_mask}, {"no_mask_realign", &t.no_mask_realign}, {"no_bwd_mask", &t.no_bwd_mask}, {"sdpa_dropout", &t.sdpa_dropout},
-            {"cast_two_pass", &t.cast_two_pass}, {"bwd_ds_lab", &t.bwd_ds_lab}, {"cast_u", &t.cast_u}, {"quant_block_wg", &t.quant_block_wg},
+            {"cast_two_pass", &t.cast_two_pass}, {"bwd_ds_lab", &t.bwd_ds_lab}, {"cast_u", &t.cast_u}, {"quant_block_wg", &t.quant_block_wg}, {"quant_q_pass", &t.quant_q_pass},
             {"cast_wait_us", &t.cast_wait_us}, {"cbal", &t.cbal}, {"cbal_delta", &t.cbal_delta}, {"decode_ks", &t.decode_ks}, {"sync_chunks", &t.sync_chunks}, {"sync_chunked_calls", &t.sync_chunked_calls}, {"mirror_cache_hits", &t.mirror_cache_hits},
         };
         const std::atomic<int>* v = nullptr;
diff --git a/universal-metal-flash-attention_amd/umfa_torch/ops.py b/universal-metal-flash-attention_amd/umfa_torch/ops.py
--- a/universal-metal-flash-attention_amd/umfa_torch/ops.py
+++ b/universal-metal-flash-attention_amd/umfa_torch/ops.py
@@ -37,7 +37,7 @@
 
 _OPTION_NAMES = ("softmax_reference", "softmax_tau", "w64_tau", "force_w64", "no_w64", "w64_grid", "w64_skew", "no_mask_flags", "bwd_exact",
                  "bwd_dq", "bwd_persist", "bwd_separate_delta", "no_split", "force_split", "no_dma", "bn64", "pv_fp16", "bwd_ds_store", "no_w64_mask", "ksplit", "no_pipe", "no_w64_mask_lazy", "no_w64_bias", "no_w64_f32_mask", "f32_mask_ratio", "mask_pass_ratio", "no_w64_ragged_mask", "no_mask_realign",
-                 "cast_two_pass", "bwd_ds_lab", "cast_u", "quant_block_wg", "cast_wait_us", "cbal", "cbal_delta", "decode_ks", "sync_chunks", "sync_chunked_calls", "mirror_cache_hits", "no_bwd_mask", "sdpa_dropout")
+                 "cast_two_pass", "bwd_ds_lab", "cast_u", "quant_block_wg", "quant_q_pass", "cast_wait_us", "cbal", "cbal_delta", "decode_ks", "sync_chunks", "sync_chunked_calls", "mirror_cache_hits", "no_bwd_mask", "sdpa_dropout")
 
 
 def get_option(name: str) -> str:
```

New measurement: 1070, median of 2. No clear change (+0.1%).
